# jolideco/jolideco

Hardware: AMD Instinct MI355X
Metric: MAP iters/sec at 2048x2048, 8-obs joint fit (higher is better)
Workload: dtype f32; 1 GPU; c3: 2048x2048, 8 observations (Gaussian PSFs sigma = 1.5 + 0.25 i on 6 x 17x17 + 2 x 33x33, varying exposure/background), GMM patch prior 8x8 stride 4 K=128, joint fit, Adam lr 0.1; global_observations=8, conv_method=separable

## Files before the change

include/jolideco_hip.h:

```cpp
#ifndef JOLIDECO_HIP_H
#define JOLIDECO_HIP_H

#include <stddef.h>
#include <stdint.h>

#ifdef __cplusplus
extern "C" {
#endif

typedef enum {
  JD_OK = 0,
  JD_ERR_INVALID = -1,
  JD_ERR_HIP = -2,
  JD_ERR_FFT = -3,
  JD_ERR_ALLOC = -4
} jd_status;

#define JD_MAX_COMPONENTS 8

typedef struct jd_conv_plan jd_conv_plan;
typedef struct jd_gmm jd_gmm;

int jd_version(void);
const char* jd_last_error(void);
// ... 14 lines not shown
int jd_conv_plan_destroy(jd_conv_plan* plan);
int jd_conv_plan_shape(const jd_conv_plan* plan, int* shape6);
int jd_conv_plan_method(const jd_conv_plan* plan);
int jd_conv_native_fft_supported(int H, int W, int kh, int kw);
int jd_conv_plan_takes_walk(const jd_conv_plan* plan, int n_datasets);
int jd_conv_plan_step_route(const jd_conv_plan* plan, int upsampling, int n_datasets, int32_t* route8);
int jd_conv_operator_walk_frame(const jd_conv_plan* plan, const float* khat);
int jd_conv_operator_forget(const float* khat);
size_t jd_conv_plan_spectrum_size(const jd_conv_plan* plan);

int jd_conv_psf_spectrum(jd_conv_plan* plan, const float* psf, float* khat, void* stream);

int jd_conv_same(jd_conv_plan* plan, const float* image, const float* scale_image, const float* khat,
                 float* out, void* stream);

int jd_npred_poisson_fwd_bwd(jd_conv_plan* plan, int n_comp, const float* const* flux,
                             const float* const* exposure, const float* const* khat,
                             const float* background, const float* counts, float stirling_mean,
                             float eps, float* loss_out, float* const* grad_flux, int accumulate,
                             float grad_scale, float* npred_out, int upsampling, void* stream);

int jd_npred_poisson_mixed_fwd_bwd(jd_conv_plan* const* plans, int n_comp, const float* const* flux,
                                   const float* const* exposure, const float* const* khat, const float* background,
                                   const float* counts, float stirling_mean, float eps, float* loss_out,
                                   float* const* grad_flux, int accumulate, float grad_scale, float* npred_out,
                                   const int* upsampling, void* stream);

int jd_npred_poisson_batch_fwd_bwd(jd_conv_plan* plan, int n_datasets, const float* flux, const float* const* exposure,
                                   const float* const* khat, const float* const* background,
                                   const float* const* counts, const float* stirling_mean, float eps,
                                   float* const* loss_out, float* grad_flux, int accumulate, float grad_scale,
                                   void* stream);

int jd_npred_poisson_batch_multi_fwd_bwd(jd_conv_plan* plan, int n_datasets, int n_components, const float* const* flux,
                                         const float* const* exposure, const float* const* khat,
                                         const float* const* background, const float* const* counts,
                                         const float* stirling_mean, float eps, float* const* loss_out,
                                         float* const* grad_flux, int accumulate, float grad_scale, void* stream);

int jd_npred_poisson_calibrated_fwd_bwd(jd_conv_plan* plan, int n_comp, const float* const* flux,
                                        const float* const* exposure, const float* const* khat,
                                        const float* background, const float* counts, float stirling_mean,
                                        float eps, float* loss_out, float* const* grad_flux, int accumulate,
                                        float grad_scale, float* npred_out, int upsampling, const float* shift_xy,
                                        const float* log_background_norm, float* grad_shift_xy,
                                        float* grad_log_background_norm, void* stream);

int jd_npred_poisson_calibrated_batch_fwd_bwd(jd_conv_plan* plan, int n_datasets, const float* flux,
                                              const float* const* exposure, const float* const* khat,
                                              const float* const* background, const float* const* counts,
                                              const float* stirling_mean, float eps, float* const* loss_out,
                                              float* grad_flux, int accumulate, float grad_scale, int upsampling,
                                              const float* const* shift_xy, const float* const* log_background_norm,
                                              float* const* grad_shift_xy, float* const* grad_log_background_norm,
                                              void* stream);

int jd_poisson_nll(const float* npred, const float* counts, size_t n, float stirling_mean, float eps,
                   float* loss_out, float* grad_npred ,
                   void* stream);
int jd_conv_same_adjoint(jd_conv_plan* plan, const float* grad_out, const float* scale_image,
                         const float* khat, float* grad_image, int accumulate, void* stream);

int jd_gmm_create(int K, int D, const float* prec_chol, const float* mu_prec, const float* const_k,
                  const float* pixel_w, jd_gmm** gmm_out);
int jd_gmm_destroy(jd_gmm* gmm);
int jd_gmm_is_triangular(const jd_gmm* gmm);

typedef struct {
  int kind;
  float p0, p1;
} jd_image_norm;
int jd_gmm_set_image_norm(jd_gmm* gmm, const jd_image_norm* norm);

int jd_gmm_prior_fwd_bwd(jd_gmm* gmm, const float* flux, int H, int W, int stride, int shift_y,
                         int shift_x, int patch_row_begin, int patch_row_end, int marginalize,
                         float value_scale, float* value_out, int accumulate_value, float grad_coef,
                         float* grad_flux_accum, int32_t* argmax_out, const int* shift_dev, int phases, void* stream);

typedef struct {
  float* theta;
  const float* flux_in;
  float* flux_out;
  const float* grad_flux;
  float* exp_avg;
  float* exp_avg_sq;
  const float* mask;
  float step_size, beta1, beta2, one_minus_beta1, one_minus_beta2, bias2_sqrt, eps;
  float lr;
  int use_log_flux, sgd;
  const float* bias_dev;
} jd_step;
int jd_gmm_prior_fwd_bwd_step(jd_gmm* gmm, const float* flux, int H, int W, int stride, int shift_y, int shift_x,
                              int marginalize, float value_scale, float* value_out, int accumulate_value,
                              float grad_coef, const jd_step* step, const int* shift_dev, int phases, void* stream);

int jd_gmm_screen_stats(const jd_gmm* gmm, int* out);
int jd_gmm_screen_clock(jd_gmm* gmm, double* mhz_out, int* samples_out);

int jd_gmm_prior_band_fwd_bwd(jd_gmm* gmm, const float* flux, int H, int W, int stride, int shift_y,
                              int shift_x, int patch_row_begin, int patch_row_end, int marginalize,
                              float value_scale, float* value_out, int accumulate_value, float grad_coef,
                              float* band_out, void* stream);
int jd_add_rolled_bands(float* grad, int H, int W, int shift_y, int shift_x, const float* bands, size_t chunk_floats,
                        int n_bands, const int* y_begin, const int* y_end, void* stream);
int jd_add_rolled_bands_step(int H, int W, int shift_y, int shift_x, const float* bands, size_t chunk_floats, int n_bands,
                             const int* y_begin, const int* y_end, const jd_step* step, void* stream);

int jd_gmm_estimate_log_prob(jd_gmm* gmm, const float* x, int n, float* out, void* stream);

int jd_elementwise_prior_fwd_bwd(int kind, const float* flux, size_t n, float alpha, float beta,
                                 float log_const, float* value_out, float grad_coef,
                                 float* grad_flux_accum, void* stream);
int jd_elementwise_prior_subpix_fwd_bwd(int kind, const float* flux, int H, int W, float alpha, float beta,
                                        float log_const, float x0, float y0, const float* offset_dev,
                                        float* value_out, float grad_coef, float* grad_flux_accum, void* stream);
int jd_smoothness_prior_fwd_bwd(jd_conv_plan* plan, const float* khat, const float* flux, float* value_out,
                                float grad_coef, float* grad_flux_accum, void* stream);

int jd_flux_from_theta(const float* theta, const float* mask, float* flux, size_t n, int use_log_flux, void* stream);

int jd_sum_images(float* out, const float* const* srcs, int n_srcs, size_t n, void* stream);
int jd_copy_image_to(const float* src, float* const* dsts, int n_dsts, size_t n, void* stream);

int jd_step_scalars_fetch(const int32_t* host_row, int32_t* dst, int n, void* stream);

int jd_adam_step(float* theta, const float* flux_in, float* flux_out, float* grad_flux, float* exp_avg,
                 float* exp_avg_sq, const float* mask, size_t n, float step_size, float beta1,
                 float beta2, float one_minus_beta1, float one_minus_beta2, float bias2_sqrt, float eps,
                 int zero_grad, int use_log_flux, const float* bias_dev, void* stream);
int jd_adam_step_multi(int n_tensors, float* const* theta, const float* const* grad, float* const* exp_avg,
                       float* const* exp_avg_sq, const int* sizes, const float* step_size, const float* bias2_sqrt,
                       float beta1, float beta2, float one_minus_beta1, float one_minus_beta2, float eps,
                       const float* bias_dev, void* stream);
int jd_sgd_step(float* theta, const float* flux_in, float* flux_out, float* grad_flux,
                const float* mask, size_t n, float lr, int zero_grad, int use_log_flux, void* stream);

int jd_sparse_max_sources(void);
int jd_sparse_render(const float* param_flux, const float* x_pos, const float* y_pos, int n, int use_log_flux, int H,
                     int W, float* flux_out, void* stream);
int jd_sparse_backward(const float* param_flux, const float* x_pos, const float* y_pos, int n, int use_log_flux, int H,
                       int W, const float* grad_flux_image, float* grad_param, float* grad_x, float* grad_y,
                       void* stream);

enum {
  JD_KERNEL_POISSON_FUSED = 0,
  JD_KERNEL_GMM_FWD = 1,
  JD_KERNEL_GMM_BWD = 2,
  JD_KERNEL_GMM_GATHER = 3,
  JD_KERNEL_PAD_MUL = 4,
  JD_KERNEL_CMUL = 5,
  JD_KERNEL_ADJOINT_EPILOGUE = 6,
  JD_KERNEL_ADAM = 7,
  JD_KERNEL_FFT_R2C = 8,
  JD_KERNEL_FFT_C2R = 9,
  JD_KERNEL_DIRECT_CONV = 10,
  JD_KERNEL_SEP_CONV = 11,
  JD_KERNEL_GMM_SCREEN = 12,
  JD_KERNEL_GMM_SORT = 13,
  JD_KERNEL_GMM_EXACT = 14,
  JD_KERNEL_GMM_STAGE = 15,
  JD_KERNEL_SHIFT = 16,
  JD_KERNEL_POISSON_MIXED = 17,
// ... 19 lines not shown
```

jolideco_amd/_hip.py:

```python
import ctypes
import os
from ctypes import POINTER, c_char_p, c_double, c_float, c_int, c_int32, c_longlong, c_size_t, c_void_p
from pathlib import Path

import torch

__all__ = ["lib", "library_path", "check", "ptr", "stream_ptr", "EXPORTS"]

LIB_NAME = "libjolideco_hip.so"


def library_path():
    override = os.environ.get("JOLIDECO_HIP_LIBRARY")
    return Path(override) if override else Path(__file__).resolve().parent / LIB_NAME


fp = POINTER(c_float)
fpp = POINTER(c_void_p)

EXPORTS = {
    "jd_version": (c_int, []),
    "jd_last_error": (c_char_p, []),
    "jd_target_arch": (c_char_p, []),
    "jd_set_option": (c_int, [c_char_p, c_char_p]),
# ... 6 lines not shown
    "jd_conv_native_fft_supported": (c_int, [c_int, c_int, c_int, c_int]),
    "jd_conv_plan_takes_walk": (c_int, [c_void_p, c_int]),
    "jd_conv_plan_step_route": (c_int, [c_void_p, c_int, c_int, POINTER(c_int32)]),
    "jd_conv_operator_walk_frame": (c_int, [c_void_p, c_void_p]),
    "jd_conv_operator_forget": (c_int, [c_void_p]),
    "jd_psf_separable_rank": (c_int, [c_void_p, c_int, c_int, c_float]),
    "jd_conv_psf_spectrum": (c_int, [c_void_p, c_void_p, c_void_p, c_void_p]),
    "jd_conv_same": (c_int, [c_void_p, c_void_p, c_void_p, c_void_p, c_void_p, c_void_p]),
    "jd_conv_same_adjoint": (c_int, [c_void_p, c_void_p, c_void_p, c_void_p, c_void_p, c_int, c_void_p]),
    "jd_npred_poisson_fwd_bwd": (
        c_int,
        [c_void_p, c_int, fpp, fpp, fpp, c_void_p, c_void_p, c_float, c_float, c_void_p, fpp, c_int, c_float,
         c_void_p, c_int, c_void_p],
    ),
    "jd_npred_poisson_mixed_fwd_bwd": (
        c_int,
        [fpp, c_int, fpp, fpp, fpp, c_void_p, c_void_p, c_float, c_float, c_void_p, fpp, c_int, c_float, c_void_p,
         POINTER(c_int), c_void_p],
    ),
    "jd_npred_poisson_calibrated_fwd_bwd": (
        c_int,
        [c_void_p, c_int, fpp, fpp, fpp, c_void_p, c_void_p, c_float, c_float, c_void_p, fpp, c_int, c_float,
         c_void_p, c_int, c_void_p, c_void_p, c_void_p, c_void_p, c_void_p],
    ),
    "jd_npred_poisson_calibrated_batch_fwd_bwd": (
        c_int,
        [c_void_p, c_int, c_void_p, fpp, fpp, fpp, fpp, fp, c_float, fpp, c_void_p, c_int, c_float, c_int, fpp, fpp, fpp, fpp,
         c_void_p],
    ),
    "jd_npred_poisson_batch_fwd_bwd": (
        c_int,
        [c_void_p, c_int, c_void_p, fpp, fpp, fpp, fpp, fp, c_float, fpp, c_void_p, c_int, c_float, c_void_p],
    ),
    "jd_npred_poisson_batch_multi_fwd_bwd": (
        c_int,
        [c_void_p, c_int, c_int, fpp, fpp, fpp, fpp, fpp, fp, c_float, fpp, fpp, c_int, c_float, c_void_p],
    ),
    "jd_poisson_nll": (c_int, [c_void_p, c_void_p, c_size_t, c_float, c_float, c_void_p, c_void_p, c_void_p]),
    "jd_gmm_create": (c_int, [c_int, c_int, fp, fp, fp, fp, POINTER(c_void_p)]),
    "jd_gmm_destroy": (c_int, [c_void_p]),
    "jd_gmm_is_triangular": (c_int, [c_void_p]),
    "jd_gmm_set_image_norm": (c_int, [c_void_p, c_void_p]),
    "jd_gmm_prior_fwd_bwd": (
        c_int,
        [c_void_p, c_void_p, c_int, c_int, c_int, c_int, c_int, c_int, c_int, c_int, c_float, c_void_p, c_int,
         c_float, c_void_p, c_void_p, c_void_p, c_int, c_void_p],
    ),
    "jd_gmm_prior_fwd_bwd_step": (
        c_int,
        [c_void_p, c_void_p, c_int, c_int, c_int, c_int, c_int, c_int, c_float, c_void_p, c_int, c_float, c_void_p, c_void_p,
         c_int, c_void_p],
    ),
    "jd_gmm_screen_stats": (c_int, [c_void_p, POINTER(c_int)]),
    "jd_gmm_screen_clock": (c_int, [c_void_p, POINTER(c_double), POINTER(c_int)]),
    "jd_gmm_prior_band_fwd_bwd": (
        c_int,
        [c_void_p, c_void_p, c_int, c_int, c_int, c_int, c_int, c_int, c_int, c_int, c_float, c_void_p, c_int,
         c_float, c_void_p, c_void_p],
    ),
    "jd_add_rolled_bands": (
        c_int, [c_void_p, c_int, c_int, c_int, c_int, c_void_p, c_size_t, c_int, POINTER(c_int), POINTER(c_int), c_void_p],
    ),
    "jd_add_rolled_bands_step": (
        c_int, [c_int, c_int, c_int, c_int, c_void_p, c_size_t, c_int, POINTER(c_int), POINTER(c_int), c_void_p, c_void_p],
    ),
    "jd_gmm_estimate_log_prob": (c_int, [c_void_p, c_void_p, c_int, c_void_p, c_void_p]),
    "jd_elementwise_prior_fwd_bwd": (
        c_int,
        [c_int, c_void_p, c_size_t, c_float, c_float, c_float, c_void_p, c_float, c_void_p, c_void_p],
    ),
    "jd_elementwise_prior_subpix_fwd_bwd": (
        c_int,
        [c_int, c_void_p, c_int, c_int, c_float, c_float, c_float, c_float, c_float, c_void_p, c_void_p, c_float, c_void_p,
         c_void_p],
    ),
    "jd_smoothness_prior_fwd_bwd": (c_int, [c_void_p, c_void_p, c_void_p, c_void_p, c_float, c_void_p, c_void_p]),
    "jd_flux_from_theta": (c_int, [c_void_p, c_void_p, c_void_p, c_size_t, c_int, c_void_p]),
    "jd_sum_images": (c_int, [c_void_p, c_void_p, c_int, c_size_t, c_void_p]),
    "jd_copy_image_to": (c_int, [c_void_p, c_void_p, c_int, c_size_t, c_void_p]),
    "jd_step_scalars_fetch": (c_int, [c_void_p, c_void_p, c_int, c_void_p]),
    "jd_adam_step": (
        c_int,
        [c_void_p, c_void_p, c_void_p, c_void_p, c_void_p, c_void_p, c_void_p, c_size_t, c_float, c_float, c_float,
         c_float, c_float, c_float, c_float, c_int, c_int, c_void_p, c_void_p],
    ),
    "jd_adam_step_multi": (
        c_int,
        [c_int, fpp, fpp, fpp, fpp, POINTER(c_int), fp, fp, c_float, c_float, c_float, c_float, c_float, c_void_p, c_void_p],
    ),
    "jd_sgd_step": (c_int, [c_void_p, c_void_p, c_void_p, c_void_p, c_void_p, c_size_t, c_float, c_int, c_int, c_void_p]),
    "jd_sparse_max_sources": (c_int, []),
    "jd_sparse_render": (c_int, [c_void_p, c_void_p, c_void_p, c_int, c_int, c_int, c_int, c_void_p, c_void_p]),
    "jd_sparse_backward": (
        c_int, [c_void_p, c_void_p, c_void_p, c_int, c_int, c_int, c_int, c_void_p, c_void_p, c_void_p, c_void_p, c_void_p],
    ),
    "jd_profile_enable": (c_int, [c_int]),
    "jd_profile_disable": (c_int, []),
    "jd_profile_pause": (c_int, [c_int]),
    "jd_profile_read": (c_int, [c_int, POINTER(c_double), POINTER(c_longlong)]),
    "jd_kernel_name": (c_char_p, [c_int]),
    "jd_clock_probe": (c_int, [c_double, POINTER(c_double), c_void_p]),
}

class Step(ctypes.Structure):

    _fields_ = [
        ("theta", c_void_p), ("flux_in", c_void_p), ("flux_out", c_void_p), ("grad_flux", c_void_p), ("exp_avg", c_void_p),
        ("exp_avg_sq", c_void_p), ("mask", c_void_p),
        ("step_size", c_float), ("beta1", c_float), ("beta2", c_float), ("one_minus_beta1", c_float),
        ("one_minus_beta2", c_float), ("bias2_sqrt", c_float), ("eps", c_float), ("lr", c_float),
        ("use_log_flux", c_int), ("sgd", c_int), ("bias_dev", c_void_p),
    ]


class ImageNormStruct(ctypes.Structure):

    _fields_ = [("kind", c_int), ("p0", c_float), ("p1", c_float)]


KERNEL_IDS = {
    "poisson_fused": 0, "gmm_fwd": 1, "gmm_bwd": 2, "gmm_gather": 3, "pad_mul": 4, "cmul": 5,
    "adjoint_epilogue": 6, "adam": 7, "fft_r2c": 8, "fft_c2r": 9, "direct_conv": 10, "sep_conv": 11,
    "gmm_screen": 12, "gmm_sort": 13, "gmm_exact": 14, "gmm_stage": 15, "shift": 16,
    "poisson_mixed": 17, "elementwise_subpix": 18, "smoothness": 19, "elementwise_prior": 20,
    "sparse_render": 21, "sparse_backward": 22,
}

_lib = None


def lib():
    global _lib
    if _lib is None:
        path = library_path()
        if not path.exists():
            raise RuntimeError(
                f"{path} not found: the HIP extension is required (no CPU fallback). "
                "Build it with `make -C jolideco_amd/csrc` or `python -c 'import __graft_entry__ as g; g.build()'`."
            )
        handle = ctypes.CDLL(str(path))
        for name, (restype, argtypes) in EXPORTS.items():
            fn = getattr(handle, name)
            fn.restype = restype
            fn.argtypes = argtypes
# ... 102 lines not shown
```

jolideco_amd/core.py:

```python
import copy
import ctypes
import os
import logging
from pathlib import Path

import numpy as np
import torch

from . import _hip
from ._hip import check, ptr, ptr_array, stream_ptr
from .distributed import DistContext
from .loss import TotalLoss
from .models import FluxComponents, SparseSpatialFluxComponent, SpatialFluxComponent
from .ops import adam_bias_terms, sparse_backward, sparse_render
from .utils.torch import TORCH_DEFAULT_DEVICE

log = logging.getLogger(__name__)

__all__ = ["MAPDeconvolver", "MAPDeconvolverResult", "FitSession"]

OPTIMIZER = ("adam", "sgd")
FIT_MODES = ("sequential", "joint")


# ... 115 lines not shown
        self.device = device
        if optimizer_type not in OPTIMIZER:
            raise ValueError(f"Unknown optimizer: {optimizer_type}, must be one of {OPTIMIZER}")
        self.optimizer_type = optimizer_type
        self.optimizer_kwargs = dict(optimizer_kwargs or {})
        self.optimizer_kwargs.setdefault("lr", self.learning_rate)
        unknown = set(self.optimizer_kwargs) - {"lr", "betas", "eps"}
        if unknown:
            raise NotImplementedError(f"optimizer_kwargs {sorted(unknown)} are not implemented in jolideco_amd")
        if checkpoint_path is not None:
            checkpoint_path = Path(checkpoint_path)
            checkpoint_path.mkdir(exist_ok=True, parents=True)
        self.checkpoint_path = checkpoint_path
        if fit_mode not in FIT_MODES:
            raise ValueError(f"Unknown fit_mode: {fit_mode}, must be one of {FIT_MODES}")
        self.fit_mode = fit_mode

    def to_dict(self):
        data = {k: v for k, v in self.__dict__.items() if k not in ("optimizer_kwargs",)}
        data["device"] = str(self.device)
        data["checkpoint_path"] = str(self.checkpoint_path)
        return data

    def __str__(self):
        lines = [self.__class__.__name__, "-" * len(self.__class__.__name__), ""]
        lines += [f"  {k:22s}: {v}" for k, v in self.to_dict().items()]
        return "\n".join(lines)

    def _step_args(self, st, step, bias_dev=None):
        lr = self.optimizer_kwargs["lr"]
        args = _hip.Step()
        args.theta, args.flux_in, args.flux_out = st.theta.data_ptr(), st.flux_cur.data_ptr(), st.flux[1 - st.cur].data_ptr()
        args.grad_flux = st.grad.data_ptr()
        args.mask = None if st.mask is None else st.mask.data_ptr()
        args.use_log_flux = int(st.use_log_flux)
        if self.optimizer_type == "adam":
            beta1, beta2 = self.optimizer_kwargs.get("betas", (0.9, 0.999))
            args.step_size, args.bias2_sqrt = adam_bias_terms(step, lr, beta1, beta2)
            args.beta1, args.beta2, args.one_minus_beta1, args.one_minus_beta2 = beta1, beta2, 1 - beta1, 1 - beta2
            args.eps = self.optimizer_kwargs.get("eps", 1e-8)
            args.exp_avg, args.exp_avg_sq = st.exp_avg.data_ptr(), st.exp_avg_sq.data_ptr()
            args.sgd = 0
            args.bias_dev = None if bias_dev is None else bias_dev.data_ptr()
        else:
            args.lr, args.sgd = lr, 1
        return args

    def _optimizer_step(self, states, step, stepped=()):
        lib = _hip.lib()
        lr = self.optimizer_kwargs["lr"]
        for ci, st in enumerate(states):
            n = st.grad.numel()
            stream = stream_ptr(st.grad.device)
            if ci in stepped:
                pass
            elif st.frozen:
                st.flux[1 - st.cur].copy_(st.flux_cur)
                st.grad.zero_()
            elif getattr(st, "is_sparse", False):
                st.step(step)
            elif self.optimizer_type == "adam":
                beta1, beta2 = self.optimizer_kwargs.get("betas", (0.9, 0.999))
                eps = self.optimizer_kwargs.get("eps", 1e-8)
                step_size, bias2_sqrt = adam_bias_terms(step, lr, beta1, beta2)
                check(
                    lib.jd_adam_step(
# ... 325 lines not shown

        from . import _hip as _hip_mod

        own_step = getattr(type(deconvolver), "_optimizer_step", None) is MAPDeconvolver._optimizer_step
        tiled = _hip_mod.get_option("JD_GMM_GATHER_TILED") in (None, 1)
        self.fuse_optimizer_step = bool(own_step and "_optimizer_step" not in vars(deconvolver) and tiled
                                        and not os.environ.get("JOLIDECO_NO_FUSED_STEP"))
        self._setup_sharded_prior(os.environ.get("JOLIDECO_DIST_OVERLAP", "1") != "0")
        batchable = not os.environ.get("JOLIDECO_NO_BATCH") and self.total_loss.poisson_loss.batchable(
            [li for _, li in self.local_idx]
        )
        self.batch_joint = self.joint and batchable
        self.flux_nonneg = all(
            st.use_log_flux and (st.mask is None or bool((st.mask >= 0).all())) for st in self.states
        )
        self.batch_joint_calibrated = bool(
            self.joint and not batchable and not os.environ.get("JOLIDECO_NO_BATCH") and self.n_c == 1
            and self.total_loss.poisson_loss.batchable_calibrated([li for _, li in self.local_idx])
        )
        self.batch_trace = (not self.joint) and batchable
        mode = os.environ.get("JOLIDECO_GRAPH", "auto").lower()
        self.graph_mode = {"1": "always", "on": "always", "0": "never", "off": "never"}.get(mode, "auto")
        if getattr(deconvolver, "use_graph", None) is not None:
            self.graph_mode = "always" if deconvolver.use_graph else "never"
        self.use_graph = self.graph_mode == "always"
        self.graph_policy = {"always": "captured epochs (forced)", "never": "no capture (forced)"}.get(self.graph_mode, "undecided")
        self._probe = []
        self._trial = None
        self.overlap_mode = {"1": "on", "0": "off"}.get(os.environ.get("JOLIDECO_PRIOR_OVERLAP", ""), "auto")
        self.overlap_prior = self.overlap_mode != "off"
        side_priority = int(os.environ.get("JOLIDECO_PRIOR_STREAM_PRIORITY", "0"))
        self._side_stream = (torch.cuda.Stream(device=device, priority=side_priority)
                             if torch.device(device).type == "cuda" else None)
        self.step_scalars = None
        self._graphs = {}
        self._epochs_done = 0
        self._total_epochs = 0
        self._planned_ok = os.environ.get("JOLIDECO_STEP_SCALARS", "device") != "host"

    def gather_calibrations(self):
        cals, dist = self.calibrations, self.dist
        if cals is None or not (self.joint and dist.sharded) or dist.dry_run:
            return
        names = self.total_loss.poisson_loss.names_all_global
        mine = {names[gslot] for gslot, _ in self.local_idx}
        flat = torch.zeros(3 * len(names), dtype=torch.float32, device=self.comm.device)
        for i, name in enumerate(names):
            if name in mine and name in cals:
                cal = cals[name]
                flat[3 * i : 3 * i + 2] = cal.shift_xy.detach().reshape(-1).to(flat.device)
                flat[3 * i + 2] = cal._background_norm.detach().reshape(-1)[0].to(flat.device)
        dist.all_reduce_sum(flat)
        host = flat.cpu()
        for i, name in enumerate(names):
            if name not in mine and name in cals:
                cal = cals[name]
                with torch.no_grad():
                    cal.shift_xy.copy_(host[3 * i : 3 * i + 2].reshape(1, 2))
                    cal._background_norm.copy_(host[3 * i + 2 : 3 * i + 3])

    def _setup_sharded_prior(self, overlap):
        from .ops import band_rows

        self.band_plan = None
        dist = self.dist
        if not (self.joint and dist.sharded):
# ... 168 lines not shown
            H, W = self.states[ci].shape
            shifts_host.append((drawn[0] % H, drawn[1] % W))
            return DeviceShifts(slot, drawn)

        if len(drawing) == 1:
            ci = drawing[0]
            for drawn in self.priors[ci].draw_shifts_many(n_eval):
                shifts.append({ci: place(ci, drawn)})
        else:
            for _ in range(n_eval):
                shifts.append({ci: place(ci, self.priors[ci].draw_shifts()) for ci in drawing})
        biases = [adam_bias_terms(self.step + j + 1, lr, beta1, beta2) if adam else (0.0, 1.0) for j in range(n_flux)]
        flux_bias = [sc.bias_slots[j] if adam else None for j in range(n_flux)]
        cal_bias, cal_items, k = [], [], n_flux
        for group in cal_groups:
            items = [(p, st) for opt in group for p, st in zip(opt.params, opt.state) if p.grad is not None]
            for _, st in items:
                biases.append(adam_bias_terms(st["step"] + 1, lr, beta1, beta2) if adam else (0.0, 1.0))
            cal_bias.append(sc.bias_range(k, len(items)) if (adam and items) else None)
            cal_items.append(items)
            k += len(items)
        sc.upload(shifts_host, biases)
        return {"shifts": shifts, "flux_bias": flux_bias, "cal_bias": cal_bias, "cal_items": cal_items, "n_steps": n_flux,
                "signature": tuple(len(items) for items in cal_items)}

    def _plan_by_value(self):
        drawing, _, n_flux, cal_groups, _ = self._plan_slots()
        n_eval = 1 if self.joint else len(self.local_idx) + 1
        shifts = [{ci: self.priors[ci].draw_shifts() for ci in drawing} for _ in range(n_eval)]
        cal_items = [[(p, st) for opt in group for p, st in zip(opt.params, opt.state)] for group in cal_groups]
        return {"shifts": shifts, "flux_bias": [None] * n_flux, "cal_bias": [None] * len(cal_groups), "cal_items": cal_items,
                "n_steps": n_flux, "signature": ()}

    def _overlap_active(self):
        return self.overlap_prior and self._side_stream is not None and not self.dist.sharded and not _hip.profile_active()

    def _prior_calls(self, coef, shifts, bias):
        cfg, n_d, slot, step_no = self.cfg, self.n_d, self._slot, self.step + 1
        calls = []
        for ci, (st, prior) in enumerate(zip(self.states, self.priors)):
            if getattr(prior, "value_is_zero", False):
                continue
            kwargs = {"shifts": shifts[ci]} if ci in shifts else {}
            flux, value = st.flux_cur, slot(n_d + ci)
            if self._fuse_step(st, prior):
                args = cfg._step_args(st, step_no, bias)

                def call(phases=3, prior=prior, flux=flux, value=value, args=args, kwargs=kwargs):
                    prior.device_fwd_bwd_step(flux, value, coef, args, **(dict(kwargs, phases=phases) if phases != 3 else kwargs))

                calls.append((ci, call, True))
            else:

                def call(phases=3, prior=prior, flux=flux, value=value, grad=st.grad, kwargs=kwargs):
                    prior.device_fwd_bwd(flux, value, grad=grad, coef=coef, **(dict(kwargs, phases=phases) if phases != 3 else kwargs))

                calls.append((ci, call, False))
        return calls

    def _start_priors(self, calls):
        if not self._overlap_active():
            return set()
        eligible, seen = [], set()
        for ci, call, _ in calls:
            prior = self.priors[ci]
            key = id(getattr(prior, "gmm", prior))
            if getattr(prior, "supports_phases", False) and key not in seen:
                seen.add(key)
                eligible.append((ci, call))
        if not eligible:
            return set()
        main = torch.cuda.current_stream(self.comm.device)
        self._side_stream.wait_stream(main)
        with torch.cuda.stream(self._side_stream):
            for _, call in eligible:
                call(1)
        return {ci for ci, _ in eligible}

    def _finish_priors(self, calls, early):
        if early:
            torch.cuda.current_stream(self.comm.device).wait_stream(self._side_stream)
# ... 54 lines not shown
        beta = -float(cfg.beta)

        def flux_step(stepped, bias):
            self.step += 1
            for st in states:
                st.bias_dev = bias
            try:
                self._apply_step(states, stepped)
            finally:
                for st in states:
                    st.bias_dev = None

        def cal_steps(items, bias):
            if not items:
                return
            if cfg.optimizer_type != "adam":
                lr = cfg.optimizer_kwargs["lr"]
                for p, st in items:
                    if p.grad is None:
                        continue
                    st["step"] += 1
                    check(_hip.lib().jd_sgd_step(ptr(p.data), ptr(p.data), ptr(p.data), ptr(p.grad), None, p.numel(), lr, 0, 0,
                                                 stream_ptr(p.device)))
                return
            _adam_step_many(cfg, items, self.__dict__.setdefault("_cal_step_cache", {}), bias)

        if self.joint:
            fluxes = [st.flux_cur for st in states]
            grads = [st.grad for st in states]
            calls = self._prior_calls(beta, plan["shifts"][0], plan["flux_bias"][0])
            early = self._start_priors(calls)
            first = True
            if self.batch_joint:
                total_loss.poisson_loss.fwd_bwd_batch(
                    [li for _, li in self.local_idx], fluxes if n_c > 1 else fluxes[0],
                    [slot(gslot) for gslot, _ in self.local_idx], grad=grads if n_c > 1 else grads[0], accumulate=False,
                    flux_nonneg=self.flux_nonneg,
                )
                first = False
            elif self.batch_joint_calibrated:
                for _, li in self.local_idx:
                    self._cal_zero_grad(li)
                total_loss.poisson_loss.fwd_bwd_batch_calibrated(
                    [li for _, li in self.local_idx], fluxes[0], [slot(gslot) for gslot, _ in self.local_idx], grad=grads[0],
                    accumulate=False,
                )
                first = False
            else:
                for gslot, li in self.local_idx:
                    self._cal_zero_grad(li)
                    total_loss.poisson_loss.fwd_bwd(li, fluxes, slot(gslot), grads=grads, accumulate=not first,
                                                    flux_nonneg=self.flux_nonneg)
                    first = False
            if first:
                for g in grads:
                    g.zero_()
            flux_step(self._finish_priors(calls, early), plan["flux_bias"][0])
            cal_steps(plan["cal_items"][0], plan["cal_bias"][0])
        else:
            coef = beta / total_loss.prior_weight
            for j, (gslot, li) in enumerate(self.local_idx):
                fluxes = [st.flux_cur for st in states]
                grads = [st.grad for st in states]
                calls = self._prior_calls(coef, plan["shifts"][j], plan["flux_bias"][j])
                early = self._start_priors(calls)
                self._cal_zero_grad(li)
                total_loss.poisson_loss.fwd_bwd(li, fluxes, slot(gslot), grads=grads, accumulate=False,
                                                flux_nonneg=self.flux_nonneg)
                flux_step(self._finish_priors(calls, early), plan["flux_bias"][j])
                cal_steps(plan["cal_items"][j], plan["cal_bias"][j])
            stale = [st.flux_trace for st in states]
# ... 91 lines not shown
        trial["times"][self.overlap_prior] = 1e-3 * float(np.median([a.elapsed_time(b) for a, b in trial["events"][2:]]))
        trial["events"] = []
        remaining = [form for form in trial["forms"] if form not in trial["times"]]
        if remaining:
            self.overlap_prior, self._graphs, self._epochs_done = remaining[0], {}, 0
            return
        times, by_value_s = trial["times"], trial["by_value"]
        best = min(times, key=times.get)
        self._trial = None
        replays = " / ".join(f"{1e6 * t:.0f} us {'on two streams' if form else 'on one stream'}" for form, t in times.items())
        numbers = (f"replayed {replays} / by value {1e6 * by_value_s:.0f} us per epoch, enqueue {1e6 * trial['host']:.0f} us"
                   f"{trial['streams']}")
        if times[best] <= self.AUTO_MARGIN * by_value_s:
            self.graph_policy = f"captured epochs (measured: {numbers})"
            if best != self.overlap_prior:
                self.overlap_prior, self._graphs, self._epochs_done = best, {}, 0
        else:
            self.use_graph = False
            self._graphs = {}
            self.overlap_prior = trial["by_value_form"]
            self.graph_policy = f"by value (measured: {numbers})"

    def _epoch_by_value(self):
        cfg, dist, states, priors, total_loss = self.cfg, self.dist, self.states, self.priors, self.total_loss
        n_d, n_c = self.n_d, self.n_c
        slot = self._slot
        if self.joint:
            fluxes = [st.flux_cur for st in states]
            grads = [st.grad for st in states]
            if dist.sharded:
                self.scalars.zero_()
            first = True
            if self.batch_joint:
                total_loss.poisson_loss.fwd_bwd_batch(
                    [li for _, li in self.local_idx], fluxes if n_c > 1 else fluxes[0],
                    [slot(gslot) for gslot, _ in self.local_idx], grad=grads if n_c > 1 else grads[0], accumulate=False,
                    flux_nonneg=self.flux_nonneg,
                )
                first = False
            elif self.batch_joint_calibrated:
                for _, li in self.local_idx:
                    self._cal_zero_grad(li)
                total_loss.poisson_loss.fwd_bwd_batch_calibrated(
                    [li for _, li in self.local_idx], fluxes[0], [slot(gslot) for gslot, _ in self.local_idx], grad=grads[0],
                    accumulate=False,
                )
                first = False
            else:
                for gslot, li in self.local_idx:
                    self._cal_zero_grad(li)
                    total_loss.poisson_loss.fwd_bwd(li, fluxes, slot(gslot), grads=grads, accumulate=not first,
                                                    flux_nonneg=self.flux_nonneg)
                    first = False
            if first:
                for g in grads:
                    g.zero_()
            banded = {item["ci"]: item for item in (self.band_plan or [])}
            stepped = set()
            for ci, (st, prior) in enumerate(zip(states, priors)):
                if ci in banded:
                    continue
                if dist.sharded and not prior.shardable and dist.rank != 0:
                    continue
                if self._fuse_step(st, prior):
                    prior.device_fwd_bwd_step(st.flux_cur, slot(n_d + ci), -float(cfg.beta), cfg._step_args(st, self.step + 1))
                    stepped.add(ci)
                    continue
                prior.device_fwd_bwd(
                    st.flux_cur, slot(n_d + ci), grad=st.grad, coef=-float(cfg.beta),
                    patch_rows=self._prior_rows(prior, st),
                )
# ... 199 lines not shown
```

jolideco_amd/csrc/elementwise.hip:

```cpp
#include <cstdint>
#include <cstdlib>

#include "jd_common.h"
#include "kernels.h"
#include "jd_adam.h"

namespace jd {

constexpr int BLOCK = 256;

__global__ __launch_bounds__(BLOCK) void finalize_sum_kernel(const double* __restrict__ partials, int n,
                                                            double scale, double offset,
                                                            float* __restrict__ out, int accumulate) {
  __shared__ double smem[BLOCK / 64];
  double acc = 0.0;
  for (int i = threadIdx.x; i < n; i += BLOCK) acc += partials[i];
  double total = block_sum<BLOCK>(acc, smem);
  if (threadIdx.x == 0) {
    double v = scale * total + offset;
    if (accumulate) v += (double)out[0];
    out[0] = (float)v;
  }
}

// ... 531 lines not shown
                                                    int ox) {
  const int y = blockIdx.y;
  const int x = blockIdx.x * BLOCK + threadIdx.x;
  if (x >= W) return;
  out[(size_t)y * W + x] = padded[(size_t)(y + oy) * Wp + (x + ox)];
}

int launch_crop(const float* padded, float* out, int H, int W, int Wp, int oy, int ox, hipStream_t stream) {
  dim3 grid((W + BLOCK - 1) / BLOCK, H);
  crop_kernel<<<grid, BLOCK, 0, stream>>>(padded, out, H, W, Wp, oy, ox);
  JD_LAUNCH_CHECK();
  return JD_OK;
}

__global__ __launch_bounds__(BLOCK) void poisson_nll_kernel(const float* __restrict__ npred,
                                                           const float* __restrict__ counts, size_t n,
                                                           float eps, float inv_n,
                                                           float* __restrict__ grad,
                                                           double* __restrict__ partials) {
  __shared__ double smem[BLOCK / 64];
  double local = 0.0;
  const size_t stride = (size_t)gridDim.x * BLOCK;
  for (size_t i = (size_t)blockIdx.x * BLOCK + threadIdx.x; i < n; i += stride) {
    const float v = npred[i], c = counts[i];
    float term, g;
    poisson_point(v, c, eps, inv_n, term, g);
    local += (double)term;
    if (grad) grad[i] = g;
  }
  const double total = block_sum<BLOCK>(local, smem);
  if (threadIdx.x == 0) partials[blockIdx.x] = total;
}

template <int VEC>
__global__ __launch_bounds__(BLOCK) void adam_kernel(AdamArgs a) {
  use_device_bias(a);
  const size_t stride = (size_t)gridDim.x * BLOCK * VEC;
  for (size_t i = ((size_t)blockIdx.x * BLOCK + threadIdx.x) * VEC; i < a.n; i += stride) {
    float th[VEC], f[VEC], gf[VEC], m[VEC], v[VEC], mk[VEC];
    if constexpr (VEC == 4) {
      const float4 t4 = *reinterpret_cast<const float4*>(a.theta + i);
      const float4 f4 = *reinterpret_cast<const float4*>(a.flux_in + i);
      const float4 g4 = *reinterpret_cast<const float4*>(a.grad_flux + i);
      th[0] = t4.x, th[1] = t4.y, th[2] = t4.z, th[3] = t4.w;
      f[0] = f4.x, f[1] = f4.y, f[2] = f4.z, f[3] = f4.w;
      gf[0] = g4.x, gf[1] = g4.y, gf[2] = g4.z, gf[3] = g4.w;
      if (!a.sgd) {
        const float4 m4 = *reinterpret_cast<const float4*>(a.m + i);
        const float4 v4 = *reinterpret_cast<const float4*>(a.v + i);
        m[0] = m4.x, m[1] = m4.y, m[2] = m4.z, m[3] = m4.w;
        v[0] = v4.x, v[1] = v4.y, v[2] = v4.z, v[3] = v4.w;
      }
      mk[0] = mk[1] = mk[2] = mk[3] = 1.f;
      if (a.mask) {
        const float4 k4 = *reinterpret_cast<const float4*>(a.mask + i);
        mk[0] = k4.x, mk[1] = k4.y, mk[2] = k4.z, mk[3] = k4.w;
      }
    } else {
      th[0] = a.theta[i], f[0] = a.flux_in[i], gf[0] = a.grad_flux[i];
      if (!a.sgd) m[0] = a.m[i], v[0] = a.v[i];
      mk[0] = a.mask ? a.mask[i] : 1.f;
    }
#pragma unroll
    for (int k = 0; k < VEC; ++k) adam_pixel(th[k], f[k], m[k], v[k], gf[k], mk[k], a);
    if constexpr (VEC == 4) {
      *reinterpret_cast<float4*>(a.theta + i) = make_float4(th[0], th[1], th[2], th[3]);
      *reinterpret_cast<float4*>(a.flux_out + i) = make_float4(f[0], f[1], f[2], f[3]);
      if (!a.sgd) {
        *reinterpret_cast<float4*>(a.m + i) = make_float4(m[0], m[1], m[2], m[3]);
        *reinterpret_cast<float4*>(a.v + i) = make_float4(v[0], v[1], v[2], v[3]);
      }
      if (a.zero_grad) *reinterpret_cast<float4*>(a.grad_flux + i) = make_float4(0.f, 0.f, 0.f, 0.f);
    } else {
      a.theta[i] = th[0], a.flux_out[i] = f[0];
      if (!a.sgd) a.m[i] = m[0], a.v[i] = v[0];
      if (a.zero_grad) a.grad_flux[i] = 0.f;
    }
  }
}

static int launch_adam(const AdamArgs& a, hipStream_t stream) {
  const bool vec = (a.n % 4 == 0);
  const size_t per_block = (size_t)BLOCK * (vec ? 4 : 1);
  size_t blocks = (a.n + per_block - 1) / per_block;
  if (blocks > 4096) blocks = 4096;
  if (blocks == 0) blocks = 1;
  ProfScope prof(JD_KERNEL_ADAM, stream);
  if (vec)
    adam_kernel<4><<<(unsigned)blocks, BLOCK, 0, stream>>>(a);
  else
    adam_kernel<1><<<(unsigned)blocks, BLOCK, 0, stream>>>(a);
  JD_LAUNCH_CHECK();
  return JD_OK;
}

__global__ __launch_bounds__(BLOCK) void flux_from_theta_kernel(const float* __restrict__ theta,
                                                               const float* __restrict__ mask,
                                                               float* __restrict__ flux, size_t n, int linear) {
  const size_t stride = (size_t)gridDim.x * BLOCK;
  for (size_t i = (size_t)blockIdx.x * BLOCK + threadIdx.x; i < n; i += stride) {
    float f = linear ? theta[i] : expf(theta[i]);
    if (mask) f *= mask[i];
    flux[i] = f;
  }
}

__global__ __launch_bounds__(BLOCK) void elementwise_prior_kernel(int kind, const float* __restrict__ flux,
                                                                 size_t n, float alpha, float beta,
                                                                 float coef, float* __restrict__ grad,
                                                                 double* __restrict__ partials) {
  __shared__ double smem[BLOCK / 64];
  double local = 0.0;
  const size_t stride = (size_t)gridDim.x * BLOCK;
  for (size_t i = (size_t)blockIdx.x * BLOCK + threadIdx.x; i < n; i += stride) {
    const float f = flux[i];
    float value, dv;
    if (kind == 1) {
      value = -beta / f + (-alpha - 1.f) * logf(f);
      dv = beta / (f * f) + (-alpha - 1.f) / f;
    } else {
      value = -alpha * f;
      dv = -alpha;
    }
    local += (double)value;
// ... 323 lines not shown
  ImagePtrs p{};
  for (int c = 0; c < n_srcs; ++c) {
    JD_REQUIRE(srcs[c], "jd_sum_images: source %d is null", c);
    p.src[c] = srcs[c];
  }
  p.n_src = n_srcs, p.dst[0] = out, p.n_dst = 1;
  return launch_sum_images(p, n, stream);
}

extern "C" int jd_copy_image_to(const float* src, float* const* dsts, int n_dsts, size_t n, void* stream) {
  JD_REQUIRE(src && dsts && n > 0, "jd_copy_image_to: null argument or n == 0");
  JD_REQUIRE(n_dsts >= 1 && n_dsts <= 4, "jd_copy_image_to: %d destination images (1 to 4)", n_dsts);
  ImagePtrs p{};
  p.src[0] = src, p.n_src = 1;
  for (int d = 0; d < n_dsts; ++d) {
    JD_REQUIRE(dsts[d] && dsts[d] != src, "jd_copy_image_to: destination %d is null or the source", d);
    p.dst[d] = dsts[d];
  }
  p.n_dst = n_dsts;
  return launch_sum_images(p, n, stream);
}

__global__ __launch_bounds__(256) void fetch_scalars_kernel(const int* __restrict__ src, int* __restrict__ dst, int n) {
  for (int i = threadIdx.x; i < n; i += 256) dst[i] = src[i];
}

extern "C" int jd_step_scalars_fetch(const int32_t* host_row, int32_t* dst, int n, void* stream) {
  JD_REQUIRE(host_row && dst && n > 0 && n <= (1 << 20), "jd_step_scalars_fetch: null argument or bad n");
  fetch_scalars_kernel<<<1, 256, 0, as_stream(stream)>>>(host_row, dst, n);
  JD_LAUNCH_CHECK();
  return JD_OK;
}

extern "C" int jd_adam_step(float* theta, const float* flux_in, float* flux_out, float* grad_flux,
                            float* exp_avg, float* exp_avg_sq, const float* mask, size_t n, float step_size,
                            float beta1, float beta2, float one_minus_beta1, float one_minus_beta2,
                            float bias2_sqrt, float eps, int zero_grad, int use_log_flux, const float* bias_dev,
                            void* stream) {
  JD_REQUIRE(theta && flux_in && flux_out && grad_flux && exp_avg && exp_avg_sq && n > 0,
             "jd_adam_step: null argument or n == 0");
  AdamArgs a{theta, flux_in, flux_out, grad_flux, exp_avg, exp_avg_sq, mask, n,
             step_size, beta1, beta2, one_minus_beta1, one_minus_beta2, bias2_sqrt, eps, 0.f, zero_grad, 0,
             use_log_flux ? 0 : 1, bias_dev};
  return launch_adam(a, as_stream(stream));
}

constexpr int ADAM_MULTI_MAX = 64;
struct AdamMultiArgs {
  float* theta[ADAM_MULTI_MAX];
  const float* grad[ADAM_MULTI_MAX];
  float* m[ADAM_MULTI_MAX];
  float* v[ADAM_MULTI_MAX];
  int size[ADAM_MULTI_MAX];
  float step_size[ADAM_MULTI_MAX], bias2_sqrt[ADAM_MULTI_MAX];
  float beta1, beta2, one_minus_beta1, one_minus_beta2, eps;
  const float* bias_dev;
};

__global__ __launch_bounds__(64) void adam_multi_kernel(AdamMultiArgs a) {
  float* theta = nullptr;
  const float* grad = nullptr;
  float *m = nullptr, *v = nullptr;
  int size = 0;
  AdamArgs s{};
  s.beta1 = a.beta1, s.beta2 = a.beta2, s.one_minus_beta1 = a.one_minus_beta1, s.one_minus_beta2 = a.one_minus_beta2, s.eps = a.eps;
#pragma unroll
  for (int i = 0; i < ADAM_MULTI_MAX; ++i)
    if ((int)blockIdx.x == i) {
      theta = a.theta[i], grad = a.grad[i], m = a.m[i], v = a.v[i], size = a.size[i];
      s.step_size = a.step_size[i], s.bias2_sqrt = a.bias2_sqrt[i];
    }
  if (a.bias_dev) s.step_size = a.bias_dev[2 * blockIdx.x], s.bias2_sqrt = a.bias_dev[2 * blockIdx.x + 1];
  for (int j = threadIdx.x; j < size; j += 64) {
    float th = theta[j], mj = m[j], vj = v[j];
    adam_update(th, mj, vj, grad[j], s);
    theta[j] = th, m[j] = mj, v[j] = vj;
  }
// ... 36 lines not shown
```

jolideco_amd/csrc/fftconv.hip:

```cpp
#include <rocfft/rocfft.h>

#include <algorithm>
#include <cstdio>
#include <cstdlib>
#include <mutex>

#include "jd_common.h"
#include "kernels.h"

#define JD_FFT(call)                                                                               \
  do {                                                                                             \
    rocfft_status s_ = (call);                                                                     \
    if (s_ != rocfft_status_success)                                                               \
      return jd::fail(JD_ERR_FFT, "%s failed with rocfft_status %d (%s:%d)", #call, (int)s_,       \
                      __FILE__, __LINE__);                                                         \
  } while (0)

struct jd_conv_plan {
  int H = 0, W = 0, kh = 0, kw = 0, Hp = 0, Wp = 0, oy = 0, ox = 0;
  int method = jd::JD_CONV_FFT;
  int py = 0, px = 0;
  size_t nspec = 0;
  int split = 0;
  bool native = false;
  jd::FftNative fftn;
  rocfft_plan fwd = nullptr, inv = nullptr;
  rocfft_execution_info info = nullptr;
  void* work = nullptr;
  size_t work_bytes = 0;
  float* pad[JD_MAX_COMPONENTS] = {nullptr};
  float* conv[JD_MAX_COMPONENTS] = {nullptr};
  float2* spec = nullptr;
  double* partials = nullptr;
  int partials_cap = 0;
  float* shifted[JD_MAX_COMPONENTS] = {nullptr};
  float* gshift[JD_MAX_COMPONENTS] = {nullptr};
  double* partials_cal = nullptr;
  float* gbatch[jd::SEP_MAX_BATCH * jd::SEP_BATCH_MAX_COMP] = {nullptr};
  double* partials_batch = nullptr;
  int partials_batch_cap = 0;
  float2* fft_extra_spec[jd::FFT_MAX_BATCH - 1] = {nullptr};
  float2* fft_extra_work[jd::FFT_MAX_BATCH - 1] = {nullptr};
  static constexpr int N_FFT_TABLES = 6;
  jd::FftBatch fft_batch_host[N_FFT_TABLES] = {};
  jd::FftBatch* fft_batch_dev[N_FFT_TABLES] = {};
  unsigned long long fft_batch_used[N_FFT_TABLES] = {};
  unsigned long long fft_batch_clock = 0;
  double* partials_shift_batch = nullptr;
  float* gshift_batch[jd::FFT_MAX_BATCH] = {nullptr};
  int partials_shift_batch_cap = 0;
  static constexpr int N_TABLES = 8;
  jd::SepBatchTable table_host[N_TABLES] = {};
  jd::SepBatchTable* table_dev[N_TABLES] = {};
  unsigned long long table_used[N_TABLES] = {};
  unsigned long long table_clock = 0;
};

namespace jd {

static bool is_smooth(int n) {
  for (int p : {2, 3, 5})
    while (n % p == 0) n /= p;
  return n == 1;
}

static int next_fast_len(int n, int mult) {
  int m = ((n + mult - 1) / mult) * mult;
  while (!is_smooth(m)) m += mult;
  return m;
}

static int ensure_component_buffers(jd_conv_plan* p, int n_comp) {
  const size_t bytes = (size_t)p->Hp * p->Wp * sizeof(float);
  for (int c = 0; c < n_comp; ++c) {
    if (!p->pad[c]) JD_HIP(hipMalloc(&p->pad[c], bytes));
    if (!p->conv[c]) JD_HIP(hipMalloc(&p->conv[c], bytes));
  }
  return JD_OK;
}

static int ensure_calibration_buffers(jd_conv_plan* p, int n_comp, bool shift) {
  if (!p->partials_cal) {
    const size_t n = (size_t)(p->partials_cap > 2 * shift_bwd_max_blocks(p->H, p->W) ? p->partials_cap
                                                                                    : 2 * shift_bwd_max_blocks(p->H, p->W));
    JD_HIP(hipMalloc(&p->partials_cal, n * sizeof(double)));
  }
  if (shift) {
    const size_t bytes = (size_t)p->H * p->W * sizeof(float);
// ... 188 lines not shown
    return cleanup(fail(JD_ERR_ALLOC, "jd_conv_plan_create: hipMalloc of the spectrum buffer failed"));
  p->partials_cap = poisson_fused_max_partials(p->Hp, p->Wp);
  if (hipMalloc(&p->partials, (size_t)p->partials_cap * sizeof(double)) != hipSuccess)
    return cleanup(fail(JD_ERR_ALLOC, "jd_conv_plan_create: hipMalloc of the partial sums failed"));
  int rc = ensure_component_buffers(p, 1);
  if (rc) return cleanup(rc);
  *plan_out = p;
  return JD_OK;
}

extern "C" int jd_conv_plan_destroy(jd_conv_plan* p) {
  if (!p) return JD_OK;
  (void)hipDeviceSynchronize();
  if (p->native) fftn_destroy(&p->fftn);
  for (int i = 0; i < jd::FFT_MAX_BATCH - 1; ++i) {
    if (p->fft_extra_spec[i]) (void)hipFree(p->fft_extra_spec[i]);
    if (p->fft_extra_work[i]) (void)hipFree(p->fft_extra_work[i]);
  }
  for (auto* t : p->fft_batch_dev)
    if (t) (void)hipFree(t);
  if (p->partials_shift_batch) (void)hipFree(p->partials_shift_batch);
  for (int i = 0; i < jd::FFT_MAX_BATCH; ++i)
    if (p->gshift_batch[i]) (void)hipFree(p->gshift_batch[i]);
  if (p->fwd) rocfft_plan_destroy(p->fwd);
  if (p->inv) rocfft_plan_destroy(p->inv);
  if (p->info) rocfft_execution_info_destroy(p->info);
  if (p->work) (void)hipFree(p->work);
  if (p->spec) (void)hipFree(p->spec);
  if (p->partials) (void)hipFree(p->partials);
  if (p->partials_cal) (void)hipFree(p->partials_cal);
  if (p->partials_batch) (void)hipFree(p->partials_batch);
  for (auto* t : p->table_dev)
    if (t) (void)hipFree(t);
  for (float* g : p->gbatch)
    if (g) (void)hipFree(g);
  for (int c = 0; c < JD_MAX_COMPONENTS; ++c) {
    if (p->pad[c]) (void)hipFree(p->pad[c]);
    if (p->conv[c]) (void)hipFree(p->conv[c]);
    if (p->shifted[c]) (void)hipFree(p->shifted[c]);
    if (p->gshift[c]) (void)hipFree(p->gshift[c]);
  }
  delete p;
  return JD_OK;
}

extern "C" int jd_conv_plan_shape(const jd_conv_plan* p, int* shape6) {
  JD_REQUIRE(p && shape6, "jd_conv_plan_shape: null argument");
  shape6[0] = p->H, shape6[1] = p->W, shape6[2] = p->Hp, shape6[3] = p->Wp, shape6[4] = p->oy, shape6[5] = p->ox;
  return JD_OK;
}

extern "C" size_t jd_conv_plan_spectrum_size(const jd_conv_plan* p) { return p ? p->nspec : 0; }

extern "C" int jd_conv_plan_method(const jd_conv_plan* p) { return p ? p->method : -1; }

extern "C" int jd_conv_native_fft_supported(int H, int W, int kh, int kw) {
  return H > 0 && W > 0 && kh > 0 && kw > 0 && opt_value(OPT_FFT_NATIVE, 1) != 0 && fftn_supported(H, W, kh, kw) ? 1 : 0;
}

extern "C" int jd_conv_plan_takes_walk(const jd_conv_plan* p, int n_datasets) {
  if (!p || p->method != JD_CONV_SEPARABLE || n_datasets < 1) return 0;
  return walk_takes_launch(p->H, p->W, n_datasets, p->kh, p->kw, p->oy, p->ox) ? 1 : 0;
}

extern "C" int jd_conv_operator_walk_frame(const jd_conv_plan* p, const float* khat) {
  if (!p || !khat || p->method != JD_CONV_SEPARABLE) return 0;
// ... 260 lines not shown
      if (plans[k] == p) ++slot[c];
  }
  jd_conv_plan* p0 = plans[0];
  JD_REQUIRE(poisson_mixed_max_partials(Hd, Wd) <= p0->partials_cap, "%s: partial sums of a (%d, %d) counts grid do not fit plans[0]",
             who, Hd, Wd);
  hipStream_t s = as_stream(stream);
  int rc = JD_OK;
  for (int c = 0; c < n_comp; ++c)
    if ((rc = ensure_component_buffers(plans[c], slot[c] + 1))) return rc;

  for (int c = 0; c < n_comp; ++c)
    if ((rc = conv_forward(plans[c], slot[c], flux[c], exposure[c], khat[c], s))) return rc;

  PoissonMixedArgs a{};
  for (int c = 0; c < n_comp; ++c) {
    const jd_conv_plan* p = plans[c];
    a.conv[c] = p->conv[slot[c]], a.g[c] = p->pad[slot[c]];
    a.up[c] = upsampling[c], a.Wp[c] = p->Wp, a.oy[c] = p->py, a.ox[c] = p->px;
  }
  const double n_pix = (double)Hd * (double)Wd;
  a.background = background, a.counts = counts, a.npred_out = npred_out, a.partials = p0->partials;
  a.n_comp = n_comp, a.Hd = Hd, a.Wd = Wd, a.eps = eps, a.inv_n = (float)(1.0 / n_pix);
  a.write_grad = grad_flux ? 1 : 0;
  int n_partials = 0;
  if ((rc = launch_poisson_mixed(a, &n_partials, s))) return rc;
  if ((rc = launch_finalize_sum(p0->partials, n_partials, 1.0 / n_pix, (double)stirling_mean, loss_out, 0, s))) return rc;
  if (!grad_flux) return JD_OK;

  for (int c = 0; c < n_comp; ++c)
    if ((rc = corr_backward_into(plans[c], slot[c], khat[c], exposure[c], grad_flux[c], grad_scale, accumulate, s))) return rc;
  return JD_OK;
}

extern "C" int jd_npred_poisson_batch_multi_fwd_bwd(jd_conv_plan* p, int n_datasets, int n_comp, const float* const* flux,
                                                    const float* const* exposure, const float* const* khat,
                                                    const float* const* background, const float* const* counts,
                                                    const float* stirling_mean, float eps, float* const* loss_out,
                                                    float* const* grad_flux, int accumulate, float grad_scale,
                                                    void* stream) {
  const char* who = "jd_npred_poisson_batch_multi_fwd_bwd";
  JD_REQUIRE(p && flux && exposure && khat && background && counts && stirling_mean && loss_out, "%s: null argument", who);
  JD_REQUIRE(p->method == JD_CONV_SEPARABLE || (p->native && n_comp == 1),
             "%s: the plan must use the separable method, or the native FFT path with one flux component (one "
             "jd_npred_poisson_fwd_bwd per dataset otherwise)", who);
  if (p->native) {
    JD_REQUIRE(flux[0], "%s: flux[0] is null", who);
    for (int d = 0; d < n_datasets; ++d)
      JD_REQUIRE(exposure[d] && khat[d] && background[d] && counts[d] && loss_out[d], "%s: null pointer for dataset %d", who, d);
    hipStream_t s = as_stream(stream);
    if (!grad_flux || !grad_flux[0] || n_datasets > FFT_MAX_BATCH || n_datasets < 2 || n_datasets > p->fftn.Hh ||
        opt_is_set(OPT_SEP_NO_FUSION) || opt_value(OPT_FFT_BATCH, 1) == 0) {
      for (int d = 0; d < n_datasets; ++d) {
        int rc = npred_poisson_impl(who, p, 1, flux, exposure + d, khat + d, background[d], counts[d], stirling_mean[d], eps,
                                    loss_out[d], grad_flux, accumulate || d > 0, grad_scale, nullptr, 1, Calibration{}, stream);
        if (rc) return rc;
      }
      return JD_OK;
    }
    const FftNative& fn = p->fftn;
    for (int d = 0; d + 1 < n_datasets; ++d) {
      if (!p->fft_extra_spec[d]) JD_HIP(hipMalloc(&p->fft_extra_spec[d], (size_t)fn.Hh * fn.Nx * sizeof(float2)));
      if (!p->fft_extra_work[d]) JD_HIP(hipMalloc(&p->fft_extra_work[d], (size_t)fn.Ny * fn.Nx * sizeof(float2)));
    }
    if (p->partials_batch_cap < n_datasets * fn.Hh) {
      if (p->partials_batch) (void)hipFree(p->partials_batch);
      p->partials_batch = nullptr, p->partials_batch_cap = 0;
      JD_HIP(hipMalloc(&p->partials_batch, (size_t)n_datasets * fn.Hh * sizeof(double)));
      p->partials_batch_cap = n_datasets * fn.Hh;
    }
    FftBatch batch{};
    batch.n = n_datasets;
    for (int d = 0; d < n_datasets; ++d) {
      batch.exposure[d] = exposure[d], batch.khat[d] = reinterpret_cast<const float2*>(khat[d]);
// ... 20 lines not shown
      JD_REQUIRE(exposure[d * n_comp + c] && khat[d * n_comp + c], "%s: null exposure or operator for dataset %d, component %d",
                 who, d, c);
  }
  hipStream_t s = as_stream(stream);
  {
    SepBatchTable probe{};
    for (int d = 0; d < n_datasets; ++d) probe.bkg[d] = background[d], probe.cnt[d] = counts[d];
    for (int i = 0; i < n_datasets * n_comp; ++i) probe.scale[i] = exposure[i], probe.op[i] = khat[i], probe.g[i] = nullptr;
    if (sep_batch_is_mixed(n_datasets, n_comp, probe, p->H, p->W, p->kh, p->kw, p->oy, p->ox)) {
      for (int d = 0; d < n_datasets; ++d) {
        int rc = npred_poisson_impl(who, p, n_comp, flux, exposure + d * n_comp, khat + d * n_comp, background[d], counts[d],
                                    stirling_mean[d], eps, loss_out[d], grad_flux, accumulate || d > 0, grad_scale, nullptr,
                                    1, Calibration{}, stream);
        if (rc) return rc;
      }
      return JD_OK;
    }
  }
  const size_t bytes = (size_t)p->H * p->W * sizeof(float);
  for (int i = 0; i < n_datasets * n_comp; ++i)
    if (!p->gbatch[i]) JD_HIP(hipMalloc(&p->gbatch[i], bytes));
  const int tiles = sep_conv_tiles(p->H, p->W);
  if (p->partials_batch_cap < n_datasets * tiles) {
    if (p->partials_batch) (void)hipFree(p->partials_batch);
    p->partials_batch = nullptr, p->partials_batch_cap = 0;
    JD_HIP(hipMalloc(&p->partials_batch, (size_t)n_datasets * tiles * sizeof(double)));
    p->partials_batch_cap = n_datasets * tiles;
  }
  SepBatchTable table{};
  for (int d = 0; d < n_datasets; ++d) table.bkg[d] = background[d], table.cnt[d] = counts[d];
  for (int i = 0; i < n_datasets * n_comp; ++i) table.scale[i] = exposure[i], table.op[i] = khat[i], table.g[i] = p->gbatch[i];
  for (int d = 0; d < n_datasets; ++d) table.loss_out[d] = loss_out[d], table.loss_offset[d] = stirling_mean[d];
  walk_batch_order(table, n_datasets, n_comp, p->kh, p->kw, p->oy, p->ox);
  int slot = -1, victim = 0;
  for (int i = 0; i < jd_conv_plan::N_TABLES; ++i) {
    if (p->table_used[i] && memcmp(&table, &p->table_host[i], sizeof(table)) == 0) slot = i;
    if (p->table_used[i] < p->table_used[victim]) victim = i;
  }
  if (slot < 0) {
    slot = victim;
    if (!p->table_dev[slot]) JD_HIP(hipMalloc(&p->table_dev[slot], sizeof(SepBatchTable)));
    if (p->table_used[slot]) JD_HIP(hipStreamSynchronize(s));
    JD_HIP(hipMemcpy(p->table_dev[slot], &table, sizeof(table), hipMemcpyHostToDevice));
    p->table_host[slot] = table;
  }
  p->table_used[slot] = ++p->table_clock;
  SepBatchTable* const table_dev = p->table_dev[slot];
  const double n_pix = (double)p->H * (double)p->W;
  int n_part = 0;
  if (n_comp == 1 && grad_flux) {
    int rc = walk_joint_step(n_datasets, flux[0], table, table_dev, grad_flux[0], p->H, p->W, p->kh, p->kw, p->oy, p->ox,
                             p->partials_batch, eps, (float)(1.0 / n_pix), grad_scale, accumulate, &n_part, s);
    if (rc != JD_WALK_NOT_TAKEN)
      return rc ? rc : launch_finalize_rows(p->partials_batch, n_part, n_datasets, 1.0 / n_pix, stirling_mean, loss_out, s);
  }
  int rc = launch_sep_conv_poisson_batch(n_datasets, n_comp, flux, table, table_dev, p->H, p->W, p->kh, p->kw, p->oy, p->ox,
                                         p->partials_batch, eps, (float)(1.0 / n_pix), grad_flux ? 1 : 0, &n_part, s);
  if (rc) return rc;
  if (!grad_flux) return launch_finalize_rows(p->partials_batch, n_part, n_datasets, 1.0 / n_pix, stirling_mean, loss_out, s);
  int folded = 0;
  rc = walk_conv_adjoint_batch_all(n_datasets, n_comp, table, table_dev, grad_flux, p->H, p->W, p->kh, p->kw, p->oy, p->ox,
                                   grad_scale, accumulate, s, p->partials_batch, 1.0 / n_pix, n_part, &folded);
  if (rc != JD_WALK_NOT_TAKEN) {
    if (rc || folded) return rc;
    return launch_finalize_rows(p->partials_batch, n_part, n_datasets, 1.0 / n_pix, stirling_mean, loss_out, s);
  }
  for (int c = 0; c < n_comp; ++c) {
    int done = 0;
    if ((rc = launch_sep_conv_adjoint_batch(n_datasets, n_comp, c, table, table_dev, grad_flux[c], p->H, p->W, p->kh,
                                            p->kw, p->oy, p->ox, grad_scale, accumulate, s,
                                            c == 0 && n_datasets <= 8 ? p->partials_batch : nullptr, 1.0 / n_pix, n_part,
                                            &done)))
      return rc;
    folded |= done;
  }
  if (!folded) return launch_finalize_rows(p->partials_batch, n_part, n_datasets, 1.0 / n_pix, stirling_mean, loss_out, s);
  return JD_OK;
}

extern "C" int jd_npred_poisson_batch_fwd_bwd(jd_conv_plan* p, int n_datasets, const float* flux,
                                              const float* const* exposure, const float* const* khat,
                                              const float* const* background, const float* const* counts,
                                              const float* stirling_mean, float eps, float* const* loss_out,
                                              float* grad_flux, int accumulate, float grad_scale, void* stream) {
  JD_REQUIRE(flux, "jd_npred_poisson_batch_fwd_bwd: null argument");
  const float* fluxes[1] = {flux};
  float* grads[1] = {grad_flux};
  return jd_npred_poisson_batch_multi_fwd_bwd(p, n_datasets, 1, fluxes, exposure, khat, background, counts, stirling_mean,
                                              eps, loss_out, grad_flux ? grads : nullptr, accumulate, grad_scale, stream);
}

static int calibrated_batch_form(const jd_conv_plan* p, int n_datasets, int upsampling, bool with_grad) {
  const int mode = opt_value(OPT_FFT_BATCH, 1);
  const bool batched = p->native && with_grad && n_datasets >= 2 && n_datasets <= FFT_MAX_BATCH &&
                       fftn_pooled_supported(p->fftn, upsampling) && !opt_is_set(OPT_SEP_NO_FUSION) && mode != 0 &&
                       (p->fftn.Hh <= 1024 || mode != 3);
  return !batched ? 0 : p->fftn.Hh > 1024 && mode == 4 ? 2 : 1;
}

extern "C" int jd_conv_plan_step_route(const jd_conv_plan* p, int upsampling, int n_datasets, int32_t* route8) {
  JD_REQUIRE(p && route8, "jd_conv_plan_step_route: null argument");
  JD_REQUIRE(upsampling >= 1 && upsampling <= 8 && n_datasets >= 1, "jd_conv_plan_step_route: upsampling = %d, n_datasets = %d",
             upsampling, n_datasets);
  const int form = calibrated_batch_form(p, n_datasets, upsampling, true);
  int fft[6] = {0, 0, -1, -1, 0, 0};
  if (p->native) fftn_step_route(p->fftn, upsampling, form == 1 ? n_datasets : 1, fft);
  for (int i = 0; i < 6; ++i) route8[i] = fft[i];
  route8[6] = form;
  route8[7] = shift_bwd_route(p->H, p->W);
  return JD_OK;
// ... 102 lines not shown
```

jolideco_amd/csrc/gmm.hip:

```cpp
#include <memory>

#include "gmm_internal.h"

using namespace jd;

extern "C" int jd_gmm_create(int K, int Dn, const float* prec_chol, const float* mu_prec, const float* const_k,
                             const float* pixel_w, jd_gmm** gmm_out) {
  JD_REQUIRE(gmm_out && prec_chol && mu_prec && const_k && pixel_w, "jd_gmm_create: null argument");
  JD_REQUIRE(K >= 1 && K <= BUCKET_MAX_K, "jd_gmm_create: K = %d out of range [1, %d]", K, BUCKET_MAX_K);
  JD_REQUIRE(Dn == D || Dn == 256, "jd_gmm_create: only 8x8 and 16x16 patches (D = 64 or D = 256) are supported, got D = %d", Dn);
  std::unique_ptr<jd_gmm> g(new (std::nothrow) jd_gmm());
  if (!g) return fail(JD_ERR_ALLOC, "jd_gmm_create: out of host memory");
  g->K = K;
  if (Dn == 256) {
    if (const int rc256 = gmm256_create(K, prec_chol, mu_prec, const_k, pixel_w, &g->d256)) return rc256;
    *gmm_out = g.release();
    return JD_OK;
  }

  std::vector<float> afrag((size_t)K * AFRAG_FLOATS), gfrag((size_t)K * AFRAG_FLOATS), mfrag((size_t)K * 64),
      prow((size_t)D * D), mrow(D);
  double sw[D];
  for (int j = 0; j < D; ++j) sw[j] = std::sqrt((double)pixel_w[j]);
  bool tri = true;
// ... 292 lines not shown
    if ((rc = g->dense.gpatch.reserve((size_t)n * D))) return rc;
    if (!lse_screened && !marginalize && !fused) {
      if ((rc = bucketed_backward(g, flux, grid, n_begin, n_end, arg, s))) return rc;
    }

    g->pass = GmmPass{true, H, W, stride, shift_y, shift_x, patch_row_begin, patch_row_end, marginalize, fused, lse_screened, g->screen.gen, shift_dev, norm};
    if (!(phases & 2)) return JD_OK;
  } else {
    const GmmPass& ps = g->pass;
    JD_REQUIRE(ps.valid && ps.H == H && ps.W == W && ps.stride == stride && ps.shift_y == shift_y && ps.shift_x == shift_x &&
                   ps.row_begin == patch_row_begin && ps.row_end == patch_row_end && ps.marginalize == marginalize &&
                   ps.gen == g->screen.gen && ps.shift_dev == shift_dev && grad_flux_accum && ps.norm.kind == norm.kind &&
                   ps.norm.p0 == norm.p0 && ps.norm.p1 == norm.p1,
               "jd_gmm_prior_fwd_bwd: phase 2 (gather) without the matching phase 1 of the same pass");
    fused = ps.fused, lse_screened = ps.lse_screened;
  }
  g->pass.valid = false;
  GmmGatherArgs ga{};
  set_patch_grid(ga, grid);
  ga.gpatch = g->dense.gpatch.ptr, ga.grad = grad_flux_accum, ga.nPy = nPy, ga.row_begin = patch_row_begin, ga.row_end = patch_row_end;
  ga.y_begin = patch_row_begin * stride;
  ga.y_end = (patch_row_end - 1) * stride + P;
  ga.coef = grad_coef;
  ga.band = band_out;
  ga.norm = norm, ga.raw_flux = raw_flux;
  if (fused) ga.winner = g->fused.winner.ptr, ga.grec = g->fused.grec.ptr, ga.flag = g->screen.ctl.ptr, ga.gen = g->screen.gen;
  auto aligned = [](const void* ptr) { return (reinterpret_cast<uintptr_t>(ptr) & 15) == 0; };
  ga.vec = W % 4 == 0 && aligned(grad_flux_accum) && (!has_norm || aligned(raw_flux)) ? 1 : 0;
  if (step) {
    ga.do_step = 1, ga.step = *step, ga.y_begin = 0, ga.y_end = H;
    ga.preload = opt_value(OPT_GMM_GATHER_PRELOAD, 1) != 0;
    ga.vec = ga.vec && aligned(step->theta) && aligned(step->flux_in) && aligned(step->flux_out) && aligned(step->m) &&
             aligned(step->v) && aligned(step->mask);
  }
  return launch_gather(ga, s);
}

extern "C" int jd_gmm_prior_fwd_bwd(jd_gmm* g, const float* flux, int H, int W, int stride, int shift_y,
                                    int shift_x, int patch_row_begin, int patch_row_end, int marginalize,
                                    float value_scale, float* value_out, int accumulate_value, float grad_coef,
                                    float* grad_flux_accum, int32_t* argmax_out, const int* shift_dev, int phases,
                                    void* stream) {
  if (g && g->d256) {
    JD_REQUIRE(flux && value_out, "jd_gmm_prior_fwd_bwd: null argument");
    JD_REQUIRE(phases == 3, "jd_gmm_prior_fwd_bwd: D = 256 handles run whole passes only (phases = %d, need 3)", phases);
    JD_REQUIRE(H >= 16 && W >= 16 && stride >= 1, "jd_gmm_prior_fwd_bwd: image (%d, %d) / stride %d not valid for D = 256", H, W, stride);
    const int nPy256 = (H - 16) / stride + 1;
    JD_REQUIRE(patch_row_begin == 0 && (patch_row_end < 0 || patch_row_end == nPy256),
               "jd_gmm_prior_fwd_bwd: D = 256 handles take no patch row shard ([%d, %d) of %d rows)", patch_row_begin,
               patch_row_end, nPy256);
    hipStream_t s = as_stream(stream);
    const ImageNormArgs norm = g->norm;
    const float* image = flux;
    if (norm.kind != NORM_IDENTITY) {
      int rc;
      if ((rc = g->normed.reserve((size_t)H * W))) return rc;
      if ((rc = launch_image_norm(flux, g->normed.ptr, (size_t)H * W, norm, g->n_cu, s))) return rc;
      image = g->normed.ptr;
    }
    return gmm256_prior(g->d256, image, flux, norm, H, W, stride, shift_y, shift_x, marginalize, value_scale, value_out,
                        accumulate_value, grad_coef, grad_flux_accum, argmax_out, shift_dev, s);
  }
  return gmm_prior_impl(g, flux, H, W, stride, shift_y, shift_x, patch_row_begin, patch_row_end, marginalize, value_scale,
                        value_out, accumulate_value, grad_coef, grad_flux_accum, argmax_out, nullptr, stream, nullptr, shift_dev,
                        phases);
}

extern "C" int jd_gmm_prior_fwd_bwd_step(jd_gmm* g, const float* flux, int H, int W, int stride, int shift_y, int shift_x,
                                         int marginalize, float value_scale, float* value_out, int accumulate_value,
                                         float grad_coef, const jd_step* step, const int* shift_dev, int phases,
                                         void* stream) {
  JD_REQUIRE(!(g && g->d256), "jd_gmm_prior_fwd_bwd_step: D = 256 handles have no fused optimizer step");
  JD_REQUIRE(step && step->theta && step->flux_in && step->flux_out && step->grad_flux, "jd_gmm_prior_fwd_bwd_step: null argument");
  JD_REQUIRE(step->sgd || (step->exp_avg && step->exp_avg_sq), "jd_gmm_prior_fwd_bwd_step: Adam needs its moment images");
  AdamArgs a{};
  a.theta = step->theta, a.flux_in = step->flux_in, a.flux_out = step->flux_out, a.grad_flux = const_cast<float*>(step->grad_flux);
  a.m = step->exp_avg, a.v = step->exp_avg_sq, a.mask = step->mask, a.n = (size_t)H * W;
  a.step_size = step->step_size, a.beta1 = step->beta1, a.beta2 = step->beta2, a.one_minus_beta1 = step->one_minus_beta1;
  a.one_minus_beta2 = step->one_minus_beta2, a.bias2_sqrt = step->bias2_sqrt, a.eps = step->eps, a.lr = step->lr;
  a.zero_grad = 0, a.sgd = step->sgd ? 1 : 0, a.linear = step->use_log_flux ? 0 : 1, a.bias_dev = step->bias_dev;
  return gmm_prior_impl(g, flux, H, W, stride, shift_y, shift_x, 0, -1, marginalize, value_scale, value_out, accumulate_value,
                        grad_coef, nullptr, nullptr, nullptr, stream, &a, shift_dev, phases);
}

extern "C" int jd_gmm_prior_band_fwd_bwd(jd_gmm* g, const float* flux, int H, int W, int stride, int shift_y,
                                         int shift_x, int patch_row_begin, int patch_row_end, int marginalize,
                                         float value_scale, float* value_out, int accumulate_value, float grad_coef,
                                         float* band_out, void* stream) {
  JD_REQUIRE(!(g && g->d256), "jd_gmm_prior_band_fwd_bwd: D = 256 handles have no band output");
  JD_REQUIRE(band_out, "jd_gmm_prior_band_fwd_bwd: null band");
  return gmm_prior_impl(g, flux, H, W, stride, shift_y, shift_x, patch_row_begin, patch_row_end, marginalize, value_scale,
                        value_out, accumulate_value, grad_coef, nullptr, nullptr, band_out, stream);
}
```

jolideco_amd/csrc/gmm_gather.hip:

```cpp
#include "gmm_internal.h"

namespace jd {


template <int KIND>
__global__ __launch_bounds__(256) void gmm_image_norm_kernel(const float* __restrict__ in, float* __restrict__ out, size_t n,
                                                             ImageNormArgs nm, size_t n4) {
  const size_t tid = (size_t)blockIdx.x * 256 + threadIdx.x, nthreads = (size_t)gridDim.x * 256;
  for (size_t i = tid; i < n4; i += nthreads) {
    const float4 v = reinterpret_cast<const float4*>(in)[i];
    reinterpret_cast<float4*>(out)[i] = make_float4(image_norm_value<KIND>(v.x, nm), image_norm_value<KIND>(v.y, nm),
                                                    image_norm_value<KIND>(v.z, nm), image_norm_value<KIND>(v.w, nm));
  }
  for (size_t i = 4 * n4 + tid; i < n; i += nthreads) out[i] = image_norm_value<KIND>(in[i], nm);
}

int launch_image_norm(const float* in, float* out, size_t n, const ImageNormArgs& nm, int n_cu, hipStream_t s) {
  const bool aligned = ((reinterpret_cast<uintptr_t>(in) | reinterpret_cast<uintptr_t>(out)) & 15) == 0;
  const size_t n4 = aligned ? n / 4 : 0;
  const size_t items = n4 + (n - 4 * n4);
  size_t blocks = (items + 255) / 256;
  const size_t cap = (size_t)n_cu * 8;
  if (blocks > cap) blocks = cap;
  if (blocks < 1) blocks = 1;
// ... 34 lines not shown
    const int r = Y - py * a.stride;
    for (int px = px_lo; px <= px_hi; ++px) {
      const int cc = X - px * a.stride;
      if (slots) {
        const int slot = a.winner[(size_t)py * a.nPx + px];
        if (slot >= 0) sum += a.grec[(size_t)slot * D + r * P + cc];
      } else {
        const size_t n = (size_t)(py - a.row_begin) * a.nPx + px;
        sum += a.gpatch[n * D + r * P + cc];
      }
      any = true;
    }
  }
  if (NORM) {
    const int yy = wrap(Y - a.shift_y, a.H), xx = wrap(X - a.shift_x, a.W);
    const size_t idx = (size_t)yy * a.W + xx;
    const bool live = any && sum != 0.f;
    const float term = live ? gather_normed_term(a, sum, a.raw_flux[idx]) : 0.f;
    if (a.band) a.band[(size_t)(Y - a.y_begin) * a.W + X] = term;
    else if (live) a.grad[idx] += term;
    return;
  }
  if (a.band) {
    a.band[(size_t)(Y - a.y_begin) * a.W + X] = any ? a.coef * sum : 0.f;
    return;
  }
  if (!any) return;
  const int yy = wrap(Y - a.shift_y, a.H), xx = wrap(X - a.shift_x, a.W);
  a.grad[(size_t)yy * a.W + xx] += a.coef * sum;
}

constexpr int GATHER_T = 32, GATHER_MAX_P = 9, GATHER_MAX_PX = GATHER_MAX_P + 1;

template <bool NORM>
__global__ __launch_bounds__(256) void gmm_gather_tile_kernel(GmmGatherArgs a) {
#pragma clang fp contract(off)
  use_device_shift(a);
  use_device_bias(a.step);
  __shared__ __attribute__((aligned(16))) float rows[GATHER_MAX_P * GATHER_MAX_PX][D];
  const int tid = threadIdx.x;
  const int xoff = a.vec ? ((a.shift_x % 4) + 4) & 3 : 0;
  const int X0 = (int)blockIdx.x * GATHER_T - ((4 - xoff) & 3), Y0 = a.y_begin + blockIdx.y * GATHER_T;
  auto ceil_div_pos = [](int v, int s) { return v <= 0 ? 0 : (v + s - 1) / s; };
  int py0 = ceil_div_pos(Y0 - (P - 1), a.stride), py1 = (Y0 + GATHER_T - 1) / a.stride;
  int px0 = ceil_div_pos(X0 - (P - 1), a.stride), px1 = (X0 + GATHER_T - 1) / a.stride;
  if (py0 < a.row_begin) py0 = a.row_begin;
  if (py1 > a.row_end - 1) py1 = a.row_end - 1;
  if (px1 > a.nPx - 1) px1 = a.nPx - 1;
  int npx = px1 - px0 + 1, npy = py1 - py0 + 1;
  if (npx > GATHER_MAX_PX) npx = GATHER_MAX_PX, px1 = px0 + npx - 1;
  if (npy > GATHER_MAX_P) npy = GATHER_MAX_P, py1 = py0 + npy - 1;
  const bool touched = npx > 0 && npy > 0;
  if (!touched && !a.do_step) {
    if (a.band) {
      const int Y = Y0 + (tid >> 3);
      for (int i = 0; i < 4; ++i) {
        const int X = X0 + (tid & 7) * 4 + i;
        if (Y < a.y_end && X >= 0 && X < a.W) a.band[(size_t)(Y - a.y_begin) * a.W + X] = 0.f;
      }
    }
    return;
  }
  const int Yt = Y0 + (tid >> 3), Xt = X0 + (tid & 7) * 4;
  const bool pre = a.do_step && a.vec && Yt < a.y_end && Xt >= 0 && Xt + 3 < a.W;
  const bool early = pre && a.preload;
  bool loaded = early;
  float4 pre_g = make_float4(0.f, 0.f, 0.f, 0.f), pre_t = pre_g, pre_f = pre_g, pre_m = pre_g, pre_v = pre_g;
  float4 pre_k = make_float4(1.f, 1.f, 1.f, 1.f);
  auto load_step_streams = [&]() {
    const AdamArgs& st = a.step;
    const size_t idx = (size_t)wrap(Yt - a.shift_y, a.H) * a.W + wrap(Xt - a.shift_x, a.W);
    pre_g = *reinterpret_cast<const float4*>(st.grad_flux + idx);
    pre_t = *reinterpret_cast<const float4*>(st.theta + idx), pre_f = *reinterpret_cast<const float4*>(st.flux_in + idx);
    if (!st.sgd) pre_m = *reinterpret_cast<const float4*>(st.m + idx), pre_v = *reinterpret_cast<const float4*>(st.v + idx);
    if (st.mask) pre_k = *reinterpret_cast<const float4*>(st.mask + idx);
  };
  if (touched) {
    const bool slots = a.winner && *a.flag != a.gen;
    constexpr int PER = (GATHER_MAX_P * GATHER_MAX_PX + 15) / 16;
    int slot_of[PER];
#pragma unroll
    for (int j = 0; j < PER; ++j) {
      const int p = (tid >> 4) + 16 * j;
      slot_of[j] = -1;
      if (p < npy * npx) {
        const int py = py0 + p / npx, px = px0 + p % npx;
        slot_of[j] = slots ? a.winner[(size_t)py * a.nPx + px] : (py - a.row_begin) * a.nPx + px;
      }
    }
    if (early) load_step_streams();
    const float* base = slots ? a.grec : a.gpatch;
    float4 rowv[PER];
#pragma unroll
    for (int j = 0; j < PER; ++j)
      rowv[j] = reinterpret_cast<const float4*>(base + (size_t)(slot_of[j] >= 0 ? slot_of[j] : 0) * D)[tid & 15];
#pragma unroll
    for (int j = 0; j < PER; ++j) {
      const int p = (tid >> 4) + 16 * j;
      if (p < npy * npx)
        *reinterpret_cast<float4*>(&rows[p][(tid & 15) * 4]) = slot_of[j] >= 0 ? rowv[j] : make_float4(0.f, 0.f, 0.f, 0.f);
    }
  } else if (early) {
    load_step_streams();
  }
  __syncthreads();
  const int Y = Y0 + (tid >> 3);
  if (Y >= a.y_end) return;
  int py_hi = Y / a.stride, py_lo = ceil_div_pos(Y - (P - 1), a.stride);
// ... 31 lines not shown
      const float4 f4 = *reinterpret_cast<const float4*>(a.raw_flux + row + wrap(Xg - a.shift_x, a.W));
      fr[0] = f4.x, fr[1] = f4.y, fr[2] = f4.z, fr[3] = f4.w;
    } else {
#pragma unroll
      for (int i = 0; i < 4; ++i)
        if (Xg + i >= 0 && Xg + i < a.W) fr[i] = a.raw_flux[row + wrap(Xg + i - a.shift_x, a.W)];
    }
#pragma unroll
    for (int i = 0; i < 4; ++i) {
      any[i] = any[i] && sum[i] != 0.f;
      if (any[i]) term[i] = gather_normed_term(a, sum[i], fr[i]);
    }
  } else {
#pragma unroll
    for (int i = 0; i < 4; ++i) term[i] = a.coef * sum[i];
  }
  if (a.band) {
#pragma unroll
    for (int i = 0; i < 4; ++i)
      if (Xg + i >= 0 && Xg + i < a.W) a.band[(size_t)(Y - a.y_begin) * a.W + Xg + i] = any[i] ? term[i] : 0.f;
    return;
  }
  if (a.vec && Xg >= 0 && Xg + 3 < a.W) {
    const size_t idx = row + wrap(Xg - a.shift_x, a.W);
    if (a.do_step) {
      const AdamArgs& st = a.step;
      if (!loaded) load_step_streams();
      const float4 g4 = pre_g, t4 = pre_t, f4 = pre_f, m4 = pre_m, v4 = pre_v, k4 = pre_k;
      float g[4] = {g4.x, g4.y, g4.z, g4.w};
      float th[4] = {t4.x, t4.y, t4.z, t4.w}, f[4] = {f4.x, f4.y, f4.z, f4.w};
      float m[4] = {m4.x, m4.y, m4.z, m4.w}, v[4] = {v4.x, v4.y, v4.z, v4.w};
      float mk[4] = {k4.x, k4.y, k4.z, k4.w};
#pragma unroll
      for (int i = 0; i < 4; ++i) {
        if (any[i]) g[i] += term[i];
        adam_pixel(th[i], f[i], m[i], v[i], g[i], mk[i], st);
      }
      *reinterpret_cast<float4*>(st.theta + idx) = make_float4(th[0], th[1], th[2], th[3]);
      *reinterpret_cast<float4*>(st.flux_out + idx) = make_float4(f[0], f[1], f[2], f[3]);
      if (!st.sgd) {
        *reinterpret_cast<float4*>(st.m + idx) = make_float4(m[0], m[1], m[2], m[3]);
        *reinterpret_cast<float4*>(st.v + idx) = make_float4(v[0], v[1], v[2], v[3]);
      }
    } else if (any[0] || any[1] || any[2] || any[3]) {
      float4 g4 = *reinterpret_cast<const float4*>(a.grad + idx);
      if (any[0]) g4.x += term[0];
      if (any[1]) g4.y += term[1];
      if (any[2]) g4.z += term[2];
      if (any[3]) g4.w += term[3];
      *reinterpret_cast<float4*>(a.grad + idx) = g4;
    }
    return;
  }
#pragma unroll
  for (int i = 0; i < 4; ++i) {
    const int X = Xg + i;
    if (X < 0 || X >= a.W) continue;
    const size_t idx = row + wrap(X - a.shift_x, a.W);
    if (a.do_step) {
      const AdamArgs& st = a.step;
      float g = st.grad_flux[idx];
      if (any[i]) g += term[i];
      float th = st.theta[idx], f = st.flux_in[idx], m = st.sgd ? 0.f : st.m[idx], v = st.sgd ? 0.f : st.v[idx];
      const float mk = st.mask ? st.mask[idx] : 1.f;
      adam_pixel(th, f, m, v, g, mk, st);
      st.theta[idx] = th, st.flux_out[idx] = f;
      if (!st.sgd) st.m[idx] = m, st.v[idx] = v;
    } else if (any[i]) {
      a.grad[idx] += term[i];
    }
  }
}

constexpr int BANDS_MAX = 64;
template <int NB>
struct AddBandsArgsT {
  float* grad;
  const float* bands;
  size_t chunk;
  int H, W, shift_y, shift_x, n_bands, y_lo, y_hi;
  const int* shift_dev;
  int y_begin[NB], y_end[NB];
};
using AddBandsArgs = AddBandsArgsT<BANDS_MAX>;

template <int NB>
static AddBandsArgsT<NB> narrow_bands(const AddBandsArgs& a) {
  AddBandsArgsT<NB> n{};
  n.grad = a.grad, n.bands = a.bands, n.chunk = a.chunk, n.H = a.H, n.W = a.W, n.shift_y = a.shift_y, n.shift_x = a.shift_x;
  n.n_bands = a.n_bands, n.y_lo = a.y_lo, n.y_hi = a.y_hi, n.shift_dev = a.shift_dev;
  for (int b = 0; b < NB; ++b) n.y_begin[b] = a.y_begin[b], n.y_end[b] = a.y_end[b];
  return n;
}

// ... 49 lines not shown
    if (Y < yb || Y >= ye) continue;
    const float* row = a.bands + (size_t)b * a.chunk + (size_t)(Y - yb) * a.W;
#pragma unroll
    for (int i = 0; i < 4; ++i) sum[i] += row[X[i]];
    any = true;
  }
  const size_t idx = (size_t)yy * a.W + xx;
  const float4 g4 = *reinterpret_cast<const float4*>(st.grad_flux + idx);
  float g[4] = {g4.x, g4.y, g4.z, g4.w};
  const float4 t4 = *reinterpret_cast<const float4*>(st.theta + idx), f4 = *reinterpret_cast<const float4*>(st.flux_in + idx);
  float th[4] = {t4.x, t4.y, t4.z, t4.w}, f[4] = {f4.x, f4.y, f4.z, f4.w}, m[4] = {0.f, 0.f, 0.f, 0.f}, v[4] = {0.f, 0.f, 0.f, 0.f};
  float mk[4] = {1.f, 1.f, 1.f, 1.f};
  if (!st.sgd) {
    const float4 m4 = *reinterpret_cast<const float4*>(st.m + idx), v4 = *reinterpret_cast<const float4*>(st.v + idx);
    m[0] = m4.x, m[1] = m4.y, m[2] = m4.z, m[3] = m4.w, v[0] = v4.x, v[1] = v4.y, v[2] = v4.z, v[3] = v4.w;
  }
  if (st.mask) {
    const float4 k4 = *reinterpret_cast<const float4*>(st.mask + idx);
    mk[0] = k4.x, mk[1] = k4.y, mk[2] = k4.z, mk[3] = k4.w;
  }
#pragma unroll
  for (int i = 0; i < 4; ++i) {
    if (any) g[i] += sum[i];
    adam_pixel(th[i], f[i], m[i], v[i], g[i], mk[i], st);
  }
  *reinterpret_cast<float4*>(st.theta + idx) = make_float4(th[0], th[1], th[2], th[3]);
  *reinterpret_cast<float4*>(st.flux_out + idx) = make_float4(f[0], f[1], f[2], f[3]);
  if (!st.sgd) {
    *reinterpret_cast<float4*>(st.m + idx) = make_float4(m[0], m[1], m[2], m[3]);
    *reinterpret_cast<float4*>(st.v + idx) = make_float4(v[0], v[1], v[2], v[3]);
  }
}

int launch_gather(const GmmGatherArgs& ga, hipStream_t s) {
  const bool has_norm = ga.norm.kind != NORM_IDENTITY;
  ProfScope prof(JD_KERNEL_GMM_GATHER, s);
  if (ga.stride >= 4 && opt_value(OPT_GMM_GATHER_TILED, 1) != 0) {
    dim3 grid((ga.W + 3 + GATHER_T - 1) / GATHER_T, (ga.y_end - ga.y_begin + GATHER_T - 1) / GATHER_T);
    if (has_norm) gmm_gather_tile_kernel<true><<<grid, 256, 0, s>>>(ga);
    else gmm_gather_tile_kernel<false><<<grid, 256, 0, s>>>(ga);
  } else {
    dim3 grid((ga.W + 255) / 256, ga.y_end - ga.y_begin);
    if (has_norm) gmm_gather_kernel<true><<<grid, 256, 0, s>>>(ga);
    else gmm_gather_kernel<false><<<grid, 256, 0, s>>>(ga);
  }
  JD_LAUNCH_CHECK();
  return JD_OK;
}

}

using namespace jd;

extern "C" int jd_add_rolled_bands(float* grad, int H, int W, int shift_y, int shift_x, const float* bands,
                                   size_t chunk_floats, int n_bands, const int* y_begin, const int* y_end, void* stream) {
  JD_REQUIRE(grad && bands && y_begin && y_end, "jd_add_rolled_bands: null argument");
  JD_REQUIRE(n_bands >= 1 && n_bands <= BANDS_MAX, "jd_add_rolled_bands: %d bands not in [1, %d]", n_bands, BANDS_MAX);
  AddBandsArgs a{};
  a.grad = grad, a.bands = bands, a.chunk = chunk_floats, a.H = H, a.W = W, a.n_bands = n_bands;
  a.shift_y = ((shift_y % H) + H) % H, a.shift_x = ((shift_x % W) + W) % W;
  a.y_lo = H, a.y_hi = 0;
  for (int b = 0; b < n_bands; ++b) {
    JD_REQUIRE(y_begin[b] >= 0 && y_begin[b] <= y_end[b] && y_end[b] <= H && (size_t)(y_end[b] - y_begin[b]) * W <= chunk_floats,
               "jd_add_rolled_bands: band %d rows [%d, %d) do not fit", b, y_begin[b], y_end[b]);
    a.y_begin[b] = y_begin[b], a.y_end[b] = y_end[b];
    if (y_begin[b] < y_end[b]) a.y_lo = std::min(a.y_lo, y_begin[b]), a.y_hi = std::max(a.y_hi, y_end[b]);
  }
  if (a.y_lo >= a.y_hi) return JD_OK;
  dim3 grid((W + 1023) / 1024, a.y_hi - a.y_lo);
  if (n_bands <= 8) add_rolled_bands_kernel<8><<<grid, 256, 0, as_stream(stream)>>>(narrow_bands<8>(a));
  else if (n_bands <= 16) add_rolled_bands_kernel<16><<<grid, 256, 0, as_stream(stream)>>>(narrow_bands<16>(a));
  else add_rolled_bands_kernel<BANDS_MAX><<<grid, 256, 0, as_stream(stream)>>>(a);
  JD_LAUNCH_CHECK();
// ... 36 lines not shown
```

jolideco_amd/csrc/jd_adam.h:

```cpp
#pragma once
#include <hip/hip_runtime.h>

namespace jd {

struct AdamArgs {
  float* theta;
  const float* flux_in;
  float* flux_out;
  float* grad_flux;
  float* m;
  float* v;
  const float* mask;
  size_t n;
  float step_size, beta1, beta2, one_minus_beta1, one_minus_beta2, bias2_sqrt, eps, lr;
  int zero_grad, sgd;
  int linear;
  const float* bias_dev;
};

__device__ __forceinline__ void use_device_bias(AdamArgs& a) {
  if (a.bias_dev) a.step_size = a.bias_dev[0], a.bias2_sqrt = a.bias_dev[1];
}

__device__ inline void adam_update(float& th, float& m, float& v, float g, const AdamArgs& a) {
#ifndef JD_ADAM_CONTRACT
#pragma clang fp contract(off)
#endif
  if (a.sgd) {
    th = th - a.lr * g;
    return;
  }
  m = m + a.one_minus_beta1 * (g - m);
  v = v * a.beta2 + a.one_minus_beta2 * (g * g);
  const float denom = sqrtf(v) / a.bias2_sqrt + a.eps;
  th = th - a.step_size * (m / denom);
}

__device__ __forceinline__ void adam_pixel(float& th, float& f, float& m, float& v, float gf, float mk, const AdamArgs& a) {
  const float dfdth = a.linear ? (a.mask ? mk : 1.f) : f;
  adam_update(th, m, v, gf * dfdth, a);
  f = a.linear ? th : expf(th);
  if (a.mask) f *= mk;
}

}
```

jolideco_amd/csrc/kernels.h:

```cpp
#pragma once
#include <vector>
#include "jd_common.h"

namespace jd {

struct PoissonArgs {
  const float* conv[JD_MAX_COMPONENTS];
  float* g[JD_MAX_COMPONENTS];
  const float* background;
  const float* counts;
  float* npred_out;
  double* partials;
  int n_comp, H, W, Hp, Wp, oy, ox;
  float eps, inv_n;
  int write_grad;
  int up;
  const float* log_bkg_norm;
  double* partials_b;
};

struct PoissonMixedArgs {
  const float* conv[JD_MAX_COMPONENTS];
  float* g[JD_MAX_COMPONENTS];
  int up[JD_MAX_COMPONENTS], Wp[JD_MAX_COMPONENTS], oy[JD_MAX_COMPONENTS], ox[JD_MAX_COMPONENTS];
// ... 23 lines not shown
                     const float* shift_xy, float scale, double* partials, int* n_blocks, hipStream_t stream);
int shift_bwd_max_blocks(int H, int W);
int shift_bwd_route(int H, int W);
struct FftBatch;
int launch_shift_bwd_batch(const float* in, const FftBatch* batch, int n_datasets, float* grad_in, int accumulate, int H, int W,
                           float scale, double* partials, size_t partials_stride, int* n_blocks, hipStream_t stream);
int launch_finalize_multi_batch(const double* partials, size_t stride, int n_blocks, int n_datasets, float* const* out,
                                hipStream_t stream);
int launch_finalize_multi(const double* partials, int n_blocks, int n_out, double scale, float* out, int accumulate,
                          hipStream_t stream);

enum { JD_CONV_FFT = 0, JD_CONV_DIRECT = 1, JD_CONV_SEPARABLE = 2 };
bool direct_conv_supported(int kh, int kw);
bool direct_conv_split_supported(int kh, int kw);
size_t direct_conv_fragment_floats(int kh, int kw, int split);
int launch_toeplitz_fragments(const float* psf, float* afrag_fwd, float* afrag_adj, int kh, int kw, int split,
                              hipStream_t stream);
int launch_direct_conv(const float* in, const float* in_scale, const float* afrag, float* out, const float* out_scale,
                       int H, int W, int kh, int kw, int oy, int ox, int adjoint, float coef, int accumulate, int split,
                       hipStream_t stream);
int direct_conv_tiles(int H, int W);
int launch_direct_conv_poisson(const float* in, const float* in_scale, const float* afrag, float* g_out, int H, int W,
                               int kh, int kw, int oy, int ox, const float* background, const float* counts,
                               float* npred_out, double* partials, float eps, float inv_n, int write_grad,
                               int* n_partials, int split, hipStream_t stream);

enum JdOption {
  OPT_SEP_NO_ALIAS, OPT_SEP_FWD_MIN_LDS, OPT_SEP_ADJ_MIN_LDS, OPT_SEP_INTERLEAVE, OPT_SEP_NO_FUSION, OPT_SEP_WALK,
  OPT_SEP_WALK_COLS, OPT_SEP_WALK_ROWS, OPT_SEP_WALK_ADJ_COLS, OPT_SEP_WALK_ADJ_ROWS, OPT_DIRECT_FP32,
  OPT_CONV_BLOCKS_PER_CU, OPT_POISSON_ROWS, OPT_GMM_NO_HOST_STATS, OPT_GMM_BLOCK_TILES, OPT_GMM_DENSE, OPT_GMM_KSPLIT,
  OPT_GMM_SCREEN_NO_LDS_CONSTS, OPT_GMM_SCREEN_DEBUG, OPT_GMM_SCREEN, OPT_GMM_FUSED_BWD,
  OPT_GMM_GATHER_TILED, OPT_GMM_LSE_SCREEN, OPT_SEP_JOINT, OPT_SEP_JOINT_ROWS, OPT_SEP_JOINT_CHUNK,
  OPT_SEP_WALK_ADJ_ALL, OPT_SEP_WALK_COST33, OPT_SEP_WALK_ROWS33, OPT_SEP_NO_TRIM, OPT_SEP_WALK_ADJ_ROWS33,
  OPT_SEP_WALK_ADJ33, OPT_FFT_NATIVE, OPT_DIRECT_AUTO_ALL, OPT_FFT_BATCH, OPT_FFT_TINY, OPT_FFT_POOL_IO, OPT_GMM_SORT_BLOCKS, OPT_GMM_GATHER_PRELOAD, OPT_COUNT
};
bool opt_is_set(int id);
int opt_value(int id, int unset_value);

constexpr int SEP_MAX_K = 68, SEP_MAX_RANK = 3, SEP_MAX_BATCH = 16;
struct SepGeom {
  int khp, kwp;
  int oy0, ox0;
  int shiftx;
  int rpairs;
  int pitch;
};
SepGeom sep_geom(int kh, int kw, int oy, int ox, bool adjoint);
struct SepOpInfo {
  int rank = 0;
  int ulo[2] = {0, 0}, uhi[2] = {0, 0}, vlo[2] = {0, 0}, vhi[2] = {0, 0};
};
inline unsigned sep_pack_support(int ulo, int uhi, int vlo, int vhi) {
  return (unsigned)ulo | (unsigned)uhi << 8 | (unsigned)vlo << 16 | (unsigned)vhi << 24;
}
void sep_register_operator(const void* op_dev, const SepOpInfo& info);
void sep_forget_operator(const void* op_dev);
int sep_operator_rank(const void* op_dev);
bool sep_operator_info(const void* op_dev, SepOpInfo* info);
constexpr double SEP_DEFAULT_TOL = 3e-7;
bool sep_conv_supported(int kh, int kw);
size_t sep_conv_operator_floats();
int sep_factorize(const float* psf_host, int kh, int kw, double tol, std::vector<double>* u, std::vector<double>* v);
int sep_build_operator(const float* psf_host, int kh, int kw, int oy, int ox, double tol, std::vector<float>* op,
                       SepOpInfo* info = nullptr);
struct SepLossFold {
  const double* partials;
  int count;
  double scale, offset;
  float* out;
};
int launch_sep_conv(const float* in, const float* in_scale, const float* op, float* out, const float* out_scale, int H,
                    int W, int kh, int kw, int oy, int ox, int adjoint, float coef, int accumulate, hipStream_t stream,
                    const SepLossFold* fold = nullptr, int* fold_done = nullptr);
int sep_guard_check(int** guard_dev);
int sep_conv_tiles(int H, int W);
constexpr int SEP_BATCH_MAX_COMP = 4;
struct SepBatchTable {
  const float* scale[SEP_MAX_BATCH * SEP_BATCH_MAX_COMP];
  const float* op[SEP_MAX_BATCH * SEP_BATCH_MAX_COMP];
  float* g[SEP_MAX_BATCH * SEP_BATCH_MAX_COMP];
  const float* bkg[SEP_MAX_BATCH];
  const float* cnt[SEP_MAX_BATCH];
  float* loss_out[SEP_MAX_BATCH];
  float loss_offset[SEP_MAX_BATCH];
  int order[SEP_MAX_BATCH];
  int n17;
  unsigned long long frame33;
};
void walk_batch_order(SepBatchTable& table, int n, int n_comp, int kh, int kw, int oy, int ox);
int launch_sep_conv_poisson_batch(int n, int n_comp, const float* const* flux, const SepBatchTable& table,
                                  const SepBatchTable* table_dev, int H, int W, int kh, int kw, int oy, int ox,
                                  double* partials, float eps, float inv_n, int write_grad, int* n_partials,
                                  hipStream_t stream);
int launch_sep_conv_adjoint_batch(int n, int n_comp, int comp, const SepBatchTable& table, const SepBatchTable* table_dev,
                                  float* grad, int H, int W, int kh, int kw, int oy, int ox, float coef, int accumulate,
                                  hipStream_t stream, const double* fin_partials = nullptr, double fin_scale = 0.0,
                                  int fin_count = 0, int* fin_done = nullptr);
bool sep_batch_is_mixed(int n, int n_comp, const SepBatchTable& table, int H, int W, int kh, int kw, int oy, int ox);

constexpr int JD_WALK_NOT_TAKEN = 1;
bool walk_takes_launch(int H, int W, int n_datasets, int kh, int kw, int oy, int ox);
int walk_operator_frame(const float* op, int kh, int kw, int oy, int ox);
int walk_info_frame(const SepOpInfo& info, int kh, int kw, int oy, int ox);
int walk_conv(const float* in, const float* in_scale, const float* op, float* out, const float* out_scale, int H, int W,
              int kh, int kw, int oy, int ox, int adjoint, float coef, int accumulate, hipStream_t stream);
int walk_conv_poisson(const float* in, const float* in_scale, const float* op, float* g_out, int H, int W, int kh, int kw,
                      int oy, int ox, const float* background, const float* counts, float* npred_out, double* partials,
                      float eps, float inv_n, int write_grad, int* n_partials, hipStream_t stream);
int walk_conv_poisson_batch(int n, const float* flux, const SepBatchTable& table, const SepBatchTable* table_dev, int H,
                            int W, int kh, int kw, int oy, int ox, double* partials, float eps, float inv_n,
                            int write_grad, int* n_partials, hipStream_t stream);
int walk_joint_step(int n, const float* flux, const SepBatchTable& table, const SepBatchTable* table_dev, float* grad, int H,
                    int W, int kh, int kw, int oy, int ox, double* partials, float eps, float inv_n, float coef,
                    int accumulate, int* n_partials, hipStream_t stream);
int walk_conv_poisson_batch_multi(int n, int n_comp, const float* const* flux, const SepBatchTable& table,
                                  const SepBatchTable* table_dev, int H, int W, int kh, int kw, int oy, int ox,
                                  double* partials, float eps, float inv_n, int write_grad, int* n_partials,
                                  hipStream_t stream);
int walk_conv_adjoint_batch(int n, int n_comp, int comp, const SepBatchTable& table, const SepBatchTable* table_dev,
                            float* grad, int H, int W, int kh, int kw, int oy, int ox, float coef, int accumulate,
                            hipStream_t stream, const double* fin_partials, double fin_scale, int fin_count, int* fin_done);
int walk_conv_adjoint_batch_all(int n, int n_comp, const SepBatchTable& table, const SepBatchTable* table_dev,
                                float* const* grads, int H, int W, int kh, int kw, int oy, int ox, float coef, int accumulate,
                                hipStream_t stream, const double* fin_partials, double fin_scale, int fin_count,
                                int* fin_done);
int launch_finalize_rows(const double* partials, int n, int n_out, double scale, const float* offset_host,
                         float* const* out, hipStream_t stream);
int launch_sep_conv_poisson(const float* in, const float* in_scale, const float* op, float* g_out, int H, int W, int kh,
                            int kw, int oy, int ox, const float* background, const float* counts, float* npred_out,
                            double* partials, float eps, float inv_n, int write_grad, int* n_partials,
                            hipStream_t stream);

struct FftNative {
  int H = 0, W = 0, kh = 0, kw = 0, oy = 0, ox = 0, Hh = 0, Nx = 0, Ny = 0;
  float2* spec = nullptr;
  float2* work = nullptr;
  float2* tw_x = nullptr;
  float2* tw_y = nullptr;
};
bool fftn_supported(int H, int W, int kh, int kw);
int fftn_create(FftNative* n, int H, int W, int kh, int kw);
void fftn_destroy(FftNative* n);
size_t fftn_spectrum_elements(const FftNative& n);
int fftn_spectrum(const FftNative& n, const float* psf, float2* khat, hipStream_t stream);
int fftn_conv(const FftNative& n, const float* in, const float* in_scale, const float2* khat, float* out, const float* out_scale,
              int adjoint, float coef, int accumulate, hipStream_t stream);
int fftn_poisson_step(const FftNative& n, const float* flux, const float* exposure, const float2* khat, const float* background,
                      const float* counts, double* partials, int* n_partials, float eps, float inv_n, float* grad, float coef,
                      int accumulate, hipStream_t stream, double loss_scale, double loss_offset, float* loss_out);

constexpr int FFT_MAX_BATCH = 16;
struct FftBatch {
  int n;
  const float* exposure[FFT_MAX_BATCH];
// ... 38 lines not shown
```

jolideco_amd/csrc/options.hip:

```cpp
#include <atomic>
#include <climits>
#include <cstdlib>
#include <cstring>

#include "jd_common.h"
#include "kernels.h"

namespace jd {

namespace {
struct OptionSlot {
  const char* name;
  std::atomic<int> value;
};
OptionSlot g_options[OPT_COUNT] = {
    {"JD_SEP_NO_ALIAS", {INT_MIN}},      {"JD_SEP_FWD_MIN_LDS", {INT_MIN}},  {"JD_SEP_ADJ_MIN_LDS", {INT_MIN}},
    {"JD_SEP_INTERLEAVE", {INT_MIN}},    {"JD_SEP_NO_FUSION", {INT_MIN}},    {"JD_SEP_WALK", {INT_MIN}},
    {"JD_SEP_WALK_COLS", {INT_MIN}},     {"JD_SEP_WALK_ROWS", {INT_MIN}},    {"JD_SEP_WALK_ADJ_COLS", {INT_MIN}},
    {"JD_SEP_WALK_ADJ_ROWS", {INT_MIN}}, {"JD_DIRECT_FP32", {INT_MIN}},      {"JD_CONV_BLOCKS_PER_CU", {INT_MIN}},
    {"JD_POISSON_ROWS", {INT_MIN}},      {"JD_GMM_NO_HOST_STATS", {INT_MIN}}, {"JD_GMM_BLOCK_TILES", {INT_MIN}},
    {"JD_GMM_DENSE", {INT_MIN}},         {"JD_GMM_KSPLIT", {INT_MIN}},
    {"JD_GMM_SCREEN_NO_LDS_CONSTS", {INT_MIN}}, {"JD_GMM_SCREEN_DEBUG", {INT_MIN}}, {"JD_GMM_SCREEN", {INT_MIN}},
    {"JD_GMM_FUSED_BWD", {INT_MIN}},     {"JD_GMM_GATHER_TILED", {INT_MIN}}, {"JD_GMM_LSE_SCREEN", {INT_MIN}},
    {"JD_SEP_JOINT", {INT_MIN}},         {"JD_SEP_JOINT_ROWS", {INT_MIN}},
    {"JD_SEP_JOINT_CHUNK", {INT_MIN}},   {"JD_SEP_WALK_ADJ_ALL", {INT_MIN}}, {"JD_SEP_WALK_COST33", {INT_MIN}},
    {"JD_SEP_WALK_ROWS33", {INT_MIN}},   {"JD_SEP_NO_TRIM", {INT_MIN}},      {"JD_SEP_WALK_ADJ_ROWS33", {INT_MIN}},
    {"JD_SEP_WALK_ADJ33", {INT_MIN}},    {"JD_FFT_NATIVE", {INT_MIN}},
    {"JD_DIRECT_AUTO_ALL", {INT_MIN}},
    {"JD_FFT_BATCH", {INT_MIN}},
    {"JD_FFT_TINY", {INT_MIN}},
    {"JD_FFT_POOL_IO", {INT_MIN}},
    {"JD_GMM_SORT_BLOCKS", {INT_MIN}},
    {"JD_GMM_GATHER_PRELOAD", {INT_MIN}},
};

int parse(const char* text) {
  char* end = nullptr;
  const long v = strtol(text, &end, 10);
  if (end == text) return 1;
  return v <= INT_MIN ? INT_MIN + 1 : v > INT_MAX ? INT_MAX : (int)v;
}

struct EnvInit {
  EnvInit() {
    for (auto& o : g_options)
      if (const char* env = getenv(o.name)) o.value.store(parse(env));
  }
} g_env_init;
}

bool opt_is_set(int id) { return g_options[id].value.load(std::memory_order_relaxed) != INT_MIN; }
int opt_value(int id, int unset_value) {
  const int v = g_options[id].value.load(std::memory_order_relaxed);
  return v == INT_MIN ? unset_value : v;
}

}

using namespace jd;

extern "C" int jd_set_option(const char* key, const char* value) {
  JD_REQUIRE(key, "jd_set_option: key is null");
  for (auto& o : g_options)
    if (strcmp(o.name, key) == 0) {
      o.value.store(value ? parse(value) : INT_MIN);
      return JD_OK;
// ... 15 lines not shown
```

jolideco_amd/csrc/sepconv.hip:

```cpp
#include <algorithm>
#include <cstring>
#include <cmath>
#include <cstdlib>
#include <mutex>
#include <unordered_map>
#include <vector>

#include "jd_common.h"
#include "kernels.h"

namespace jd {

namespace {

#ifndef JD_SEP_WAVES_POISSON
#define JD_SEP_WAVES_POISSON 6
#endif
#ifndef JD_SEP_WAVES_MULTI
#define JD_SEP_WAVES_MULTI 4
#endif
#ifndef JD_SEP_WAVES_OTHER
#define JD_SEP_WAVES_OTHER 1
#endif
constexpr int TY = 32, TX = 64, THREADS = 256, STAGE_BATCH = 3;
// ... 594 lines not shown
  if (n_comp < 1 || n_comp > SEP_BATCH_MAX_COMP)
    return fail(JD_ERR_INVALID, "separable batch: %d components not in [1, %d]", n_comp, SEP_BATCH_MAX_COMP);
  return JD_OK;
}

int launch_sep_conv_poisson_batch(int n, int n_comp, const float* const* flux, const SepBatchTable& table,
                                  const SepBatchTable* table_dev, int H, int W, int kh, int kw, int oy, int ox,
                                  double* partials, float eps, float inv_n, int write_grad, int* n_partials,
                                  hipStream_t stream) {
  int rc = check_batch(n, n_comp);
  if (rc) return rc;
  rc = n_comp == 1 ? walk_conv_poisson_batch(n, flux[0], table, table_dev, H, W, kh, kw, oy, ox, partials, eps, inv_n,
                                             write_grad, n_partials, stream)
                   : walk_conv_poisson_batch_multi(n, n_comp, flux, table, table_dev, H, W, kh, kw, oy, ox, partials, eps,
                                                   inv_n, write_grad, n_partials, stream);
  if (rc != JD_WALK_NOT_TAKEN) return rc;
  *n_partials = sep_conv_tiles(H, W);
  SepArgs a{};
  a.in = flux[0], a.in_c1 = n_comp > 1 ? flux[1] : nullptr, a.in_c2 = n_comp > 2 ? flux[2] : nullptr;
  a.in_c3 = n_comp > 3 ? flux[3] : nullptr;
  a.H = H, a.W = W, a.coef = 1.f, a.partials = partials;
  a.eps = eps, a.inv_n = inv_n, a.write_grad = write_grad, a.n_batch = n, a.n_comp = n_comp, a.table = table_dev;
  a.op = table.op[0], a.in_scale = table.scale[0];
  a.interleave = opt_is_set(OPT_SEP_INTERLEAVE) ? 1 : 0;
  bool flux_aligned = true;
  for (int c = 0; c < n_comp; ++c) flux_aligned = flux_aligned && (reinterpret_cast<uintptr_t>(flux[c]) & 15) == 0;
  return launch_sep(a, kh, kw, oy, ox, 0, true, stream, table_rank1(table, n * n_comp), table.op, n * n_comp,
                    flux_aligned && table_aligned(table, n, n_comp));
}

int launch_sep_conv_adjoint_batch(int n, int n_comp, int comp, const SepBatchTable& table, const SepBatchTable* table_dev,
                                  float* grad, int H, int W, int kh, int kw, int oy, int ox, float coef, int accumulate,
                                  hipStream_t stream, const double* fin_partials, double fin_scale, int fin_count,
                                  int* fin_done) {
  int rc = check_batch(n, n_comp);
  if (rc) return rc;
  if (comp < 0 || comp >= n_comp) return fail(JD_ERR_INVALID, "separable batch: component %d not in [0, %d)", comp, n_comp);
  if (fin_done) *fin_done = 0;
  {
    int folded = 0;
    rc = walk_conv_adjoint_batch(n, n_comp, comp, table, table_dev, grad, H, W, kh, kw, oy, ox, coef, accumulate, stream,
                                 fin_partials, fin_scale, fin_count, &folded);
    if (rc != JD_WALK_NOT_TAKEN) {
      if (fin_done) *fin_done = folded;
      return rc;
    }
  }
  SepArgs a{};
  a.out = grad, a.H = H, a.W = W, a.coef = coef, a.accumulate = accumulate, a.n_batch = n, a.table = table_dev;
  a.n_comp = n_comp, a.comp = comp;
  if (fin_partials && fin_count == sep_conv_tiles(H, W)) {
    a.fin_partials = fin_partials, a.fin_scale = fin_scale;
    if (fin_done) *fin_done = 1;
  }
  a.in = table.g[comp], a.op = table.op[comp];
  return launch_sep(a, kh, kw, oy, ox, 1, false, stream, table_rank1(table, n * n_comp), table.op, n * n_comp,
                    table_aligned(table, n, n_comp));
}

}
```

jolideco_amd/csrc/walkconv.hip:

```cpp
#include <cmath>
#include <utility>

#include "jd_common.h"
#include "kernels.h"

namespace jd {

namespace {

template <int WKT> struct Frame;
template <> struct Frame<17> { static constexpr int WK = 17, WH = 8, WS = 18; };
template <> struct Frame<33> { static constexpr int WK = 33, WH = 16, WS = 36; };
constexpr int WK = Frame<17>::WK, WH = Frame<17>::WH, WS = Frame<17>::WS;
constexpr int XG_MAX = 6;
constexpr int XW = 8;
#ifndef JD_WALK_PREFETCH
#define JD_WALK_PREFETCH 2
#endif
constexpr int WALK_PREFETCH = JD_WALK_PREFETCH;
constexpr int WALK_PREFETCH_ADJ = 3;
constexpr size_t WALK_MIN_PIXELS = (size_t)1 << 24;

template <int... I, class F>
__device__ __forceinline__ void static_for_impl(std::integer_sequence<int, I...>, F&& f) {
// ... 2 lines not shown
template <int N, class F>
__device__ __forceinline__ void static_for(F&& f) {
  static_for_impl(std::make_integer_sequence<int, N>{}, f);
}

template <int C> struct Vec;
template <> struct Vec<2> { typedef float T __attribute__((ext_vector_type(2))); };
template <> struct Vec<4> { typedef float T __attribute__((ext_vector_type(4))); };

struct WalkArgs {
  const float* in;
  const float* in_scale;
  const float* op;
  float* out;
  const float* out_scale;
  const float* background;
  const float* counts;
  float* npred_out;
  double* partials;
  int H, W, strips, tiles_y, rows;
  int taps_u, taps_v;
  int kh, kw, oy0, ox0;
  int blocks17, n17;
  int ilv17, ilv33;
  int strips33, tiles_y33, rows33;
  int part_stride;
  float coef;
  int accumulate;
  float eps, inv_n;
  int write_grad;
  int n_batch;
  const SepBatchTable* table;
  int d_base;
  int n_comp, comp;
  const double* fin_partials;
  double fin_scale;
  int fin_count, fin_n;
  int* guard;
  int comp_blocks;
  float* out_comp[4];
};

__device__ __forceinline__ void wave_lds_fence() {
  __builtin_amdgcn_fence(__ATOMIC_ACQ_REL, "wavefront");
  __builtin_amdgcn_wave_barrier();
}

typedef float v2f __attribute__((ext_vector_type(2)));
template <int SEL>
__device__ __forceinline__ v2f pk_fma_tap(v2f taps, v2f h, v2f acc) {
  if constexpr (SEL == 0)
    asm("v_pk_fma_f32 %0, %1, %2, %0 op_sel_hi:[0,1,1]" : "+v"(acc) : "v"(taps), "v"(h));
  else
    asm("v_pk_fma_f32 %0, %1, %2, %0 op_sel:[1,0,0] op_sel_hi:[1,1,1]" : "+v"(acc) : "v"(taps), "v"(h));
  return acc;
}
template <int SEL>
__device__ __forceinline__ v2f pk_mul_tap(v2f taps, v2f h) {
  v2f r;
  if constexpr (SEL == 0)
    asm("v_pk_mul_f32 %0, %1, %2 op_sel_hi:[0,1]" : "=v"(r) : "v"(taps), "v"(h));
  else
    asm("v_pk_mul_f32 %0, %1, %2 op_sel:[1,0] op_sel_hi:[1,1]" : "=v"(r) : "v"(taps), "v"(h));
  return r;
}

// ... 50 lines not shown
    __syncthreads();
    if (threadIdx.x == 0) {
      double total = 0.0;
#pragma unroll
      for (int i = 0; i < 4; ++i) total += fin_red[i];
      a.table->loss_out[blockIdx.x][0] = (float)(a.fin_scale * total + (double)a.table->loss_offset[blockIdx.x]);
    }
  }

  const int n_tiles = strips * tiles_y;
  const int per_xcd = (n_tiles + 7) / 8;
  int comp = a.comp;
  if (XCHG && a.comp_blocks) comp = bid / a.comp_blocks, bid -= comp * a.comp_blocks;
  const int q = bid / 8;
  const int ilv = !XCHG && a.n_batch > 0 ? (slot0 ? a.ilv33 : a.ilv17) : 0;
  const int dsel = (!XCHG && a.n_batch > 0) ? a.table->order[slot0 + (ilv ? q % ilv : q / per_xcd)] : 0;
  const int tile = (bid % 8) * per_xcd + (ilv ? q / ilv : q % per_xcd);
  if (tile >= n_tiles) return;
  const int sx = tile / tiles_y, ty = tile - sx * tiles_y;

  typedef const float __attribute__((address_space(1)))* gcp;
  typedef float __attribute__((address_space(1)))* gp;
  typedef const vC __attribute__((address_space(1)))* gcv;
  typedef vC __attribute__((address_space(1)))* gv;
  const bool batch = a.n_batch > 0;
  const int d = XCHG ? a.d_base + wv : dsel;
  const int slot = XCHG ? d * a.n_comp + comp : d;
  const gcp in = (gcp)(batch && !POISSON ? a.table->g[slot] : a.in);
  const gcp in_scale = (gcp)(batch ? a.table->scale[slot] : a.in_scale);
  const gcp op = (gcp)(batch ? a.table->op[slot] : a.op);
  const gcp out_scale = (gcp)(batch ? a.table->scale[slot] : a.out_scale);
  const gcp background = (gcp)(batch ? a.table->bkg[d] : a.background);
  const gcp counts = (gcp)(batch ? a.table->cnt[d] : a.counts);
  const gp out = (gp)(POISSON && batch ? a.table->g[d] : XCHG && a.comp_blocks ? a.out_comp[comp] : a.out);
  const gp npred_out = (gp)a.npred_out;

  float tu[WK], tv[WK];
  {
    if (((int)op[0] != 1 || (int)op[1] > WK) && lane == 0) *a.guard = 1;
    float mu = 0.f, mv = 0.f;
    const int iu = lane - (WH + a.oy0), iv = lane - (WH + a.ox0);
    if (iu >= 0 && iu < a.kh) mu = op[a.taps_u + iu];
    if (iv >= 0 && iv < a.kw) mv = op[a.taps_v + iv];
#pragma unroll
    for (int t = 0; t < WK; ++t) {
      tu[t] = __int_as_float(__builtin_amdgcn_readlane(__float_as_int(mu), t));
      tv[t] = __int_as_float(__builtin_amdgcn_readlane(__float_as_int(mv), t));
    }
  }

  constexpr bool PK = C == 4 || WKT == 33;
  v2f tup[PK ? (WK + 1) / 2 : 1];
  if constexpr (PK) {
#pragma unroll
    for (int j = 0; j < (WK + 1) / 2; ++j) {
      float lo = tu[2 * j], hi = 2 * j + 1 < WK ? tu[2 * j + 1] : 0.f;
      asm volatile("" : "+v"(lo), "+v"(hi));
      tup[j] = v2f{lo, hi};
    }
  }

  const int X0 = sx * 64 * C;
  const int xm = X0 - WH + C * lane;
  const int xe = X0 - WH + 64 * C + C * lane;
  const int xo = X0 + C * lane;
  const bool vm = xm >= 0 && xm < a.W, ve = lane < NX && xe < a.W, vo = xo < a.W;
  const int xd = X0 - WH + 64 * C + C * (lane % NX);
// ... 210 lines not shown
        const int gy = (i + WS - 2 * WH) % XG;
        const int mine = wv < XG ? wv : XG - 1;
        if (gy == 0) {
          const int yy = min(max(y + mine, Y0), y_end - 1);
          oprev = *(gcv)(out + (size_t)yy * a.W + oo);
        }
        if (gy == XG - 1 && y - gy >= Y0 && y - gy < y_end) {
          __syncthreads();
          const int k = (y - Y0) / XG, yy = y - gy + mine;
          vC res = oprev;
          for (int dd = 0; dd < nb; ++dd) {
            const vC pd = *reinterpret_cast<const vC*>(xbuf + (size_t)((((k & 1) * XG + mine) * XWT + dd) * 64 + lane) * C);
            res = dd == 0 && !a.accumulate ? pd : res + pd;
          }
          if (vo && wv < XG && yy < y_end) *(gv)(out + (size_t)yy * a.W + oo) = res;
        }
      }
      load_epi(y + P, ce);
    });
  }
  if (POISSON) {
    loss = wave_sum(loss);
    const int stride = a.part_stride ? a.part_stride : n_tiles;
    if (lane == 0) {
      double* row = a.partials + (size_t)d * stride;
      row[tile] = loss;
      for (int t = tile + n_tiles; t < stride; t += n_tiles) row[t] = 0.0;
    }
  }
}

template <int WKT, int C, int P, bool POISSON, bool IN_SCALE, int XG, int XWT = XW>
__global__ __launch_bounds__(XG ? 64 * XWT : 64) void walk_kernel(WalkArgs a) {
  walk_body<WKT, C, P, POISSON, IN_SCALE, XG, XWT>(a, (int)blockIdx.x, a.strips, a.tiles_y, a.rows, 0);
}

template <int C17, int P>
__global__ __launch_bounds__(64) void walk_mixed_kernel(WalkArgs a) {
  if ((int)blockIdx.x < a.blocks17)
    walk_body<17, C17, P, true, true, 0, XW>(a, (int)blockIdx.x, a.strips, a.tiles_y, a.rows, 0);
  else
    walk_body<33, 2, P, true, true, 0, XW>(a, (int)blockIdx.x - a.blocks17, a.strips33, a.tiles_y33, a.rows33, a.n17);
}

constexpr int MG = 6;
constexpr int MULTI_MAX = 4;

struct MultiArgs {
  const float* flux[MULTI_MAX];
  double* partials;
  int H, W, strips, tiles_y, rows;
  int taps_u, taps_v, kh, kw, oy0, ox0;
  float eps, inv_n;
  int write_grad, n_comp;
  const SepBatchTable* table;
  int* guard;
};

template <int WKT, int C, int P>
__device__ __forceinline__ void walk_multi_body(const MultiArgs& a, float* multi_lds) {
#pragma clang fp contract(off)
  constexpr int WK = Frame<WKT>::WK, WH = Frame<WKT>::WH, WS = Frame<WKT>::WS;
  typedef typename Vec<C>::T vC;
  static_assert(WS % MG == 0 && WS % P == 0, "group size and prefetch depth must divide the rotation period");
  constexpr int NX = 2 * WH / C;
  constexpr int NWIN = 2 * WH + C;
  const int lane = threadIdx.x & 63, wv = (int)(threadIdx.x >> 6), nc = a.n_comp;
// ... 603 lines not shown
  return walk_enabled(H, W, n_datasets) && plan_frame(kh, kw, oy, ox) != 0;
}

int walk_operator_frame(const float* op, int kh, int kw, int oy, int ox) { return walk_frame(op, kh, kw, oy, ox); }

int walk_info_frame(const SepOpInfo& info, int kh, int kw, int oy, int ox) { return frame_of_info(info, kh, kw, oy, ox); }

void walk_batch_order(SepBatchTable& table, int n, int n_comp, int kh, int kw, int oy, int ox) {
  int k = 0;
  table.n17 = 0;
  for (int pass = 0; pass < 2; ++pass)
    for (int d = 0; d < n; ++d) {
      const bool is17 = n_comp != 1 || walk_frame(table.op[d], kh, kw, oy, ox) != 33;
      if (is17 == (pass == 0)) table.order[k++] = d;
      if (is17 && pass == 0) ++table.n17;
    }
  for (; k < SEP_MAX_BATCH; ++k) table.order[k] = 0;
  table.frame33 = 0;
  for (int i = 0; i < n * n_comp && i < 64; ++i)
    if (walk_frame(table.op[i], kh, kw, oy, ox) == 33) table.frame33 |= 1ull << i;
}

bool sep_batch_is_mixed(int n, int n_comp, const SepBatchTable& table, int H, int W, int kh, int kw, int oy, int ox) {
  if (n_comp > MULTI_MAX || !walk_enabled(H, W, n * n_comp)) return false;
  int yes = 0;
  for (int d = 0; d < n; ++d)
    for (int c = 0; c < n_comp; ++c) {
      const int f = dataset_frame(table, d * n_comp + c, d, kh, kw, oy, ox);
      yes += f != 0 ? 1 : 0;
    }
  return yes != 0 && yes != n * n_comp;
}

int walk_conv(const float* in, const float* in_scale, const float* op, float* out, const float* out_scale, int H, int W,
              int kh, int kw, int oy, int ox, int adjoint, float coef, int accumulate, hipStream_t stream) {
  if (!walk_enabled(H, W, 1)) return JD_WALK_NOT_TAKEN;
  const int frame = walk_frame(op, kh, kw, oy, ox);
  if (!frame) return JD_WALK_NOT_TAKEN;
  if (!aligned16(in) || !aligned16(in_scale) || !aligned16(out) || !aligned16(out_scale)) return JD_WALK_NOT_TAKEN;
  WalkArgs a{};
  a.in = in, a.in_scale = in_scale, a.op = op, a.out = out, a.out_scale = out_scale;
  a.H = H, a.W = W, a.coef = coef, a.accumulate = accumulate;
  walk_setup(a, kh, kw, oy, ox, adjoint);
  int C, rows;
  walk_shape(a, 1, adjoint != 0, frame, &C, &rows);
  walk_tiles(a, C, rows);
  return in_scale ? launch_walk<false, true>(a, frame, C, 1, stream) : launch_walk<false, false>(a, frame, C, 1, stream);
}

int walk_conv_poisson(const float* in, const float* in_scale, const float* op, float* g_out, int H, int W, int kh, int kw,
                      int oy, int ox, const float* background, const float* counts, float* npred_out, double* partials,
                      float eps, float inv_n, int write_grad, int* n_partials, hipStream_t stream) {
  if (!walk_enabled(H, W, 1) || !in_scale) return JD_WALK_NOT_TAKEN;
  const int frame = walk_frame(op, kh, kw, oy, ox);
  if (!frame) return JD_WALK_NOT_TAKEN;
  if (!aligned16(in) || !aligned16(in_scale) || !aligned16(g_out) || !aligned16(background) || !aligned16(counts) ||
      !aligned16(npred_out))
    return JD_WALK_NOT_TAKEN;
  WalkArgs a{};
  a.in = in, a.in_scale = in_scale, a.op = op, a.out = g_out;
  a.H = H, a.W = W, a.coef = 1.f;
  a.background = background, a.counts = counts, a.npred_out = npred_out, a.partials = partials;
  a.eps = eps, a.inv_n = inv_n, a.write_grad = write_grad;
  walk_setup(a, kh, kw, oy, ox, 0);
  int C, rows;
  walk_shape(a, 1, false, frame, &C, &rows);
// ... 108 lines not shown
    if (eff > best) best = eff, rows = r;
  }
  if (rows > (H + MG - 1) / MG * MG) rows = (H + MG - 1) / MG * MG;
  const int orows = opt_value(OPT_SEP_WALK_ROWS, 0);
  if (orows >= 18) rows = orows;
  rows = (rows + MG - 1) / MG * MG;
  a.rows = rows, a.strips = (W + 64 * C - 1) / (64 * C), a.tiles_y = (H + rows - 1) / rows;
  int rc = sep_guard_check(&a.guard);
  if (rc) return rc;
  const int n_tiles = a.strips * a.tiles_y;
  *n_partials = n_tiles;
  const unsigned blocks = (unsigned)(((n_tiles + 7) / 8) * 8 * n);
  const size_t lds = (size_t)n_comp * 64 * C * (2 + 3 * MG) * sizeof(float);
  ProfScope prof(JD_KERNEL_POISSON_FUSED, stream);
  if (C == 4) {
    static size_t lds_set = 0;
    if (lds > 64 * 1024 && lds > lds_set) {
      JD_HIP(hipFuncSetAttribute(reinterpret_cast<const void*>(walk_multi_kernel<4, WALK_PREFETCH, 17>),
                                 hipFuncAttributeMaxDynamicSharedMemorySize, (int)lds));
      lds_set = lds;
    }
    hipLaunchKernelGGL((walk_multi_kernel<4, WALK_PREFETCH, 17>), dim3(blocks), dim3(64 * n_comp), lds, stream, a);
  } else if (any33) {
    hipLaunchKernelGGL((walk_multi_kernel<2, WALK_PREFETCH, 33>), dim3(blocks), dim3(64 * n_comp), lds, stream, a);
  } else {
    hipLaunchKernelGGL((walk_multi_kernel<2, WALK_PREFETCH, 17>), dim3(blocks), dim3(64 * n_comp), lds, stream, a);
  }
  JD_LAUNCH_CHECK();
  return JD_OK;
}

int walk_conv_adjoint_batch(int n, int n_comp, int comp, const SepBatchTable& table, const SepBatchTable* table_dev,
                            float* grad, int H, int W, int kh, int kw, int oy, int ox, float coef, int accumulate,
                            hipStream_t stream, const double* fin_partials, double fin_scale, int fin_count, int* fin_done) {
  *fin_done = 0;
  if (!walk_enabled(H, W, n * n_comp) || !aligned16(grad)) return JD_WALK_NOT_TAKEN;
  int frames[SEP_MAX_BATCH];
  for (int d = 0; d < n; ++d)
    for (int c = 0; c < n_comp; ++c) {
      const int f = dataset_frame(table, d * n_comp + c, d, kh, kw, oy, ox);
      if (!f) return JD_WALK_NOT_TAKEN;
      if (c == comp) frames[d] = f;
    }
  WalkArgs a{};
  a.out = grad, a.H = H, a.W = W, a.coef = coef, a.table = table_dev, a.n_comp = n_comp, a.comp = comp;
  walk_setup(a, kh, kw, oy, ox, 1);
  int rc = sep_guard_check(&a.guard);
  if (rc) return rc;
  for (int d0 = 0; d0 < n;) {
    const int frame = frames[d0];
    int m = 1;
    while (d0 + m < n && m < XW && frames[d0 + m] == frame) ++m;
    if (frame == 33 && opt_value(OPT_SEP_WALK_ADJ33, 0) == 1) m = 1;
    const int xg = m >= 6 ? 6 : m >= 3 ? 3 : 2;
    const bool wide = frame == 17 && m >= 6 && opt_value(OPT_SEP_WALK_ADJ_COLS, 4) != 2;
    const int C = wide ? 4 : 2;
    const int lds = (2 * xg * XW * 64 * C + XW * 128 * C) * 4;
    int per_cu = 160 * 1024 / lds;
    const int by_regs = (wide || frame == 33 ? 8 : 16) / m;
    if (per_cu > by_regs) per_cu = by_regs;
    if (per_cu < 1) per_cu = 1;
    const long slots = (long)device_cus() * per_cu * (per_cu > 1 ? 15 : 16) / 16;
    const int strips = (W + 64 * C - 1) / (64 * C);
    int rows = 36;
    while (rows < 4096 && (long)strips * ((H + rows - 1) / rows) > slots) rows += 6;
    const int orows = opt_value(frame == 33 ? OPT_SEP_WALK_ADJ_ROWS33 : OPT_SEP_WALK_ADJ_ROWS, 0);
    if (orows >= 18) rows = orows;
    rows = (rows + 5) / 6 * 6;
    walk_tiles(a, C, rows);
    const int n_tiles = a.strips * a.tiles_y;
    const unsigned blocks = (unsigned)(((n_tiles + 7) / 8) * 8);
    a.d_base = d0, a.n_batch = m, a.accumulate = d0 == 0 ? accumulate : 1;
    a.fin_partials = nullptr;
    if (d0 == 0 && fin_partials && m >= 4 && (int)blocks >= n) {
      a.fin_partials = fin_partials, a.fin_scale = fin_scale, a.fin_count = fin_count, a.fin_n = n;
      *fin_done = 1;
    }
    ProfScope prof(JD_KERNEL_SEP_CONV, stream);
    if (frame == 33 && m >= 6)
      hipLaunchKernelGGL((walk_kernel<33, 2, WALK_PREFETCH, false, false, 6>), dim3(blocks), dim3(64 * m), 0, stream, a);
    else if (frame == 33 && m >= 3)
      hipLaunchKernelGGL((walk_kernel<33, 2, WALK_PREFETCH, false, false, 3>), dim3(blocks), dim3(64 * m), 0, stream, a);
    else if (frame == 33 && m == 2)
      hipLaunchKernelGGL((walk_kernel<33, 2, WALK_PREFETCH, false, false, 2>), dim3(blocks), dim3(64 * m), 0, stream, a);
    else if (m >= 6 && wide)
// ... 153 lines not shown
```

jolideco_amd/loss.py:

```python
import os

import numpy as np
import torch

from .models import NPredModels
from .models.npred import common_kernel_shape
from .ops import PoissonNLLFunction, stirling_mean
from .utils.table import TraceTable
from .utils.torch import TORCH_DEFAULT_DEVICE

__all__ = ["PoissonLoss", "PriorLoss", "TotalLoss"]


class _PoissonNLLLoss:

    def __init__(self):
        self._stirling = {}

    def stirling(self, counts):
        key = (counts.data_ptr(), counts.numel())
        if key not in self._stirling:
            self._stirling[key] = stirling_mean(counts.detach().cpu().numpy())
        return self._stirling[key]

# ... 60 lines not shown

    def batchable_calibrated(self, indices):
        models_all = [self.npred_models_all[i] for i in indices]
        if len(models_all) < 2 or any(len(models) != 1 for models in models_all):
            return False
        first = next(iter(models_all[0].values()))
        u = first.upsampling_factor or 1
        if u not in (2, 3, 4) or first.plan.method != "fft" or not first.plan.native_fft:
            return False
        return all(
            (m.upsampling_factor or 1) == u and m.plan is first.plan for models in models_all for m in models.values()
        )

    def fwd_bwd_batch_calibrated(self, indices, flux, loss_outs, grad=None, accumulate=False, grad_scale=1.0):
        per_dataset = [self.npred_models_all[i] for i in indices]
        models = [next(iter(mm.values())) for mm in per_dataset]
        models[0].plan.npred_poisson_calibrated_batch_fwd_bwd(
            flux=flux, exposures=[m.exposure for m in models], khats=[m.khat for m in models],
            backgrounds=[mm.background for mm in per_dataset], counts=[self.counts_all[i] for i in indices],
            stirlings=[self.stirling_all[i] for i in indices], loss_outs=loss_outs,
            calibrations=[mm.calibration_pointers(grad is not None) for mm in per_dataset],
            upsampling=models[0].upsampling_factor or 1, grad=grad, accumulate=accumulate, grad_scale=grad_scale,
        )

    def mergeable(self, indices):
        key = tuple(indices)
        cache = self.__dict__.setdefault("_mergeable", {})
        if key not in cache:
            cache[key] = os.environ.get("JOLIDECO_MERGE_COMPONENTS", "1") != "0" and all(
                getattr(self.npred_models_all[i], "shared_operator", False) for i in indices
            )
        return cache[key]

    def fwd_bwd_batch(self, indices, flux, loss_outs, grad=None, accumulate=False, grad_scale=1.0, flux_nonneg=False):
        per_dataset = [list(self.npred_models_all[i].values()) for i in indices]
        single = torch.is_tensor(flux)
        if not single and len(flux) > 1 and flux_nonneg and not accumulate and self.mergeable(indices):
            from .ops import copy_image_to, sum_images

            total = self.__dict__.get("_merged_flux")
            if total is None or total.shape != flux[0].shape or total.device != flux[0].device:
                total = self._merged_flux = torch.empty_like(flux[0])
            sum_images(total, list(flux))
            per_dataset[0][0].plan.npred_poisson_batch_fwd_bwd(
                flux=total, exposures=[models[0].exposure for models in per_dataset],
                khats=[models[0].khat for models in per_dataset],
                backgrounds=[self.npred_models_all[i].background for i in indices],
                counts=[self.counts_all[i] for i in indices], stirlings=[self.stirling_all[i] for i in indices],
                loss_outs=loss_outs, grad=None if grad is None else grad[0], accumulate=False, grad_scale=grad_scale,
            )
            if grad is not None:
                copy_image_to(grad[0], list(grad[1:]))
            return
        exposures = [[m.exposure for m in models] for models in per_dataset]
        khats = [[m.khat for m in models] for models in per_dataset]
        if single:
            exposures, khats = [e[0] for e in exposures], [k[0] for k in khats]
        per_dataset[0][0].plan.npred_poisson_batch_fwd_bwd(
            flux=flux, exposures=exposures, khats=khats,
            backgrounds=[self.npred_models_all[i].background for i in indices],
            counts=[self.counts_all[i] for i in indices], stirlings=[self.stirling_all[i] for i in indices],
            loss_outs=loss_outs, grad=grad, accumulate=accumulate, grad_scale=grad_scale,
        )

    @classmethod
    def from_datasets(cls, datasets, components, calibrations=None, device=TORCH_DEFAULT_DEVICE):
        npred_models_all, counts_all = [], []
        kernel_shape = common_kernel_shape(datasets, components, calibrations)
        for name, dataset in datasets.items():
            calibration = calibrations[name] if calibrations else None
            models = NPredModels.from_dataset_numpy(
                dataset=dataset, components=components, calibration=calibration, device=device, kernel_shape=kernel_shape
            )
            npred_models_all.append(models)
            counts = torch.from_numpy(np.ascontiguousarray(dataset["counts"], dtype=np.float32)[None, None])
            counts_all.append(counts.to(device))
        return cls(counts_all=counts_all, npred_models_all=npred_models_all, names_all=list(datasets))


class PriorLoss:

    def __init__(self, priors):
        self.priors = priors

    def evaluate(self, fluxes):
        return [prior(flux=flux) for flux, prior in zip(fluxes, self.priors.values())]

    def __call__(self, fluxes):
        return sum(self.evaluate(fluxes=fluxes))


class TotalLoss:

    def __init__(self, poisson_loss, prior_loss, poisson_loss_validation=None, beta=1):
        self.poisson_loss = poisson_loss
# ... 85 lines not shown
```

jolideco_amd/ops.py:

```python
import ctypes
import math
import weakref
from ctypes import c_float, c_int, c_void_p

import numpy as np
import torch

from . import _hip
from ._hip import check, ptr, ptr_array, stream_ptr

__all__ = [
    "ConvPlan",
    "GmmHandle",
    "ConvSameFunction",
    "PoissonNLLFunction",
    "GMMPatchPriorFunction",
    "ElementwisePriorFunction",
    "SmoothnessPriorFunction",
    "stirling_mean",
    "require_hip_tensor",
    "band_rows",
    "add_rolled_bands",
]

# ... 186 lines not shown
                self._handle, n, ptr_array(fluxes), ptr_array(exposures), ptr_array(khats), ptr(background),
                ptr(counts), c_float(stirling), c_float(eps), ptr(loss_out),
                ptr_array(grads) if grads is not None else None, int(accumulate), c_float(grad_scale),
                ptr(npred_out), int(upsampling), stream_ptr(background.device),
            )
        )

    @staticmethod
    def npred_poisson_mixed_fwd_bwd(
        plans, upsamplings, fluxes, exposures, khats, background, counts, stirling, loss_out, grads=None,
        accumulate=False, grad_scale=1.0, npred_out=None, eps=POISSON_EPS,
    ):
        n = len(plans)
        if not (len(upsamplings) == len(fluxes) == len(exposures) == len(khats) == n):
            raise ValueError("plans, upsamplings, fluxes, exposures and khats must have the same length")
        if grads is not None and len(grads) != n:
            raise ValueError("one gradient image per flux component")
        for plan, f in zip(plans, fluxes):
            plan._check_image(f, "flux")
        handles = (c_void_p * n)(*[plan._handle.value for plan in plans])
        factors = (c_int * n)(*[int(u) for u in upsamplings])
        check(
            _hip.lib().jd_npred_poisson_mixed_fwd_bwd(
                handles, n, ptr_array(fluxes), ptr_array(exposures), ptr_array(khats), ptr(background), ptr(counts),
                c_float(stirling), c_float(eps), ptr(loss_out), ptr_array(grads) if grads is not None else None,
                int(accumulate), c_float(grad_scale), ptr(npred_out), factors, stream_ptr(background.device),
            )
        )

    MAX_BATCH = 16
    MAX_BATCH_COMPONENTS = 4

    def npred_poisson_batch_fwd_bwd(self, flux, exposures, khats, backgrounds, counts, stirlings, loss_outs, grad=None,
                                    accumulate=False, grad_scale=1.0, eps=POISSON_EPS):
        n = len(exposures)
        if not (len(khats) == len(backgrounds) == len(counts) == len(stirlings) == len(loss_outs) == n):
            raise ValueError("all per-dataset lists must have the same length")
        single = torch.is_tensor(flux)
        fluxes = [flux] if single else list(flux)
        grads = None if grad is None else ([grad] if single else list(grad))
        if single:
            exposures, khats = [[e] for e in exposures], [[k] for k in khats]
        n_comp = len(fluxes)
        if not 1 <= n_comp <= self.MAX_BATCH_COMPONENTS:
            raise ValueError(f"{n_comp} flux components: the batched joint step takes 1 to {self.MAX_BATCH_COMPONENTS}")
        if any(len(e) != n_comp for e in exposures) or any(len(k) != n_comp for k in khats):
            raise ValueError("every dataset needs one exposure and one operator per flux component")
        if grads is not None and len(grads) != n_comp:
            raise ValueError("one gradient image per flux component")
        for f in fluxes:
            self._check_image(f, "flux")
        for start in range(0, n, self.MAX_BATCH):
            sl = slice(start, min(n, start + self.MAX_BATCH))
            m = sl.stop - sl.start
            stirling_arr = (c_float * m)(*[float(v) for v in stirlings[sl]])
            check(
                _hip.lib().jd_npred_poisson_batch_multi_fwd_bwd(
                    self._handle, m, n_comp, ptr_array(fluxes), ptr_array([e for es in exposures[sl] for e in es]),
                    ptr_array([k for ks in khats[sl] for k in ks]), ptr_array(backgrounds[sl]), ptr_array(counts[sl]),
                    stirling_arr, c_float(eps), ptr_array(loss_outs[sl]), None if grads is None else ptr_array(grads),
                    int(accumulate or start > 0), c_float(grad_scale), stream_ptr(fluxes[0].device),
                )
            )

    def npred_poisson_calibrated_batch_fwd_bwd(self, flux, exposures, khats, backgrounds, counts, stirlings, loss_outs,
                                               calibrations, upsampling=1, grad=None, accumulate=False, grad_scale=1.0,
                                               eps=POISSON_EPS):
        n = len(exposures)
        if not (len(khats) == len(backgrounds) == len(counts) == len(stirlings) == len(loss_outs) == len(calibrations) == n):
            raise ValueError("all per-dataset lists must have the same length")
        self._check_image(flux, "flux")
        cals = [c if c is not None else (None, None, None, None) for c in calibrations]
        for start in range(0, n, self.MAX_BATCH):
            sl = slice(start, min(n, start + self.MAX_BATCH))
            m = sl.stop - sl.start
            stirling_arr = (c_float * m)(*[float(v) for v in stirlings[sl]])
            check(
                _hip.lib().jd_npred_poisson_calibrated_batch_fwd_bwd(
                    self._handle, m, ptr(flux), ptr_array(exposures[sl]), ptr_array(khats[sl]), ptr_array(backgrounds[sl]),
                    ptr_array(counts[sl]), stirling_arr, c_float(eps), ptr_array(loss_outs[sl]), ptr(grad),
                    int(accumulate or start > 0), c_float(grad_scale), int(upsampling),
                    ptr_array([c[0] for c in cals[sl]]), ptr_array([c[1] for c in cals[sl]]),
                    ptr_array([c[2] for c in cals[sl]]), ptr_array([c[3] for c in cals[sl]]), stream_ptr(flux.device),
                )
            )


class DeviceShifts:

    __slots__ = ("dev", "host")

    def __init__(self, dev, host):
        self.dev, self.host = dev, host


class GmmHandle:
# ... 359 lines not shown
```

Measured before the change: 1736 iters/s.

## Run late-frame adjoint convolutions on a side stream and fold them into Adam

The datasets whose PSF frame differs from the first (the two 33x33 observations) are split off from the batched adjoint walk. Their gradient goes into separate addend images, computed on a second stream joined back by events, and the Adam step kernel sums these addends into the gradient as it reads it. The aim is to run the smaller late-frame adjoint work alongside the main adjoint and prior work, and to drop an accumulate pass into the shared gradient. In exchange it adds extra buffers, more memory reads in the Adam kernel, and stream/event synchronisation complexity.

```diff
diff --git a/include/jolideco_hip.h b/include/jolideco_hip.h
--- a/include/jolideco_hip.h
+++ b/include/jolideco_hip.h
@@ -70,6 +70,14 @@
                                    float* const* loss_out, float* grad_flux, int accumulate, float grad_scale,
                                    void* stream);
 
+#define JD_ADDEND_MAX 4
+int jd_npred_poisson_batch_addends_fwd_bwd(jd_conv_plan* plan, int n_datasets, const float* flux,
+                                           const float* const* exposure, const float* const* khat,
+                                           const float* const* background, const float* const* counts,
+                                           const float* stirling_mean, float eps, float* const* loss_out, float* grad_flux,
+                                           int accumulate, float grad_scale, float* const* addends, void* stream2,
+                                           int* n_addends, void* stream);
+
 int jd_npred_poisson_batch_multi_fwd_bwd(jd_conv_plan* plan, int n_datasets, int n_components, const float* const* flux,
                                          const float* const* exposure, const float* const* khat,
                                          const float* const* background, const float* const* counts,
@@ -127,6 +135,7 @@
   float lr;
   int use_log_flux, sgd;
   const float* bias_dev;
+  const float* addend[JD_ADDEND_MAX];
 } jd_step;
 int jd_gmm_prior_fwd_bwd_step(jd_gmm* gmm, const float* flux, int H, int W, int stride, int shift_y, int shift_x,
                               int marginalize, float value_scale, float* value_out, int accumulate_value,
@@ -166,6 +175,10 @@
                  float* exp_avg_sq, const float* mask, size_t n, float step_size, float beta1,
                  float beta2, float one_minus_beta1, float one_minus_beta2, float bias2_sqrt, float eps,
                  int zero_grad, int use_log_flux, const float* bias_dev, void* stream);
+int jd_adam_step_addends(float* theta, const float* flux_in, float* flux_out, float* grad_flux, float* exp_avg,
+                         float* exp_avg_sq, const float* mask, size_t n, float step_size, float beta1,
+                         float beta2, float one_minus_beta1, float one_minus_beta2, float bias2_sqrt, float eps,
+                         int zero_grad, int use_log_flux, const float* bias_dev, const float* const* addends, void* stream);
 int jd_adam_step_multi(int n_tensors, float* const* theta, const float* const* grad, float* const* exp_avg,
                        float* const* exp_avg_sq, const int* sizes, const float* step_size, const float* bias2_sqrt,
                        float beta1, float beta2, float one_minus_beta1, float one_minus_beta2, float eps,
diff --git a/jolideco_amd/_hip.py b/jolideco_amd/_hip.py
--- a/jolideco_amd/_hip.py
+++ b/jolideco_amd/_hip.py
@@ -62,6 +62,11 @@
         c_int,
         [c_void_p, c_int, c_void_p, fpp, fpp, fpp, fpp, fp, c_float, fpp, c_void_p, c_int, c_float, c_void_p],
     ),
+    "jd_npred_poisson_batch_addends_fwd_bwd": (
+        c_int,
+        [c_void_p, c_int, c_void_p, fpp, fpp, fpp, fpp, fp, c_float, fpp, c_void_p, c_int, c_float, fpp, c_void_p,
+         POINTER(c_int), c_void_p],
+    ),
     "jd_npred_poisson_batch_multi_fwd_bwd": (
         c_int,
         [c_void_p, c_int, c_int, fpp, fpp, fpp, fpp, fpp, fp, c_float, fpp, fpp, c_int, c_float, c_void_p],
@@ -113,6 +118,11 @@
         c_int,
         [c_void_p, c_void_p, c_void_p, c_void_p, c_void_p, c_void_p, c_void_p, c_size_t, c_float, c_float, c_float,
          c_float, c_float, c_float, c_float, c_int, c_int, c_void_p, c_void_p],
+    ),
+    "jd_adam_step_addends": (
+        c_int,
+        [c_void_p, c_void_p, c_void_p, c_void_p, c_void_p, c_void_p, c_void_p, c_size_t, c_float, c_float, c_float,
+         c_float, c_float, c_float, c_float, c_int, c_int, c_void_p, fpp, c_void_p],
     ),
     "jd_adam_step_multi": (
         c_int,
@@ -132,6 +142,9 @@
     "jd_clock_probe": (c_int, [c_double, POINTER(c_double), c_void_p]),
 }
 
+ADDEND_MAX = 4
+
+
 class Step(ctypes.Structure):
 
     _fields_ = [
@@ -139,7 +152,7 @@
         ("exp_avg_sq", c_void_p), ("mask", c_void_p),
         ("step_size", c_float), ("beta1", c_float), ("beta2", c_float), ("one_minus_beta1", c_float),
         ("one_minus_beta2", c_float), ("bias2_sqrt", c_float), ("eps", c_float), ("lr", c_float),
-        ("use_log_flux", c_int), ("sgd", c_int), ("bias_dev", c_void_p),
+        ("use_log_flux", c_int), ("sgd", c_int), ("bias_dev", c_void_p), ("addend", c_void_p * ADDEND_MAX),
     ]
 
 
diff --git a/jolideco_amd/core.py b/jolideco_amd/core.py
--- a/jolideco_amd/core.py
+++ b/jolideco_amd/core.py
@@ -171,6 +171,8 @@
         args = _hip.Step()
         args.theta, args.flux_in, args.flux_out = st.theta.data_ptr(), st.flux_cur.data_ptr(), st.flux[1 - st.cur].data_ptr()
         args.grad_flux = st.grad.data_ptr()
+        for k, image in enumerate(getattr(st, "addends", ())):
+            args.addend[k] = image.data_ptr()
         args.mask = None if st.mask is None else st.mask.data_ptr()
         args.use_log_flux = int(st.use_log_flux)
         if self.optimizer_type == "adam":
@@ -562,6 +564,9 @@
         side_priority = int(os.environ.get("JOLIDECO_PRIOR_STREAM_PRIORITY", "0"))
         self._side_stream = (torch.cuda.Stream(device=device, priority=side_priority)
                              if torch.device(device).type == "cuda" else None)
+        self._addend_stream = None
+        self._addend_images = None
+        self.addends_used = 0
         self.step_scalars = None
         self._graphs = {}
         self._epochs_done = 0
@@ -796,6 +801,38 @@
         return {"shifts": shifts, "flux_bias": [None] * n_flux, "cal_bias": [None] * len(cal_groups), "cal_items": cal_items,
                 "n_steps": n_flux, "signature": ()}
 
+    def _likelihood_addends(self, early):
+        if not (self.batch_joint and self.n_c == 1 and not self.dist.sharded and self.dist.world_size == 1):
+            return None
+        st, prior = self.states[0], self.priors[0]
+        if st.frozen or getattr(st, "is_sparse", False) or "_optimizer_step" in vars(self.cfg):
+            return None
+        if 0 not in early or not self._fuse_step(st, prior):
+            return None
+        if st.grad.shape[-1] % 4 or len(self.local_idx) > 16:
+            return None
+        if self._addend_images is None:
+            models = self.total_loss.poisson_loss.npred_models_all
+            frames = [models[li][st.name].plan.walk_frame(models[li][st.name].khat) for _, li in self.local_idx]
+            late = sum(1 for f in frames if f != frames[0])
+            self._addend_images = []
+            if 0 < late <= _hip.ADDEND_MAX and all(f != frames[0] for f in frames[-late:]):
+                self._addend_images = [torch.empty_like(st.grad) for _ in range(late)]
+                self._addend_stream = torch.cuda.Stream(device=st.grad.device)
+        return self._addend_images or None
+
+    def _joint_likelihood(self, fluxes, grads, early=()):
+        n_c = self.n_c
+        addends = self._likelihood_addends(early)
+        beside = None if addends is None else self._addend_stream
+        used = self.total_loss.poisson_loss.fwd_bwd_batch(
+            [li for _, li in self.local_idx], fluxes if n_c > 1 else fluxes[0],
+            [self._slot(gslot) for gslot, _ in self.local_idx], grad=grads if n_c > 1 else grads[0], accumulate=False,
+            flux_nonneg=self.flux_nonneg, addends=addends, side_stream=beside,
+        )
+        self.addends_used = used or 0
+        self.states[0].addends = tuple(addends[: self.addends_used]) if self.addends_used else ()
+
     def _overlap_active(self):
         return self.overlap_prior and self._side_stream is not None and not self.dist.sharded and not _hip.profile_active()
 
@@ -808,9 +845,9 @@
             kwargs = {"shifts": shifts[ci]} if ci in shifts else {}
             flux, value = st.flux_cur, slot(n_d + ci)
             if self._fuse_step(st, prior):
-                args = cfg._step_args(st, step_no, bias)
-
-                def call(phases=3, prior=prior, flux=flux, value=value, args=args, kwargs=kwargs):
+
+                def call(phases=3, prior=prior, flux=flux, value=value, st=st, kwargs=kwargs):
+                    args = cfg._step_args(st, step_no, bias)
                     prior.device_fwd_bwd_step(flux, value, coef, args, **(dict(kwargs, phases=phases) if phases != 3 else kwargs))
 
                 calls.append((ci, call, True))
@@ -931,11 +968,7 @@
             early = self._start_priors(calls)
             first = True
             if self.batch_joint:
-                total_loss.poisson_loss.fwd_bwd_batch(
-                    [li for _, li in self.local_idx], fluxes if n_c > 1 else fluxes[0],
-                    [slot(gslot) for gslot, _ in self.local_idx], grad=grads if n_c > 1 else grads[0], accumulate=False,
-                    flux_nonneg=self.flux_nonneg,
-                )
+                self._joint_likelihood(fluxes, grads, early)
                 first = False
             elif self.batch_joint_calibrated:
                 for _, li in self.local_idx:
@@ -1093,11 +1126,7 @@
                 self.scalars.zero_()
             first = True
             if self.batch_joint:
-                total_loss.poisson_loss.fwd_bwd_batch(
-                    [li for _, li in self.local_idx], fluxes if n_c > 1 else fluxes[0],
-                    [slot(gslot) for gslot, _ in self.local_idx], grad=grads if n_c > 1 else grads[0], accumulate=False,
-                    flux_nonneg=self.flux_nonneg,
-                )
+                self._joint_likelihood(fluxes, grads)
                 first = False
             elif self.batch_joint_calibrated:
                 for _, li in self.local_idx:
diff --git a/jolideco_amd/csrc/elementwise.hip b/jolideco_amd/csrc/elementwise.hip
--- a/jolideco_amd/csrc/elementwise.hip
+++ b/jolideco_amd/csrc/elementwise.hip
@@ -587,7 +587,7 @@
   if (threadIdx.x == 0) partials[blockIdx.x] = total;
 }
 
-template <int VEC>
+template <int VEC, int NA>
 __global__ __launch_bounds__(BLOCK) void adam_kernel(AdamArgs a) {
   use_device_bias(a);
   const size_t stride = (size_t)gridDim.x * BLOCK * VEC;
@@ -597,6 +597,9 @@
       const float4 t4 = *reinterpret_cast<const float4*>(a.theta + i);
       const float4 f4 = *reinterpret_cast<const float4*>(a.flux_in + i);
       const float4 g4 = *reinterpret_cast<const float4*>(a.grad_flux + i);
+      float4 a4[NA ? NA : 1];
+#pragma unroll
+      for (int k = 0; k < NA; ++k) a4[k] = *reinterpret_cast<const float4*>(a.addend[k] + i);
       th[0] = t4.x, th[1] = t4.y, th[2] = t4.z, th[3] = t4.w;
       f[0] = f4.x, f[1] = f4.y, f[2] = f4.z, f[3] = f4.w;
       gf[0] = g4.x, gf[1] = g4.y, gf[2] = g4.z, gf[3] = g4.w;
@@ -611,8 +614,12 @@
         const float4 k4 = *reinterpret_cast<const float4*>(a.mask + i);
         mk[0] = k4.x, mk[1] = k4.y, mk[2] = k4.z, mk[3] = k4.w;
       }
+#pragma unroll
+      for (int k = 0; k < NA; ++k) gf[0] += a4[k].x, gf[1] += a4[k].y, gf[2] += a4[k].z, gf[3] += a4[k].w;
     } else {
       th[0] = a.theta[i], f[0] = a.flux_in[i], gf[0] = a.grad_flux[i];
+#pragma unroll
+      for (int k = 0; k < NA; ++k) gf[0] += a.addend[k][i];
       if (!a.sgd) m[0] = a.m[i], v[0] = a.v[i];
       mk[0] = a.mask ? a.mask[i] : 1.f;
     }
@@ -634,17 +641,31 @@
   }
 }
 
+template <int NA>
+static void launch_adam_kernel(bool vec, unsigned blocks, const AdamArgs& a, hipStream_t stream) {
+  if (vec)
+    adam_kernel<4, NA><<<blocks, BLOCK, 0, stream>>>(a);
+  else
+    adam_kernel<1, NA><<<blocks, BLOCK, 0, stream>>>(a);
+}
+
 static int launch_adam(const AdamArgs& a, hipStream_t stream) {
-  const bool vec = (a.n % 4 == 0);
+  int na = 0;
+  while (na < ADDEND_MAX && a.addend[na]) ++na;
+  bool vec = (a.n % 4 == 0);
+  for (int k = 0; k < na; ++k) vec = vec && (reinterpret_cast<uintptr_t>(a.addend[k]) & 15) == 0;
   const size_t per_block = (size_t)BLOCK * (vec ? 4 : 1);
   size_t blocks = (a.n + per_block - 1) / per_block;
   if (blocks > 4096) blocks = 4096;
   if (blocks == 0) blocks = 1;
   ProfScope prof(JD_KERNEL_ADAM, stream);
-  if (vec)
-    adam_kernel<4><<<(unsigned)blocks, BLOCK, 0, stream>>>(a);
-  else
-    adam_kernel<1><<<(unsigned)blocks, BLOCK, 0, stream>>>(a);
+  switch (na) {
+    case 0: launch_adam_kernel<0>(vec, (unsigned)blocks, a, stream); break;
+    case 1: launch_adam_kernel<1>(vec, (unsigned)blocks, a, stream); break;
+    case 2: launch_adam_kernel<2>(vec, (unsigned)blocks, a, stream); break;
+    case 3: launch_adam_kernel<3>(vec, (unsigned)blocks, a, stream); break;
+    default: launch_adam_kernel<4>(vec, (unsigned)blocks, a, stream); break;
+  }
   JD_LAUNCH_CHECK();
   return JD_OK;
 }
@@ -1034,17 +1055,29 @@
   return JD_OK;
 }
 
+extern "C" int jd_adam_step_addends(float* theta, const float* flux_in, float* flux_out, float* grad_flux,
+                                    float* exp_avg, float* exp_avg_sq, const float* mask, size_t n, float step_size,
+                                    float beta1, float beta2, float one_minus_beta1, float one_minus_beta2,
+                                    float bias2_sqrt, float eps, int zero_grad, int use_log_flux, const float* bias_dev,
+                                    const float* const* addends, void* stream) {
+  JD_REQUIRE(theta && flux_in && flux_out && grad_flux && exp_avg && exp_avg_sq && n > 0,
+             "jd_adam_step: null argument or n == 0");
+  AdamArgs a{theta, flux_in, flux_out, grad_flux, exp_avg, exp_avg_sq, mask, n,
+             step_size, beta1, beta2, one_minus_beta1, one_minus_beta2, bias2_sqrt, eps, 0.f, zero_grad, 0,
+             use_log_flux ? 0 : 1, bias_dev};
+  static_assert(ADDEND_MAX == JD_ADDEND_MAX, "the host array of jd_adam_step_addends and AdamArgs::addend");
+  for (int k = 0; addends && k < ADDEND_MAX && addends[k]; ++k) a.addend[k] = addends[k];
+  return launch_adam(a, as_stream(stream));
+}
+
 extern "C" int jd_adam_step(float* theta, const float* flux_in, float* flux_out, float* grad_flux,
                             float* exp_avg, float* exp_avg_sq, const float* mask, size_t n, float step_size,
                             float beta1, float beta2, float one_minus_beta1, float one_minus_beta2,
                             float bias2_sqrt, float eps, int zero_grad, int use_log_flux, const float* bias_dev,
                             void* stream) {
-  JD_REQUIRE(theta && flux_in && flux_out && grad_flux && exp_avg && exp_avg_sq && n > 0,
-             "jd_adam_step: null argument or n == 0");
-  AdamArgs a{theta, flux_in, flux_out, grad_flux, exp_avg, exp_avg_sq, mask, n,
-             step_size, beta1, beta2, one_minus_beta1, one_minus_beta2, bias2_sqrt, eps, 0.f, zero_grad, 0,
-             use_log_flux ? 0 : 1, bias_dev};
-  return launch_adam(a, as_stream(stream));
+  return jd_adam_step_addends(theta, flux_in, flux_out, grad_flux, exp_avg, exp_avg_sq, mask, n, step_size, beta1, beta2,
+                              one_minus_beta1, one_minus_beta2, bias2_sqrt, eps, zero_grad, use_log_flux, bias_dev, nullptr,
+                              stream);
 }
 
 constexpr int ADAM_MULTI_MAX = 64;
diff --git a/jolideco_amd/csrc/fftconv.hip b/jolideco_amd/csrc/fftconv.hip
--- a/jolideco_amd/csrc/fftconv.hip
+++ b/jolideco_amd/csrc/fftconv.hip
@@ -54,6 +54,7 @@
   jd::SepBatchTable* table_dev[N_TABLES] = {};
   unsigned long long table_used[N_TABLES] = {};
   unsigned long long table_clock = 0;
+  hipEvent_t addend_events[2] = {nullptr, nullptr};
 };
 
 namespace jd {
@@ -308,6 +309,8 @@
   if (p->partials_batch) (void)hipFree(p->partials_batch);
   for (auto* t : p->table_dev)
     if (t) (void)hipFree(t);
+  for (hipEvent_t e : p->addend_events)
+    if (e) (void)hipEventDestroy(e);
   for (float* g : p->gbatch)
     if (g) (void)hipFree(g);
   for (int c = 0; c < JD_MAX_COMPONENTS; ++c) {
@@ -634,13 +637,13 @@
   return JD_OK;
 }
 
-extern "C" int jd_npred_poisson_batch_multi_fwd_bwd(jd_conv_plan* p, int n_datasets, int n_comp, const float* const* flux,
-                                                    const float* const* exposure, const float* const* khat,
-                                                    const float* const* background, const float* const* counts,
-                                                    const float* stirling_mean, float eps, float* const* loss_out,
-                                                    float* const* grad_flux, int accumulate, float grad_scale,
-                                                    void* stream) {
-  const char* who = "jd_npred_poisson_batch_multi_fwd_bwd";
+static int npred_poisson_batch_impl(const char* who, jd_conv_plan* p, int n_datasets, int n_comp, const float* const* flux,
+                                    const float* const* exposure, const float* const* khat,
+                                    const float* const* background, const float* const* counts,
+                                    const float* stirling_mean, float eps, float* const* loss_out,
+                                    float* const* grad_flux, int accumulate, float grad_scale, void* stream,
+                                    float* const* addends, void* stream2, int* n_addends) {
+  if (n_addends) *n_addends = 0;
   JD_REQUIRE(p && flux && exposure && khat && background && counts && stirling_mean && loss_out, "%s: null argument", who);
   JD_REQUIRE(p->method == JD_CONV_SEPARABLE || (p->native && n_comp == 1),
              "%s: the plan must use the separable method, or the native FFT path with one flux component (one "
@@ -727,6 +730,22 @@
   for (int i = 0; i < n_datasets * n_comp; ++i) table.scale[i] = exposure[i], table.op[i] = khat[i], table.g[i] = p->gbatch[i];
   for (int d = 0; d < n_datasets; ++d) table.loss_out[d] = loss_out[d], table.loss_offset[d] = stirling_mean[d];
   walk_batch_order(table, n_datasets, n_comp, p->kh, p->kw, p->oy, p->ox);
+  static_assert(SEP_ADDEND_MAX == JD_ADDEND_MAX, "the caller's addend images and the split's limit");
+  int addend_first = n_datasets;
+  if (addends && n_addends && n_comp == 1 && grad_flux && !accumulate && (reinterpret_cast<uintptr_t>(grad_flux[0]) & 15) == 0) {
+    addend_first = sep_addend_split(n_datasets, table, p->H, p->W, p->kh, p->kw, p->oy, p->ox);
+    for (int d = addend_first; d < n_datasets; ++d) {
+      float* image = addends[d - addend_first];
+      if (!image || (reinterpret_cast<uintptr_t>(image) & 15) != 0) {
+        addend_first = n_datasets;
+        break;
+      }
+    }
+    for (int d = addend_first; d < n_datasets; ++d) table.addend[d] = addends[d - addend_first];
+    if (addend_first < n_datasets && stream2 && stream2 != stream)
+      for (hipEvent_t& e : p->addend_events)
+        if (!e) JD_HIP(hipEventCreateWithFlags(&e, hipEventDisableTiming));
+  }
   int slot = -1, victim = 0;
   for (int i = 0; i < jd_conv_plan::N_TABLES; ++i) {
     if (p->table_used[i] && memcmp(&table, &p->table_host[i], sizeof(table)) == 0) slot = i;
@@ -743,7 +762,7 @@
   SepBatchTable* const table_dev = p->table_dev[slot];
   const double n_pix = (double)p->H * (double)p->W;
   int n_part = 0;
-  if (n_comp == 1 && grad_flux) {
+  if (n_comp == 1 && grad_flux && addend_first == n_datasets) {
     int rc = walk_joint_step(n_datasets, flux[0], table, table_dev, grad_flux[0], p->H, p->W, p->kh, p->kw, p->oy, p->ox,
                              p->partials_batch, eps, (float)(1.0 / n_pix), grad_scale, accumulate, &n_part, s);
     if (rc != JD_WALK_NOT_TAKEN)
@@ -754,8 +773,10 @@
   if (rc) return rc;
   if (!grad_flux) return launch_finalize_rows(p->partials_batch, n_part, n_datasets, 1.0 / n_pix, stirling_mean, loss_out, s);
   int folded = 0;
-  rc = walk_conv_adjoint_batch_all(n_datasets, n_comp, table, table_dev, grad_flux, p->H, p->W, p->kh, p->kw, p->oy, p->ox,
-                                   grad_scale, accumulate, s, p->partials_batch, 1.0 / n_pix, n_part, &folded);
+  rc = addend_first < n_datasets
+           ? JD_WALK_NOT_TAKEN
+           : walk_conv_adjoint_batch_all(n_datasets, n_comp, table, table_dev, grad_flux, p->H, p->W, p->kh, p->kw, p->oy,
+                                         p->ox, grad_scale, accumulate, s, p->partials_batch, 1.0 / n_pix, n_part, &folded);
   if (rc != JD_WALK_NOT_TAKEN) {
     if (rc || folded) return rc;
     return launch_finalize_rows(p->partials_batch, n_part, n_datasets, 1.0 / n_pix, stirling_mean, loss_out, s);
@@ -765,12 +786,39 @@
     if ((rc = launch_sep_conv_adjoint_batch(n_datasets, n_comp, c, table, table_dev, grad_flux[c], p->H, p->W, p->kh,
                                             p->kw, p->oy, p->ox, grad_scale, accumulate, s,
                                             c == 0 && n_datasets <= 8 ? p->partials_batch : nullptr, 1.0 / n_pix, n_part,
-                                            &done)))
+                                            &done, addend_first < n_datasets ? addend_first : -1, as_stream(stream2),
+                                            p->addend_events)))
       return rc;
     folded |= done;
   }
+  if (n_addends) *n_addends = n_datasets - addend_first;
   if (!folded) return launch_finalize_rows(p->partials_batch, n_part, n_datasets, 1.0 / n_pix, stirling_mean, loss_out, s);
   return JD_OK;
+}
+
+extern "C" int jd_npred_poisson_batch_multi_fwd_bwd(jd_conv_plan* p, int n_datasets, int n_comp, const float* const* flux,
+                                                    const float* const* exposure, const float* const* khat,
+                                                    const float* const* background, const float* const* counts,
+                                                    const float* stirling_mean, float eps, float* const* loss_out,
+                                                    float* const* grad_flux, int accumulate, float grad_scale,
+                                                    void* stream) {
+  return npred_poisson_batch_impl("jd_npred_poisson_batch_multi_fwd_bwd", p, n_datasets, n_comp, flux, exposure, khat, background,
+                                  counts, stirling_mean, eps, loss_out, grad_flux, accumulate, grad_scale, stream, nullptr,
+                                  nullptr, nullptr);
+}
+
+extern "C" int jd_npred_poisson_batch_addends_fwd_bwd(jd_conv_plan* p, int n_datasets, const float* flux,
+                                                      const float* const* exposure, const float* const* khat,
+                                                      const float* const* background, const float* const* counts,
+                                                      const float* stirling_mean, float eps, float* const* loss_out,
+                                                      float* grad_flux, int accumulate, float grad_scale,
+                                                      float* const* addends, void* stream2, int* n_addends, void* stream) {
+  const char* who = "jd_npred_poisson_batch_addends_fwd_bwd";
+  JD_REQUIRE(flux && grad_flux && n_addends, "%s: null argument", who);
+  const float* fluxes[1] = {flux};
+  float* grads[1] = {grad_flux};
+  return npred_poisson_batch_impl(who, p, n_datasets, 1, fluxes, exposure, khat, background, counts, stirling_mean, eps, loss_out,
+                                  grads, accumulate, grad_scale, stream, addends, stream2, n_addends);
 }
 
 extern "C" int jd_npred_poisson_batch_fwd_bwd(jd_conv_plan* p, int n_datasets, const float* flux,
diff --git a/jolideco_amd/csrc/gmm.hip b/jolideco_amd/csrc/gmm.hip
--- a/jolideco_amd/csrc/gmm.hip
+++ b/jolideco_amd/csrc/gmm.hip
@@ -348,6 +348,7 @@
     ga.preload = opt_value(OPT_GMM_GATHER_PRELOAD, 1) != 0;
     ga.vec = ga.vec && aligned(step->theta) && aligned(step->flux_in) && aligned(step->flux_out) && aligned(step->m) &&
              aligned(step->v) && aligned(step->mask);
+    for (int k = 0; k < ADDEND_MAX; ++k) ga.vec = ga.vec && aligned(step->addend[k]);
   }
   return launch_gather(ga, s);
 }
@@ -395,6 +396,11 @@
   a.step_size = step->step_size, a.beta1 = step->beta1, a.beta2 = step->beta2, a.one_minus_beta1 = step->one_minus_beta1;
   a.one_minus_beta2 = step->one_minus_beta2, a.bias2_sqrt = step->bias2_sqrt, a.eps = step->eps, a.lr = step->lr;
   a.zero_grad = 0, a.sgd = step->sgd ? 1 : 0, a.linear = step->use_log_flux ? 0 : 1, a.bias_dev = step->bias_dev;
+  static_assert(ADDEND_MAX == JD_ADDEND_MAX, "jd_step::addend and AdamArgs::addend");
+  for (int k = 0, live = 1; k < ADDEND_MAX; ++k) {
+    live = live && step->addend[k] != nullptr;
+    a.addend[k] = live ? step->addend[k] : nullptr;
+  }
   return gmm_prior_impl(g, flux, H, W, stride, shift_y, shift_x, 0, -1, marginalize, value_scale, value_out, accumulate_value,
                         grad_coef, nullptr, nullptr, nullptr, stream, &a, shift_dev, phases);
 }
diff --git a/jolideco_amd/csrc/gmm_gather.hip b/jolideco_amd/csrc/gmm_gather.hip
--- a/jolideco_amd/csrc/gmm_gather.hip
+++ b/jolideco_amd/csrc/gmm_gather.hip
@@ -90,7 +90,7 @@
 
 constexpr int GATHER_T = 32, GATHER_MAX_P = 9, GATHER_MAX_PX = GATHER_MAX_P + 1;
 
-template <bool NORM>
+template <bool NORM, int NA>
 __global__ __launch_bounds__(256) void gmm_gather_tile_kernel(GmmGatherArgs a) {
 #pragma clang fp contract(off)
   use_device_shift(a);
@@ -125,6 +125,9 @@
   bool loaded = early;
   float4 pre_g = make_float4(0.f, 0.f, 0.f, 0.f), pre_t = pre_g, pre_f = pre_g, pre_m = pre_g, pre_v = pre_g;
   float4 pre_k = make_float4(1.f, 1.f, 1.f, 1.f);
+  float4 pre_a[NA ? NA : 1];
+#pragma unroll
+  for (int k = 0; k < (NA ? NA : 1); ++k) pre_a[k] = pre_g;
   auto load_step_streams = [&]() {
     const AdamArgs& st = a.step;
     const size_t idx = (size_t)wrap(Yt - a.shift_y, a.H) * a.W + wrap(Xt - a.shift_x, a.W);
@@ -132,6 +135,8 @@
     pre_t = *reinterpret_cast<const float4*>(st.theta + idx), pre_f = *reinterpret_cast<const float4*>(st.flux_in + idx);
     if (!st.sgd) pre_m = *reinterpret_cast<const float4*>(st.m + idx), pre_v = *reinterpret_cast<const float4*>(st.v + idx);
     if (st.mask) pre_k = *reinterpret_cast<const float4*>(st.mask + idx);
+#pragma unroll
+    for (int k = 0; k < NA; ++k) pre_a[k] = *reinterpret_cast<const float4*>(st.addend[k] + idx);
   };
   if (touched) {
     const bool slots = a.winner && *a.flag != a.gen;
@@ -229,6 +234,8 @@
       float m[4] = {m4.x, m4.y, m4.z, m4.w}, v[4] = {v4.x, v4.y, v4.z, v4.w};
       float mk[4] = {k4.x, k4.y, k4.z, k4.w};
 #pragma unroll
+      for (int k = 0; k < NA; ++k) g[0] += pre_a[k].x, g[1] += pre_a[k].y, g[2] += pre_a[k].z, g[3] += pre_a[k].w;
+#pragma unroll
       for (int i = 0; i < 4; ++i) {
         if (any[i]) g[i] += term[i];
         adam_pixel(th[i], f[i], m[i], v[i], g[i], mk[i], st);
@@ -257,6 +264,8 @@
     if (a.do_step) {
       const AdamArgs& st = a.step;
       float g = st.grad_flux[idx];
+#pragma unroll
+      for (int k = 0; k < NA; ++k) g += st.addend[k][idx];
       if (any[i]) g += term[i];
       float th = st.theta[idx], f = st.flux_in[idx], m = st.sgd ? 0.f : st.m[idx], v = st.sgd ? 0.f : st.v[idx];
       const float mk = st.mask ? st.mask[idx] : 1.f;
@@ -372,13 +381,27 @@
   }
 }
 
+template <int NA>
+static void tile_launch(bool has_norm, dim3 grid, const GmmGatherArgs& ga, hipStream_t s) {
+  static_assert(NA <= ADDEND_MAX, "AdamArgs::addend");
+  if (has_norm) gmm_gather_tile_kernel<true, NA><<<grid, 256, 0, s>>>(ga);
+  else gmm_gather_tile_kernel<false, NA><<<grid, 256, 0, s>>>(ga);
+}
+
 int launch_gather(const GmmGatherArgs& ga, hipStream_t s) {
   const bool has_norm = ga.norm.kind != NORM_IDENTITY;
   ProfScope prof(JD_KERNEL_GMM_GATHER, s);
   if (ga.stride >= 4 && opt_value(OPT_GMM_GATHER_TILED, 1) != 0) {
     dim3 grid((ga.W + 3 + GATHER_T - 1) / GATHER_T, (ga.y_end - ga.y_begin + GATHER_T - 1) / GATHER_T);
-    if (has_norm) gmm_gather_tile_kernel<true><<<grid, 256, 0, s>>>(ga);
-    else gmm_gather_tile_kernel<false><<<grid, 256, 0, s>>>(ga);
+    int na = 0;
+    while (ga.do_step && na < ADDEND_MAX && ga.step.addend[na]) ++na;
+    switch (na) {
+      case 0: tile_launch<0>(has_norm, grid, ga, s); break;
+      case 1: tile_launch<1>(has_norm, grid, ga, s); break;
+      case 2: tile_launch<2>(has_norm, grid, ga, s); break;
+      case 3: tile_launch<3>(has_norm, grid, ga, s); break;
+      default: tile_launch<4>(has_norm, grid, ga, s); break;
+    }
   } else {
     dim3 grid((ga.W + 255) / 256, ga.y_end - ga.y_begin);
     if (has_norm) gmm_gather_kernel<true><<<grid, 256, 0, s>>>(ga);
diff --git a/jolideco_amd/csrc/jd_adam.h b/jolideco_amd/csrc/jd_adam.h
--- a/jolideco_amd/csrc/jd_adam.h
+++ b/jolideco_amd/csrc/jd_adam.h
@@ -2,6 +2,8 @@
 #include <hip/hip_runtime.h>
 
 namespace jd {
+
+constexpr int ADDEND_MAX = 4;
 
 struct AdamArgs {
   float* theta;
@@ -16,6 +18,7 @@
   int zero_grad, sgd;
   int linear;
   const float* bias_dev;
+  const float* addend[ADDEND_MAX];
 };
 
 __device__ __forceinline__ void use_device_bias(AdamArgs& a) {
diff --git a/jolideco_amd/csrc/kernels.h b/jolideco_amd/csrc/kernels.h
--- a/jolideco_amd/csrc/kernels.h
+++ b/jolideco_amd/csrc/kernels.h
@@ -79,7 +79,8 @@
   OPT_GMM_SCREEN_NO_LDS_CONSTS, OPT_GMM_SCREEN_DEBUG, OPT_GMM_SCREEN, OPT_GMM_FUSED_BWD,
   OPT_GMM_GATHER_TILED, OPT_GMM_LSE_SCREEN, OPT_SEP_JOINT, OPT_SEP_JOINT_ROWS, OPT_SEP_JOINT_CHUNK,
   OPT_SEP_WALK_ADJ_ALL, OPT_SEP_WALK_COST33, OPT_SEP_WALK_ROWS33, OPT_SEP_NO_TRIM, OPT_SEP_WALK_ADJ_ROWS33,
-  OPT_SEP_WALK_ADJ33, OPT_FFT_NATIVE, OPT_DIRECT_AUTO_ALL, OPT_FFT_BATCH, OPT_FFT_TINY, OPT_FFT_POOL_IO, OPT_GMM_SORT_BLOCKS, OPT_GMM_GATHER_PRELOAD, OPT_COUNT
+  OPT_SEP_WALK_ADJ33, OPT_FFT_NATIVE, OPT_DIRECT_AUTO_ALL, OPT_FFT_BATCH, OPT_FFT_TINY, OPT_FFT_POOL_IO, OPT_GMM_SORT_BLOCKS, OPT_GMM_GATHER_PRELOAD,
+  OPT_SEP_ADJ_ADDENDS, OPT_COUNT
 };
 bool opt_is_set(int id);
 int opt_value(int id, int unset_value);
@@ -133,7 +134,10 @@
   int order[SEP_MAX_BATCH];
   int n17;
   unsigned long long frame33;
-};
+  float* addend[SEP_MAX_BATCH];
+};
+constexpr int SEP_ADDEND_MAX = 4;
+int sep_addend_split(int n, const SepBatchTable& table, int H, int W, int kh, int kw, int oy, int ox);
 void walk_batch_order(SepBatchTable& table, int n, int n_comp, int kh, int kw, int oy, int ox);
 int launch_sep_conv_poisson_batch(int n, int n_comp, const float* const* flux, const SepBatchTable& table,
                                   const SepBatchTable* table_dev, int H, int W, int kh, int kw, int oy, int ox,
@@ -142,7 +146,8 @@
 int launch_sep_conv_adjoint_batch(int n, int n_comp, int comp, const SepBatchTable& table, const SepBatchTable* table_dev,
                                   float* grad, int H, int W, int kh, int kw, int oy, int ox, float coef, int accumulate,
                                   hipStream_t stream, const double* fin_partials = nullptr, double fin_scale = 0.0,
-                                  int fin_count = 0, int* fin_done = nullptr);
+                                  int fin_count = 0, int* fin_done = nullptr, int addend_first = -1,
+                                  hipStream_t stream2 = nullptr, const hipEvent_t* fork_join = nullptr);
 bool sep_batch_is_mixed(int n, int n_comp, const SepBatchTable& table, int H, int W, int kh, int kw, int oy, int ox);
 
 constexpr int JD_WALK_NOT_TAKEN = 1;
@@ -166,7 +171,8 @@
                                   hipStream_t stream);
 int walk_conv_adjoint_batch(int n, int n_comp, int comp, const SepBatchTable& table, const SepBatchTable* table_dev,
                             float* grad, int H, int W, int kh, int kw, int oy, int ox, float coef, int accumulate,
-                            hipStream_t stream, const double* fin_partials, double fin_scale, int fin_count, int* fin_done);
+                            hipStream_t stream, const double* fin_partials, double fin_scale, int fin_count, int* fin_done,
+                            int addend_first = -1, hipStream_t stream2 = nullptr, const hipEvent_t* fork_join = nullptr);
 int walk_conv_adjoint_batch_all(int n, int n_comp, const SepBatchTable& table, const SepBatchTable* table_dev,
                                 float* const* grads, int H, int W, int kh, int kw, int oy, int ox, float coef, int accumulate,
                                 hipStream_t stream, const double* fin_partials, double fin_scale, int fin_count,
diff --git a/jolideco_amd/csrc/options.hip b/jolideco_amd/csrc/options.hip
--- a/jolideco_amd/csrc/options.hip
+++ b/jolideco_amd/csrc/options.hip
@@ -32,6 +32,7 @@
     {"JD_FFT_POOL_IO", {INT_MIN}},
     {"JD_GMM_SORT_BLOCKS", {INT_MIN}},
     {"JD_GMM_GATHER_PRELOAD", {INT_MIN}},
+    {"JD_SEP_ADJ_ADDENDS", {INT_MIN}},
 };
 
 int parse(const char* text) {
diff --git a/jolideco_amd/csrc/sepconv.hip b/jolideco_amd/csrc/sepconv.hip
--- a/jolideco_amd/csrc/sepconv.hip
+++ b/jolideco_amd/csrc/sepconv.hip
@@ -650,7 +650,7 @@
 int launch_sep_conv_adjoint_batch(int n, int n_comp, int comp, const SepBatchTable& table, const SepBatchTable* table_dev,
                                   float* grad, int H, int W, int kh, int kw, int oy, int ox, float coef, int accumulate,
                                   hipStream_t stream, const double* fin_partials, double fin_scale, int fin_count,
-                                  int* fin_done) {
+                                  int* fin_done, int addend_first, hipStream_t stream2, const hipEvent_t* fork_join) {
   int rc = check_batch(n, n_comp);
   if (rc) return rc;
   if (comp < 0 || comp >= n_comp) return fail(JD_ERR_INVALID, "separable batch: component %d not in [0, %d)", comp, n_comp);
@@ -658,12 +658,13 @@
   {
     int folded = 0;
     rc = walk_conv_adjoint_batch(n, n_comp, comp, table, table_dev, grad, H, W, kh, kw, oy, ox, coef, accumulate, stream,
-                                 fin_partials, fin_scale, fin_count, &folded);
+                                 fin_partials, fin_scale, fin_count, &folded, addend_first, stream2, fork_join);
     if (rc != JD_WALK_NOT_TAKEN) {
       if (fin_done) *fin_done = folded;
       return rc;
     }
   }
+  if (addend_first > 0 && addend_first < n) return fail(JD_ERR_INVALID, "separable batch: the addend split needs the strip-walk kernels");
   SepArgs a{};
   a.out = grad, a.H = H, a.W = W, a.coef = coef, a.accumulate = accumulate, a.n_batch = n, a.table = table_dev;
   a.n_comp = n_comp, a.comp = comp;
diff --git a/jolideco_amd/csrc/walkconv.hip b/jolideco_amd/csrc/walkconv.hip
--- a/jolideco_amd/csrc/walkconv.hip
+++ b/jolideco_amd/csrc/walkconv.hip
@@ -58,6 +58,7 @@
   int n_batch;
   const SepBatchTable* table;
   int d_base;
+  int order0;
   int n_comp, comp;
   const double* fin_partials;
   double fin_scale;
@@ -174,7 +175,9 @@
   const gcp out_scale = (gcp)(batch ? a.table->scale[slot] : a.out_scale);
   const gcp background = (gcp)(batch ? a.table->bkg[d] : a.background);
   const gcp counts = (gcp)(batch ? a.table->cnt[d] : a.counts);
-  const gp out = (gp)(POISSON && batch ? a.table->g[d] : XCHG && a.comp_blocks ? a.out_comp[comp] : a.out);
+  const gp out = (gp)(POISSON && batch ? a.table->g[d]
+                      : XCHG && a.comp_blocks ? a.out_comp[comp]
+                      : !XCHG && !POISSON && batch ? a.table->addend[d] : a.out);
   const gp npred_out = (gp)a.npred_out;
 
   float tu[WK], tv[WK];
@@ -451,7 +454,7 @@
 
 template <int WKT, int C, int P, bool POISSON, bool IN_SCALE, int XG, int XWT = XW>
 __global__ __launch_bounds__(XG ? 64 * XWT : 64) void walk_kernel(WalkArgs a) {
-  walk_body<WKT, C, P, POISSON, IN_SCALE, XG, XWT>(a, (int)blockIdx.x, a.strips, a.tiles_y, a.rows, 0);
+  walk_body<WKT, C, P, POISSON, IN_SCALE, XG, XWT>(a, (int)blockIdx.x, a.strips, a.tiles_y, a.rows, POISSON ? 0 : a.order0);
 }
 
 template <int C17, int P>
@@ -1121,6 +1124,19 @@
   return yes != 0 && yes != n * n_comp;
 }
 
+int sep_addend_split(int n, const SepBatchTable& table, int H, int W, int kh, int kw, int oy, int ox) {
+  if (opt_value(OPT_SEP_ADJ_ADDENDS, 1) == 0 || n < 2 || n > SEP_MAX_BATCH || !walk_enabled(H, W, n)) return n;
+  int first = n, f0 = 0;
+  for (int d = 0; d < n; ++d) {
+    const int f = dataset_frame(table, d, d, kh, kw, oy, ox);
+    if (!f) return n;
+    if (d == 0) f0 = f;
+    if (first == n && f != f0) first = d;
+    if (first != n && f == f0) return n;
+  }
+  return n - first <= SEP_ADDEND_MAX ? first : n;
+}
+
 int walk_conv(const float* in, const float* in_scale, const float* op, float* out, const float* out_scale, int H, int W,
               int kh, int kw, int oy, int ox, int adjoint, float coef, int accumulate, hipStream_t stream) {
   if (!walk_enabled(H, W, 1)) return JD_WALK_NOT_TAKEN;
@@ -1295,7 +1311,8 @@
 
 int walk_conv_adjoint_batch(int n, int n_comp, int comp, const SepBatchTable& table, const SepBatchTable* table_dev,
                             float* grad, int H, int W, int kh, int kw, int oy, int ox, float coef, int accumulate,
-                            hipStream_t stream, const double* fin_partials, double fin_scale, int fin_count, int* fin_done) {
+                            hipStream_t stream, const double* fin_partials, double fin_scale, int fin_count, int* fin_done,
+                            int addend_first, hipStream_t stream2, const hipEvent_t* fork_join) {
   *fin_done = 0;
   if (!walk_enabled(H, W, n * n_comp) || !aligned16(grad)) return JD_WALK_NOT_TAKEN;
   int frames[SEP_MAX_BATCH];
@@ -1310,10 +1327,58 @@
   walk_setup(a, kh, kw, oy, ox, 1);
   int rc = sep_guard_check(&a.guard);
   if (rc) return rc;
-  for (int d0 = 0; d0 < n;) {
+  int n_main = n;
+  hipEvent_t join = nullptr;
+  if (addend_first > 0 && addend_first < n) {
+    const int m = n - addend_first, frame = frames[addend_first];
+    if (n_comp != 1 || m > SEP_ADDEND_MAX || !table_dev) return fail(JD_ERR_INVALID, "walk_conv_adjoint_batch: not an addend split");
+    for (int d = addend_first; d < n; ++d)
+      if (frames[d] != frame || !table.addend[d] || !aligned16(table.addend[d]))
+        return fail(JD_ERR_INVALID, "walk_conv_adjoint_batch: not an addend split");
+    const bool beside = stream2 && stream2 != stream;
+    if (beside && !(fork_join && fork_join[0] && fork_join[1]))
+      return fail(JD_ERR_INVALID, "walk_conv_adjoint_batch: a second stream needs the caller's fork and join events");
+    const hipStream_t s2 = beside ? stream2 : stream;
+    WalkArgs b = a;
+    b.out = nullptr, b.n_batch = m, b.accumulate = 0;
+    b.order0 = frame == 33 ? table.n17 : 0;
+    int C1, r1;
+    walk_shape(b, m, true, frame, &C1, &r1);
+    if (beside) {
+      const long half = (long)(7.25 * device_cus()) / 2;
+      const int ws = frame == 33 ? Frame<33>::WS : Frame<17>::WS;
+      while (r1 < 4096 && (long)((W + 64 * C1 - 1) / (64 * C1)) * ((H + r1 - 1) / r1) * m > half) r1 += ws;
+    }
+    const int orows1 = opt_value(frame == 33 ? OPT_SEP_WALK_ADJ_ROWS33 : OPT_SEP_WALK_ADJ_ROWS, 0);
+    if (orows1 >= 20 && orows1 <= 4096) r1 = orows1;
+    walk_tiles(b, C1, r1);
+    if (beside) {
+      JD_HIP(hipEventRecord(fork_join[0], stream));
+      JD_HIP(hipStreamWaitEvent(stream2, fork_join[0], 0));
+    }
+    rc = launch_walk<false, false>(b, frame, C1, m, s2);
+    if (beside) {
+      join = fork_join[1];
+      const hipError_t e = hipEventRecord(join, s2);
+      if (e != hipSuccess) return rc ? rc : fail(JD_ERR_HIP, "hipEventRecord failed: %s", hipGetErrorString(e));
+    }
+    if (rc) {
+      if (join) (void)hipStreamWaitEvent(stream, join, 0);
+      return rc;
+    }
+    n_main = addend_first;
+  }
+  struct JoinOnExit {
+    hipStream_t stream;
+    hipEvent_t event;
+    ~JoinOnExit() {
+      if (event) (void)hipStreamWaitEvent(stream, event, 0);
+    }
+  } join_on_exit{stream, join};
+  for (int d0 = 0; d0 < n_main;) {
     const int frame = frames[d0];
     int m = 1;
-    while (d0 + m < n && m < XW && frames[d0 + m] == frame) ++m;
+    while (d0 + m < n_main && m < XW && frames[d0 + m] == frame) ++m;
     if (frame == 33 && opt_value(OPT_SEP_WALK_ADJ33, 0) == 1) m = 1;
     const int xg = m >= 6 ? 6 : m >= 3 ? 3 : 2;
     const bool wide = frame == 17 && m >= 6 && opt_value(OPT_SEP_WALK_ADJ_COLS, 4) != 2;
diff --git a/jolideco_amd/loss.py b/jolideco_amd/loss.py
--- a/jolideco_amd/loss.py
+++ b/jolideco_amd/loss.py
@@ -116,7 +116,8 @@
             )
         return cache[key]
 
-    def fwd_bwd_batch(self, indices, flux, loss_outs, grad=None, accumulate=False, grad_scale=1.0, flux_nonneg=False):
+    def fwd_bwd_batch(self, indices, flux, loss_outs, grad=None, accumulate=False, grad_scale=1.0, flux_nonneg=False,
+                      addends=None, side_stream=None):
         per_dataset = [list(self.npred_models_all[i].values()) for i in indices]
         single = torch.is_tensor(flux)
         if not single and len(flux) > 1 and flux_nonneg and not accumulate and self.mergeable(indices):
@@ -135,16 +136,17 @@
             )
             if grad is not None:
                 copy_image_to(grad[0], list(grad[1:]))
-            return
+            return 0
         exposures = [[m.exposure for m in models] for models in per_dataset]
         khats = [[m.khat for m in models] for models in per_dataset]
         if single:
             exposures, khats = [e[0] for e in exposures], [k[0] for k in khats]
-        per_dataset[0][0].plan.npred_poisson_batch_fwd_bwd(
+        return per_dataset[0][0].plan.npred_poisson_batch_fwd_bwd(
             flux=flux, exposures=exposures, khats=khats,
             backgrounds=[self.npred_models_all[i].background for i in indices],
             counts=[self.counts_all[i] for i in indices], stirlings=[self.stirling_all[i] for i in indices],
             loss_outs=loss_outs, grad=grad, accumulate=accumulate, grad_scale=grad_scale,
+            addends=addends if single else None, side_stream=side_stream,
         )
 
     @classmethod
diff --git a/jolideco_amd/ops.py b/jolideco_amd/ops.py
--- a/jolideco_amd/ops.py
+++ b/jolideco_amd/ops.py
@@ -242,7 +242,7 @@
     MAX_BATCH_COMPONENTS = 4
 
     def npred_poisson_batch_fwd_bwd(self, flux, exposures, khats, backgrounds, counts, stirlings, loss_outs, grad=None,
-                                    accumulate=False, grad_scale=1.0, eps=POISSON_EPS):
+                                    accumulate=False, grad_scale=1.0, eps=POISSON_EPS, addends=None, side_stream=None):
         n = len(exposures)
         if not (len(khats) == len(backgrounds) == len(counts) == len(stirlings) == len(loss_outs) == n):
             raise ValueError("all per-dataset lists must have the same length")
@@ -260,6 +260,23 @@
             raise ValueError("one gradient image per flux component")
         for f in fluxes:
             self._check_image(f, "flux")
+        if addends and single and grads is not None and n <= self.MAX_BATCH and not accumulate:
+            for image in addends:
+                self._check_image(image, "addend")
+            used = c_int(0)
+            images = list(addends)[: _hip.ADDEND_MAX]
+            images += [None] * (_hip.ADDEND_MAX - len(images))
+            stirling_arr = (c_float * n)(*[float(v) for v in stirlings])
+            check(
+                _hip.lib().jd_npred_poisson_batch_addends_fwd_bwd(
+                    self._handle, n, ptr(fluxes[0]), ptr_array([e[0] for e in exposures]), ptr_array([k[0] for k in khats]),
+                    ptr_array(backgrounds), ptr_array(counts), stirling_arr, c_float(eps), ptr_array(loss_outs), ptr(grads[0]),
+                    0, c_float(grad_scale), ptr_array(images),
+                    None if side_stream is None else c_void_p(side_stream.cuda_stream), ctypes.byref(used),
+                    stream_ptr(fluxes[0].device),
+                )
+            )
+            return used.value
         for start in range(0, n, self.MAX_BATCH):
             sl = slice(start, min(n, start + self.MAX_BATCH))
             m = sl.stop - sl.start
@@ -272,6 +289,7 @@
                     int(accumulate or start > 0), c_float(grad_scale), stream_ptr(fluxes[0].device),
                 )
             )
+        return 0
 
     def npred_poisson_calibrated_batch_fwd_bwd(self, flux, exposures, khats, backgrounds, counts, stirlings, loss_outs,
                                                calibrations, upsampling=1, grad=None, accumulate=False, grad_scale=1.0,
```

After: 1810 iters/s (median of 6 runs). 1.04x the previous value.
